# mmaker/c-lwe-snarks

Hardware: AMD Instinct MI355X
Metric: snark_proofs_per_sec (higher is better)
Workload: dtype u32 limbs (704-bit integers mod 2^704) + AES-256 bytes; int8 digits on the matrix cores, int32 accumulation (exact)

## Files before the change

### c-lwe-snarks_amd/__init__.py

```python
from __future__ import annotations

import ctypes
import os
from dataclasses import dataclass

import numpy as np

_HERE = os.path.dirname(os.path.abspath(__file__))
LIB_PATH = os.environ.get("MFHIP_LIB") or os.path.join(_HERE, "libmfhip.so")
P = 0xFFFFFFFB


class MfhError(RuntimeError):
    pass


@dataclass(frozen=True)
class Params:

    n: int = 1470
    logq: int = 736
    d: int = 1 << 15
    m: int = 21845

# ... 4 lines not shown
    @property
    def K(self):
        return self.logq // 64

    @property
    def lanes(self):
        return (64 * self.K + 55) // 56

    @property
    def ctb(self):
        return self.logq // 8

    @property
    def ctr_ct(self):
        return self.ctb * self.n

    @property
    def ctr_s(self):
        return 0

    @property
    def ctr_as(self):
        return self.ctr_ct * self.d

    @property
    def ctr_bt(self):
        return 2 * self.ctr_ct * self.d

    @property
    def ctr_bv(self):
        return 2 * self.ctr_ct * self.d + self.ctr_ct

    @property
    def ct_limbs(self):
        return (self.n + 1) * self.L


DEBUG = Params(d=256, m=64)
DEFAULT = Params()


class _CParams(ctypes.Structure):
    _fields_ = [("n", ctypes.c_uint32), ("logq", ctypes.c_uint32), ("d", ctypes.c_uint32), ("m", ctypes.c_uint32)]


_lib = None

EXPORTS = [
    "mfh_ctx_create", "mfh_ctx_destroy", "mfh_set_stream", "mfh_sync", "mfh_scrub_staging", "mfh_last_error", "mfh_set_seed",
    "mfh_keystream", "mfh_sample_rows", "mfh_ct_add", "mfh_ct_mul_ui", "mfh_ct_addmul_ui", "mfh_eval_rows",
    "mfh_encrypt_rows", "mfh_decrypt", "mfh_ct_smudge", "mfh_ssp_upload", "mfh_witness_poly", "mfh_version",
    "mfh_workspace_bytes", "mfh_last_kernel_ms", "mfh_set_timing", "mfh_set_overlap", "mfh_eval_rows_multi", "mfh_prove_batch", "mfh_crs_mm_image_bytes", "mfh_crs_expand_mm", "mfh_crs_set_resident_mm", "mfh_witness_poly_multi", "mfh_witness_poly_mm", "mfh_poly_h_multi", "mfh_poly_mul", "mfh_poly_add", "mfh_poly_prepare_t",
    "mfh_ssp_prepare", "mfh_poly_h", "mfh_setup_messages", "mfh_setup", "mfh_setup_image", "mfh_crs_image_set_b", "mfh_prove",
    "mfh_prove_partial", "mfh_prove_finish", "mfh_ct_to_lanes", "mfh_ct_from_lanes", "mfh_lanes_per_value", "mfh_digest128", "mfh_timing_drain", "mfh_timing_busy_ms", "mfh_timing_work_rows", "mfh_set_batch_image", "mfh_set_batch_slabs", "mfh_set_expand_path", "mfh_set_expand_periods", "mfh_set_encrypt_path", "mfh_set_batch_launch", "mfh_set_batch_bw", "mfh_set_mm_chunk_rows", "mfh_set_mm_pack", "mfh_set_poly_exact", "mfh_poly_exact_fallbacks", "mfh_poly_exact_points", "mfh_set_poly_exact_points", "mfh_set_mm_stream", "mfh_add_dotp", "mfh_set_encrypt_chunks", "mfh_set_witness_per", "mfh_set_eval_path", "mfh_set_decrypt_path", "mfh_decrypt_rows",
    "mfh_crs_mm_share_bytes", "mfh_crs_expand_mm_share", "mfh_crs_set_resident_mm_share", "mfh_batch_chain", "mfh_batch_witness_cols", "mfh_batch_chain_from_w", "mfh_witness_poly_mm_cols", "mfh_prove_batch_partial", "mfh_prove_batch_finish",
    "mfh_resident_row_bytes", "mfh_crs_expand", "mfh_eval_rows_resident", "mfh_crs_set_resident",
    "mfh_witness_lanes", "mfh_witness_from_lanes", "mfh_prove_partial_w", "mfh_verify",
    "mfh_ssp_set_prg", "mfh_ssp_prg_make_t", "mfh_ssp_prg_fill",
    "mfh_resident_share_rows", "mfh_crs_expand_share", "mfh_crs_set_resident_share", "mfh_crs_set_resident_prefix",
    "mfh_prove_batch_supergroup", "mfh_prove_batch_stream_wait", "mfh_set_mm_width", "mfh_set_mm_queue", "mfh_set_mm_claim_log", "mfh_mm_claim_log_launches",
    "mfh_setup_public", "mfh_prove_public", "mfh_prove_batch_public", "mfh_vk_derive", "mfh_verify_public",
    "mfh_ssp_from_rows", "mfh_ssp_set_rows", "mfh_ssp_rows_fill", "mfh_ssp_rows_violations", "mfh_circuit_create", "mfh_circuit_destroy", "mfh_circuit_assign",
    "mfh_circuit_create_global", "mfh_circuit_create_ex", "mfh_circuit_create_out", "mfh_circuit_create_sum",
    "mfh_merkle_create", "mfh_merkle_destroy", "mfh_merkle_set_leaves", "mfh_merkle_root", "mfh_merkle_nodes", "mfh_merkle_paths",
    "mfh_sha256_records", "mfh_merkle_set_records", "mfh_merkle_update_rows", "mfh_merkle_update_records",
    "mfh_merkle_absent_rows", "mfh_merkle_insert_keys", "mfh_merkle_update_rows_cut", "mfh_merkle_update_records_cut", "mfh_merkle_insert_keys_cut",
    "mfh_merkle_remove_keys", "mfh_merkle_remove_keys_cut", "mfh_merkle_transfer_keys", "mfh_merkle_transfer_keys_cut",
    "mfh_merkle_paths_cut", "mfh_merkle_absent_rows_cut", "mfh_merkle_range_rows", "mfh_merkle_range_rows_cut",
    "mfh_merkle_load_keys", "mfh_merkle_check_table", "mfh_merkle_grow", "mfh_merkle_grow_leaves",
]


OPTIONAL_EXPORTS = {
    "mfh_set_mm_queue": "tuning knob; older builds walk fixed lists",
    "mfh_set_mm_claim_log": "test instrumentation of mfh_set_mm_queue",
    "mfh_mm_claim_log_launches": "test instrumentation of mfh_set_mm_queue",
    "mfh_set_expand_periods": "test knob; older builds pick the periods per chunk from the row count",
}


def load_library():
    global _lib
    if _lib is not None:
        return _lib
    if not os.path.exists(LIB_PATH):
        raise MfhError(f"{LIB_PATH} is missing: run `python -c 'import __graft_entry__ as g; g.build()'` "
                       "(hipcc --offload-arch=gfx950).  There is no CPU fallback.")
    lib = ctypes.CDLL(LIB_PATH)
    vp, u64, sz, i32, u32 = ctypes.c_void_p, ctypes.c_uint64, ctypes.c_size_t, ctypes.c_int, ctypes.c_uint32
    sig = {
        "mfh_ctx_create": (i32, [ctypes.POINTER(vp), i32, ctypes.POINTER(_CParams)]),
        "mfh_ctx_destroy": (None, [vp]),
        "mfh_set_stream": (i32, [vp, vp]),
        "mfh_sync": (i32, [vp]),
        "mfh_scrub_staging": (i32, [vp]),
        "mfh_last_error": (ctypes.c_char_p, [vp]),
        "mfh_set_seed": (i32, [vp, ctypes.c_char_p]),
        "mfh_keystream": (i32, [vp, u64, vp, sz]),
        "mfh_sample_rows": (i32, [vp, u64, sz, vp]),
        "mfh_ct_add": (i32, [vp, vp, vp, vp, sz]),
        "mfh_ct_mul_ui": (i32, [vp, vp, vp, u32, sz]),
        "mfh_ct_addmul_ui": (i32, [vp, vp, vp, u32, sz]),
        "mfh_eval_rows": (i32, [vp, u64, sz, vp, vp, vp, vp, vp, i32]),
        "mfh_encrypt_rows": (i32, [vp, u64, sz, vp, vp, vp, vp]),
        "mfh_decrypt": (i32, [vp, vp, vp, sz, vp]),
        "mfh_ct_smudge": (i32, [vp, vp, sz, ctypes.c_char_p, sz, ctypes.c_char_p]),
        "mfh_ssp_upload": (i32, [vp, vp, vp, sz, sz]),
        "mfh_witness_poly": (i32, [vp, vp, ctypes.c_char_p, u32, vp]),
        "mfh_version": (ctypes.c_char_p, []),
        "mfh_workspace_bytes": (sz, [vp]),
        "mfh_last_kernel_ms": (ctypes.c_float, [vp, ctypes.c_char_p]),
        "mfh_set_timing": (i32, [vp, i32]),
        "mfh_set_overlap": (i32, [vp, i32]),
        "mfh_eval_rows_multi": (i32, [vp, u64, sz, vp, vp, u32, u32, vp, i32]),
        "mfh_poly_h_multi": (i32, [vp, vp, vp, u32]),
        "mfh_witness_poly_mm": (i32, [vp, vp, u32, ctypes.c_char_p, sz, vp, vp]),
        "mfh_witness_poly_multi": (i32, [vp, vp, u32, ctypes.c_char_p, sz, vp, vp]),
        "mfh_crs_mm_image_bytes": (sz, [vp]),
        "mfh_crs_expand_mm": (i32, [vp, vp, vp]),
        "mfh_crs_set_resident_mm": (i32, [vp, vp]),
        "mfh_prove_batch": (i32, [vp, vp, vp, u32, ctypes.c_char_p, sz, vp, ctypes.c_char_p, sz, ctypes.c_char_p, vp]),
        "mfh_prove_batch_supergroup": (u32, [vp]),
        "mfh_set_mm_width": (i32, [vp, u32, i32]),
        "mfh_set_mm_queue": (i32, [vp, i32, u32, i32]),
        "mfh_set_mm_claim_log": (i32, [vp, vp, sz]),
        "mfh_mm_claim_log_launches": (u32, [vp, ctypes.POINTER(u32), u32]),
        "mfh_prove_batch_stream_wait": (i32, [vp, u32, vp]),
        "mfh_poly_mul": (i32, [vp, vp, sz, vp, sz, vp]),
        "mfh_poly_add": (i32, [vp, vp, vp, sz, vp]),
        "mfh_poly_prepare_t": (i32, [vp, vp]),
        "mfh_ssp_prepare": (i32, [vp, vp]),
        "mfh_poly_h": (i32, [vp, vp, vp]),
        "mfh_setup_messages": (i32, [vp, vp, u32, u32, u32, vp]),
        "mfh_setup": (i32, [vp, vp, u32, u32, u32, vp, vp, vp]),
        "mfh_setup_image": (i32, [vp, vp, u32, u32, u32, vp, vp, vp, vp]),
        "mfh_prove": (i32, [vp, vp, vp, ctypes.c_char_p, u32, ctypes.c_char_p, sz, ctypes.c_char_p, vp]),
        "mfh_prove_partial": (i32, [vp, vp, vp, ctypes.c_char_p, u32, u32, u32, vp]),
        "mfh_prove_finish": (i32, [vp, vp, ctypes.c_char_p, sz, ctypes.c_char_p]),
        "mfh_lanes_per_value": (u32, [vp]),
        "mfh_digest128": (i32, [vp, vp, sz, vp]),
        "mfh_ct_to_lanes": (i32, [vp, vp, sz, vp]),
        "mfh_ct_from_lanes": (i32, [vp, vp, sz, vp]),
        "mfh_add_dotp": (i32, [vp, vp, vp, vp, sz]),
        "mfh_crs_set_resident_prefix": (i32, [vp, vp, sz]),
        "mfh_resident_share_rows": (sz, [vp, u32, u32]),
        "mfh_crs_expand_share": (i32, [vp, vp, u32, u32, vp]),
        "mfh_crs_set_resident_share": (i32, [vp, vp, u32, u32]),
        "mfh_ssp_set_prg": (i32, [vp, u64, vp]),
        "mfh_ssp_prg_make_t": (i32, [vp, u64, ctypes.c_char_p, vp]),
        "mfh_ssp_prg_fill": (i32, [vp, u64, sz, sz, vp]),
        "mfh_verify": (i32, [vp, vp, u32, u32, u32, vp, vp, sz, vp]),
        "mfh_witness_lanes": (i32, [vp, vp, ctypes.c_char_p, u32, u32, vp]),
        "mfh_witness_from_lanes": (i32, [vp, vp, vp, u32, vp]),
        "mfh_prove_partial_w": (i32, [vp, vp, vp, ctypes.c_char_p, u32, u32, u32, vp, vp]),
        "mfh_resident_row_bytes": (sz, [vp]),
        "mfh_crs_expand": (i32, [vp, u64, sz, vp, vp]),
        "mfh_crs_image_set_b": (i32, [vp, sz, sz, vp, vp]),
        "mfh_eval_rows_resident": (i32, [vp, vp, sz, sz, vp, vp, vp, vp, i32]),
        "mfh_crs_set_resident": (i32, [vp, vp]),
        "mfh_timing_drain": (i32, [vp, ctypes.c_char_p, ctypes.POINTER(u64), ctypes.POINTER(ctypes.c_double), ctypes.POINTER(u64),
                                   ctypes.POINTER(ctypes.c_float)]),
        "mfh_timing_busy_ms": (ctypes.c_double, [vp]),
        "mfh_timing_work_rows": (u64, [vp]),
        "mfh_set_batch_image": (i32, [vp, i32]),
        "mfh_set_mm_chunk_rows": (i32, [vp, u32]),
        "mfh_set_mm_pack": (i32, [vp, i32]),
        "mfh_set_poly_exact": (i32, [vp, i32]),
        "mfh_poly_exact_fallbacks": (ctypes.c_long, [vp]),
        "mfh_poly_exact_points": (i32, [vp, ctypes.POINTER(u32)]),
        "mfh_set_poly_exact_points": (i32, [vp, ctypes.POINTER(u32)]),
        "mfh_set_mm_stream": (i32, [vp, i32, i32, i32, u32]),
        "mfh_set_batch_launch": (i32, [vp, u32, i32]),
        "mfh_set_batch_bw": (i32, [vp, i32]),
        "mfh_set_encrypt_path": (i32, [vp, i32]),
        "mfh_set_expand_path": (i32, [vp, i32]),
        "mfh_set_expand_periods": (i32, [vp, u32]),
        "mfh_set_batch_slabs": (i32, [vp, u32]),
        "mfh_set_encrypt_chunks": (i32, [vp, u32]),
        "mfh_set_eval_path": (i32, [vp, i32]),
        "mfh_set_decrypt_path": (i32, [vp, i32]),
        "mfh_decrypt_rows": (i32, [vp, u64, sz, vp, vp, vp]),
        "mfh_set_witness_per": (i32, [vp, u32]),
        "mfh_crs_mm_share_bytes": (sz, [vp, u32, u32]),
        "mfh_crs_expand_mm_share": (i32, [vp, vp, u32, u32, vp]),
        "mfh_crs_set_resident_mm_share": (i32, [vp, vp, u32, u32]),
        "mfh_batch_chain": (i32, [vp, vp, u32, ctypes.c_char_p, sz, vp, vp, vp, vp]),
        "mfh_batch_witness_cols": (i32, [vp, vp, u32, ctypes.c_char_p, sz, vp, u32, u32, vp, sz]),
        "mfh_batch_chain_from_w": (i32, [vp, vp, u32, vp, vp, vp]),
        "mfh_witness_poly_mm_cols": (i32, [vp, vp, u32, ctypes.c_char_p, sz, vp, u32, u32, vp, sz]),
        "mfh_prove_batch_partial": (i32, [vp, vp, u32, u32, u32, ctypes.c_char_p, sz, vp, vp, vp, sz, vp]),
        "mfh_prove_batch_finish": (i32, [vp, vp, u32, vp, ctypes.c_char_p, sz, ctypes.c_char_p, vp]),
        "mfh_setup_public": (i32, [vp, vp, u32, u32, u32, u32, vp, vp, vp, vp]),
        "mfh_prove_public": (i32, [vp, vp, vp, u32, ctypes.c_char_p, u32, ctypes.c_char_p, sz, ctypes.c_char_p, vp]),
        "mfh_prove_batch_public": (i32, [vp, vp, vp, u32, u32, ctypes.c_char_p, sz, vp, ctypes.c_char_p, sz, ctypes.c_char_p, vp]),
        "mfh_vk_derive": (i32, [vp, vp, u32, u32, vp]),
        "mfh_verify_public": (i32, [vp, vp, u32, u32, u32, vp, vp, ctypes.c_char_p, sz, sz, vp]),
        "mfh_ssp_from_rows": (i32, [vp, u32, vp, vp, vp, vp]),
        "mfh_ssp_set_rows": (i32, [vp, u32, vp, vp, vp, u32]),
        "mfh_ssp_rows_fill": (i32, [vp, sz, sz, vp]),
        "mfh_ssp_rows_violations": (i32, [vp, u32, vp, sz, vp, vp]),
        "mfh_circuit_create": (i32, [vp, u32, u32, vp, u32, vp, ctypes.POINTER(vp)]),
        "mfh_circuit_create_global": (i32, [vp, u32, u32, vp, u32, vp, ctypes.POINTER(vp)]),
        "mfh_circuit_create_ex": (i32, [vp, u32, u32, vp, u32, vp, u32, vp, u32, ctypes.POINTER(vp)]),
        "mfh_circuit_create_out": (i32, [vp, u32, u32, vp, u32, vp, u32, vp, u32, vp, u32, ctypes.POINTER(vp)]),
        "mfh_circuit_create_sum": (i32, [vp, u32, u32, vp, u32, vp, u32, vp, u32, vp, u32, vp, u32, ctypes.POINTER(vp)]),
        "mfh_circuit_destroy": (None, [vp]),
        "mfh_circuit_assign": (i32, [vp, vp, u32, vp, sz, vp, sz, vp]),
        "mfh_merkle_create": (i32, [vp, u32, ctypes.POINTER(vp)]),
        "mfh_merkle_destroy": (None, [vp]),
        "mfh_merkle_set_leaves": (i32, [vp, vp, u32, u32, vp]),
        "mfh_merkle_root": (i32, [vp, vp, vp]),
        "mfh_merkle_nodes": (i32, [vp, u32, ctypes.POINTER(vp)]),
        "mfh_merkle_paths": (i32, [vp, vp, u32, vp, vp, sz]),
        "mfh_sha256_records": (i32, [vp, vp, sz, u32, u32, vp]),
        "mfh_merkle_set_records": (i32, [vp, vp, u32, u32, vp, sz, u32]),
        "mfh_merkle_update_rows": (i32, [vp, vp, u32, vp, vp, vp, sz, vp]),
        "mfh_merkle_update_records": (i32, [vp, vp, u32, vp, vp, sz, u32, vp, sz, vp, sz, vp]),
        "mfh_merkle_absent_rows": (i32, [vp, vp, vp, sz, u32, u32, u32, vp, sz, vp, sz, vp, vp]),
        "mfh_merkle_insert_keys": (i32, [vp, vp, vp, sz, u32, u32, u32, vp, sz, vp, sz, vp, sz, vp, vp, vp]),
        "mfh_merkle_update_rows_cut": (i32, [vp, vp, u32, vp, vp, u32, vp, vp, vp, vp]),
        "mfh_merkle_update_records_cut": (i32, [vp, vp, u32, vp, vp, sz, u32, vp, sz, u32, vp, vp, vp, vp]),
        "mfh_merkle_insert_keys_cut": (i32, [vp, vp, vp, sz, u32, u32, u32, vp, sz, vp, sz, u32, vp, vp, vp, vp, vp, vp]),
        "mfh_merkle_remove_keys": (i32, [vp, vp, vp, sz, u32, u32, u32, vp, sz, vp, sz, vp, vp, vp]),
        "mfh_merkle_remove_keys_cut": (i32, [vp, vp, vp, sz, u32, u32, u32, vp, sz, u32, vp, vp, vp, vp, vp, vp]),
        "mfh_merkle_transfer_keys": (i32, [vp, vp, vp, sz, u32, u32, u32, u32, vp, vp, sz, vp, vp, sz, vp, vp, vp]),
        "mfh_merkle_transfer_keys_cut": (i32, [vp, vp, vp, sz, u32, u32, u32, u32, vp, vp, sz, vp, u32, vp, vp, vp, vp, vp, vp]),
# ... 784 lines not shown

    def sync(self):
        self._chk(self.lib.mfh_sync(self._h))

    def set_stream(self, stream):
        self._chk(self.lib.mfh_set_stream(self._h, ctypes.c_void_p(stream.cuda_stream if stream is not None else 0)))

    def scrub_staging(self):
        rc = self.lib.mfh_scrub_staging(self._h)
        self._chk(rc)
        return rc

    def workspace_bytes(self):
        return int(self.lib.mfh_workspace_bytes(self._h))

    def set_timing(self, on=True):
        self._chk(self.lib.mfh_set_timing(self._h, 1 if on else 0))

    def set_overlap(self, mode=1):
        self._chk(self.lib.mfh_set_overlap(self._h, int(mode)))

    def set_batch_image(self, on=True):
        self._chk(self.lib.mfh_set_batch_image(self._h, 1 if on else 0))

    def set_batch_slabs(self, nslabs=0):
        self._chk(self.lib.mfh_set_batch_slabs(self._h, int(nslabs)))

    def set_expand_path(self, path=0):
        self._chk(self.lib.mfh_set_expand_path(self._h, int(path)))

    def set_expand_periods(self, periods=0):
        if not 0 <= int(periods) <= 0xFFFFFFFF:
            raise MfhError("set_expand_periods: 0 or 2 .. 10")
        self._chk(self.lib.mfh_set_expand_periods(self._h, int(periods)))

    def set_encrypt_path(self, path=0):
        self._chk(self.lib.mfh_set_encrypt_path(self._h, int(path)))

    def set_eval_path(self, path=0):
        self._chk(self.lib.mfh_set_eval_path(self._h, int(path)))

    def set_encrypt_chunks(self, chunks=0):
        self._chk(self.lib.mfh_set_encrypt_chunks(self._h, int(chunks)))

    def set_witness_per(self, statements=0):
        self._chk(self.lib.mfh_set_witness_per(self._h, int(statements)))

    def set_batch_launch(self, groups_per_launch=4, merge_regions=True):
        self._chk(self.lib.mfh_set_batch_launch(self._h, int(groups_per_launch), 1 if merge_regions else 0))

    def set_batch_bw(self, merged=True):
        self._chk(self.lib.mfh_set_batch_bw(self._h, 1 if merged else 0))

    def set_mm_stream(self, map=0, persistent=False, sync_mode=0, spin_max=64):
        self._chk(self.lib.mfh_set_mm_stream(self._h, int(map), int(persistent), int(sync_mode), int(spin_max)))

    def set_mm_width(self, per_xcd=32, early_chain=False):
        self._chk(self.lib.mfh_set_mm_width(self._h, int(per_xcd), 1 if early_chain else 0))

    def set_mm_queue(self, mode=1, start_shift=0, prefix=-8):
        self._chk(self.lib.mfh_set_mm_queue(self._h, int(mode), int(start_shift), int(prefix)))

    def set_mm_claim_log(self, log):
        if log is None:
            self._chk(self.lib.mfh_set_mm_claim_log(self._h, None, 0))
        else:
            self._chk(self.lib.mfh_set_mm_claim_log(self._h, log.data_ptr(), log.numel()))

    def mm_claim_log_launches(self):
        out = (ctypes.c_uint32 * (16 * 12))()
        n = int(self.lib.mfh_mm_claim_log_launches(self._h, out, 16))
        keys = ("offset", "nchunks", "nblk", "ngt", "ngr", "map", "tgs", "width", "coeff_bytes", "queue", "prefix", "shift")
        return [dict(zip(keys, (int(x) for x in out[12 * i:12 * i + 12]))) for i in range(n)]

    def set_mm_pack(self, on=True):
        self._chk(self.lib.mfh_set_mm_pack(self._h, 1 if on else 0))

    def set_poly_exact(self, mode=1):
        self._chk(self.lib.mfh_set_poly_exact(self._h, int(mode)))

    def poly_exact_fallbacks(self):
        return int(self.lib.mfh_poly_exact_fallbacks(self._h))

    def exact_points(self):
        out = (ctypes.c_uint32 * 4)()
        self._chk(self.lib.mfh_poly_exact_points(self._h, out))
        return [int(x) for x in out]

    def set_exact_points(self, pts):
        if pts is None:
            self._chk(self.lib.mfh_set_poly_exact_points(self._h, None))
            return
        pts = [int(x) for x in pts]
        if len(pts) != 4 or not all(0 <= x < 2**32 for x in pts):
            raise MfhError(f"set_exact_points: four uint32 values, got {pts!r}")
        self._chk(self.lib.mfh_set_poly_exact_points(self._h, (ctypes.c_uint32 * 4)(*pts)))

    def set_mm_chunk_rows(self, rows=0):
        self._chk(self.lib.mfh_set_mm_chunk_rows(self._h, int(rows)))

    def timing_drain(self, which):
        n, rows, ms, last = ctypes.c_uint64(), ctypes.c_uint64(), ctypes.c_double(), ctypes.c_float()
        self._chk(self.lib.mfh_timing_drain(self._h, which.encode(), ctypes.byref(n), ctypes.byref(ms), ctypes.byref(rows), ctypes.byref(last)))
        return n.value, ms.value, rows.value

    def timing_busy_ms(self):
# ... 196 lines not shown
    def poly_h(self, d_v):
        out = self.empty(self.params.d * 4)
        self._chk(self.lib.mfh_poly_h(self._h, _ptr(d_v), _ptr(out)))
        return out

    def poly_h_many(self, d_v, nb):
        out = self.empty(nb * self.params.d * 4)
        self._chk(self.lib.mfh_poly_h_multi(self._h, _ptr(d_v), _ptr(out), nb))
        return out

    def setup_messages(self, d_ssp, alpha, beta, s):
        p = self.params
        out = self.empty((2 * p.d + p.m) * 4)
        self._chk(self.lib.mfh_setup_messages(self._h, _ptr(d_ssp), alpha, beta, s, _ptr(out)))
        return out

    def setup(self, d_ssp, alpha, beta, s, d_sk, d_err, out=None):
        p = self.params
        out = self.empty((2 * p.d + p.m) * p.ctb) if out is None else out
        self._chk(self.lib.mfh_setup(self._h, _ptr(d_ssp), alpha, beta, s, _ptr(d_sk), _ptr(d_err), _ptr(out)))
        return out

    def setup_image(self, d_ssp, alpha, beta, s, d_sk, d_err, out=None, rows=None):
        p = self.params
        out = self.empty((2 * p.d + p.m) * p.ctb) if out is None else out
        rows = self.empty((2 * p.d + p.m) * self.resident_row_bytes()) if rows is None else rows
        self._chk(self.lib.mfh_setup_image(self._h, _ptr(d_ssp), alpha, beta, s, _ptr(d_sk), _ptr(d_err), _ptr(out), _ptr(rows)))
        return out, rows

    def prove(self, d_crs, d_ssp, witness_bits: bytes, delta, smudge_mag: bytes, smudge_sign: bytes, maglen=80, out=None):
        p = self.params
        out = self.empty(5 * p.ct_limbs * 8) if out is None else out
        assert len(smudge_mag) == 5 * maglen and len(smudge_sign) == 5
        self._chk(self.lib.mfh_prove(self._h, _ptr(d_crs), _ptr(d_ssp), bytes(witness_bits), delta, bytes(smudge_mag), maglen,
                                     bytes(smudge_sign), _ptr(out)))
        return out

    def crs_expand_mm(self, d_crs, out=None):
        out = self.empty(int(self.lib.mfh_crs_mm_image_bytes(self._h))) if out is None else out
        self._chk(self.lib.mfh_crs_expand_mm(self._h, _ptr(d_crs), _ptr(out)))
        return out

    def set_resident_mm(self, image):
        self._resident_mm = image
        self._chk(self.lib.mfh_crs_set_resident_mm(self._h, _ptr(image)))

    def witness_poly_many(self, d_ssp, witness_bits_list, deltas, mm=True):
        p = self.params
        nb = len(witness_bits_list)
        stride = (p.m + 6) // 8
        bits = b"".join(bytes(w[:stride]).ljust(stride, b"\0") for w in witness_bits_list)
        dl = (ctypes.c_uint32 * nb)(*[int(x) for x in deltas])
        out = self.empty(nb * p.d * 4)
        fn = self.lib.mfh_witness_poly_mm if mm else self.lib.mfh_witness_poly_multi
        self._chk(fn(self._h, _ptr(d_ssp), nb, bits, stride, ctypes.cast(dl, ctypes.c_void_p), _ptr(out)))
        return out

    def prove_batch(self, d_crs, d_ssp, witness_bits_list, deltas, smudge_mags, smudge_signs, maglen=80, out=None):
        p = self.params
        nb = len(witness_bits_list)
        stride = (p.m + 6) // 8
        bits = b"".join(bytes(w[:stride]).ljust(stride, b"\0") for w in witness_bits_list)
        dl = (ctypes.c_uint32 * nb)(*[int(x) for x in deltas])
        mags = b"".join(bytes(x) for x in smudge_mags)
        signs = b"".join(bytes(x) for x in smudge_signs)
        assert len(mags) == nb * 5 * maglen and len(signs) == nb * 5
        out = self.empty(nb * 5 * p.ct_limbs * 8) if out is None else out
        self._chk(self.lib.mfh_prove_batch(self._h, _ptr(d_crs), _ptr(d_ssp), nb, bits, stride, ctypes.cast(dl, ctypes.c_void_p), mags, maglen,
                                           signs, _ptr(out)))
        return out

    def prove_batch_supergroup(self):
        return int(self.lib.mfh_prove_batch_supergroup(self._h))

    def prove_batch_stream_wait(self, upto, stream):
        self._chk(self.lib.mfh_prove_batch_stream_wait(self._h, int(upto), ctypes.c_void_p(stream.cuda_stream)))

    def _pack_bits(self, witness_bits_list):
        stride = (self.params.m + 6) // 8
        return b"".join(bytes(w[:stride]).ljust(stride, b"\0") for w in witness_bits_list), stride

    def crs_expand_mm_share(self, d_crs, rank, world, out=None):
        out = self.empty(int(self.lib.mfh_crs_mm_share_bytes(self._h, rank, world))) if out is None else out
        self._chk(self.lib.mfh_crs_expand_mm_share(self._h, _ptr(d_crs), rank, world, _ptr(out)))
        return out

    def set_resident_mm_share(self, image, rank, world):
        self._resident_mm = image
        self._chk(self.lib.mfh_crs_set_resident_mm_share(self._h, _ptr(image), rank, world))

    def batch_chain(self, d_ssp, witness_bits_list, deltas, out=None):
        p = self.params
        nb = len(witness_bits_list)
        out = self.torch.empty((3, nb, p.d), dtype=self.torch.int32, device=self.device) if out is None else out
        if nb == 0:
            return out
        bits, stride = self._pack_bits(witness_bits_list)
        dl = (ctypes.c_uint32 * nb)(*[int(x) for x in deltas])
        self._chk(self.lib.mfh_batch_chain(self._h, _ptr(d_ssp), nb, bits, stride, ctypes.cast(dl, ctypes.c_void_p), _ptr(out[0]), _ptr(out[1]), _ptr(out[2])))
        return out

    def batch_witness_cols(self, d_ssp, witness_bits_list, deltas, col0, ncols, out=None):
        nb = len(witness_bits_list)
        out = self.torch.empty((nb, ncols), dtype=self.torch.int32, device=self.device) if out is None else out
        if nb == 0 or ncols == 0:
            return out
        bits, stride = self._pack_bits(witness_bits_list)
# ... 178 lines not shown
```

### c-lwe-snarks_amd/csrc/ctx.hpp

```cpp
#pragma once
#include <hip/hip_runtime.h>

#include <stdint.h>
#include <string.h>

#include <string>
#include <vector>

#include "aes_dev.hpp"
#include "mfhip.h"
#include "ssp_prg.hpp"

#define HIP_TRY(ctx, expr)                                                        \
  do {                                                                            \
    hipError_t e_ = (expr);                                                       \
    if (e_ != hipSuccess) {                                                       \
      (ctx)->err = std::string(#expr) + ": " + hipGetErrorString(e_);             \
      return MFH_EDEVICE;                                                         \
    }                                                                             \
  } while (0)

struct PolyState;
struct SspInterp;
struct SspRows;
// ... 12 lines not shown
  size_t cap = 0;
  template <class T> T *as() const { return static_cast<T *>(p); }
};

struct mfh_ctx {
  mfh_params P{};
  int device = 0;
  hipStream_t own_stream = nullptr;
  hipStream_t stream = nullptr;
  mf::AesKey key{};
  bool have_seed = false;
  uint32_t *d_t0 = nullptr;
  DevBuf ws;
  DevBuf ws2;
  int mm_ws_sel = 0;
  DevBuf ws3;
  std::vector<hipEvent_t> ev_cdone, ev_rdone, ev_wdone;
  std::vector<hipEvent_t> ev_round;
  std::vector<hipEvent_t> ev_sgdone;
  uint32_t last_batch_sg = 0, last_batch_n = 0;
  DevBuf wws;
  DevBuf lazy;
  uint32_t *lazy_cnt = nullptr;
  bool eval_dense = false;
  bool overlap = true;
  int overlap_mode = 1;
  hipStream_t side = nullptr, side2 = nullptr;
  hipEvent_t ev_fork = nullptr, ev_join = nullptr;
  hipEvent_t ev_chain = nullptr, ev_chain_done = nullptr;
  std::string err;
  bool timing = false;
  struct Timed {
    hipEvent_t e0, e1;
    int kind;
    uint64_t rows;
    uint64_t work;
    int sub;
  };
  std::vector<Timed> timed;
  double last_busy_ms = 0;
  uint64_t last_work_rows = 0;
  std::vector<hipEvent_t> ev_pool;
  PolyState *poly = nullptr;
  DevBuf aux;
  DevBuf d_msg;
  DevBuf d_prover;
  std::vector<uint32_t> h_cw;
  const uint8_t *mm_image = nullptr;
  uint32_t mm_rank = 0, mm_world = 1;
  uint64_t mm_off[3] = {0, 0, 0}, mm_rows[3] = {0, 0, 0};
  size_t mm_base[3] = {0, 0, 0};
  DevBuf ssp_frag;
  const uint32_t *ssp_frag_src = nullptr;
  SspInterp *interp = nullptr;
  DevBuf circ_io;
  DevBuf circ_state;
  DevBuf d_batch;
  DevBuf batch_img;
  int batch_image = 1;
  int mm_map = 1;
  bool mm_persist = true;
  bool mm_wave1 = false;
  uint32_t mm_sync_mode = 0, mm_spin = 64;
  uint32_t mm_width = 32;
  size_t early_ws_half = 0;
  bool batch_early_chain = false;
  uint32_t *mm_sync = nullptr;
  uint32_t mm_queue = 1, mm_queue_shift = 0; int mm_queue_prefix = -8;
  uint32_t *mm_log = nullptr; size_t mm_log_words = 0, mm_log_used = 0; uint32_t mm_log_n = 0, mm_log_desc[16][12];
  int poly_exact = 1;
  bool poly_pts_pinned = false;
  uint32_t poly_pts[4] = {0, 0, 0, 0};
  bool mm_pack = true;
  uint32_t mm_chunk_rows = 131071;
  int expand_path = 0;
  uint32_t expand_periods = 0;
  int enc_path = 0;
  uint32_t ncu = 256;
  int dec_path = 0;
  int eval_path = 0;
  uint32_t enc_chunks = 0;
  uint32_t witness_per = 0;
  uint32_t batch_slabs = 0;
  int batch_bw_merged = 1;
  int batch_merge = 1;
  uint32_t batch_ngl = 8;
  PinBuf pin_rows, pin_cw, pin_smudge;
  PinBuf pin_pub;
  DevBuf d_pub;
  PinBuf pin_wring[8];
  uint32_t pin_wnext = 0;
  hipEvent_t ev_sample = nullptr;
  DevBuf sample_tmp;
  void *uploader = nullptr;
  bool prg_on = false;
  uint64_t prg_seed = 0;
  const uint32_t *prg_t = nullptr;
  SspRows *rows = nullptr;
  RowsTree *rows_tree = nullptr;
  const uint32_t *rows_prefix = nullptr;
  uint32_t rows_lu_max = 0;
  const uint8_t *resident_rows = nullptr;
  uint64_t resident_nrows = ~0ull;
  bool resident_sharded = false;
  uint32_t res_rank = 0, res_world = 1;
};

struct Timer {
  mfh_ctx *c;
  mfh_ctx::Timed t{};
  bool on;
  Timer(mfh_ctx *c_, int kind, uint64_t rows, uint64_t work = 0, int sub = 0) : c(c_), on(c_->timing) {
    if (!on) return;
    auto get = [&]() {
      hipEvent_t e;
      if (!c->ev_pool.empty()) { e = c->ev_pool.back(); c->ev_pool.pop_back(); }
      else hipEventCreate(&e);
      return e;
    };
    t.e0 = get(); t.e1 = get(); t.kind = kind; t.rows = rows; t.work = work ? work : rows; t.sub = sub;
    hipEventRecord(t.e0, c->stream);
  }
  ~Timer() {
    if (!on) return;
    hipEventRecord(t.e1, c->stream);
    c->timed.push_back(t);
  }
};

inline void *pin_acquire(mfh_ctx *c, PinBuf &b, size_t bytes) {
  if (b.pending) { hipEventSynchronize(b.ev); b.pending = false; }
  if (bytes > b.cap) {
    if (b.p) hipHostFree(b.p);
    b.cap = (bytes + 4095) & ~(size_t)4095;
    if (hipHostMalloc(&b.p, b.cap, hipHostMallocDefault) != hipSuccess) { b.p = nullptr; b.cap = 0; c->err = "hipHostMalloc failed"; return nullptr; }
  }
  if (!b.ev) hipEventCreateWithFlags(&b.ev, hipEventDisableTiming);
  b.used = bytes;
  return b.p;
}
inline void pin_release(mfh_ctx *c, PinBuf &b) {
  hipEventRecord(b.ev, c->stream);
  b.pending = true;
}
inline void pin_scrub(PinBuf &b) {
  if (b.pending) { hipEventSynchronize(b.ev); b.pending = false; }
  if (b.p && b.used) {
    volatile unsigned char *q = (volatile unsigned char *)b.p;
    memset((void *)q, 0, b.used);
    __asm__ __volatile__("" : : "r"(b.p) : "memory");
  }
  b.used = 0;
}
inline void pin_free(PinBuf &b) {
  if (b.pending) hipEventSynchronize(b.ev);
  if (b.p) hipHostFree(b.p);
  if (b.ev) hipEventDestroy(b.ev);
  b = PinBuf();
}

// ... 55 lines not shown
    return MFH_OK;
  }
  if (!c->prg_on || !c->prg_t) { c->err = "d_ssp is NULL and no generator-defined SSP is registered (mfh_ssp_set_prg)"; return MFH_EINVAL; }
  src = mf::SspSrc{nullptr, c->prg_t, c->prg_seed};
  return MFH_OK;
}

void mfh_poly_destroy(mfh_ctx *c);
void ssp_interp_free(mfh_ctx *c);
void ssp_rows_free(mfh_ctx *c, bool tree);
int ssp_rows_check(mfh_ctx *c, const char *who, uint32_t nrows, const uint32_t *h_row_ptr, const uint32_t *h_wire, const uint32_t *h_coef);
int ssp_rows_tree(mfh_ctx *c, const char *who, const uint32_t *&d_t, const uint32_t *&h_w);
int ssp_rows_witness(mfh_ctx *c, uint32_t nstmt, const uint8_t *h_bits, size_t bits_stride, const uint32_t *h_delta, uint32_t *d_w, size_t w_stride);
int ssp_rows_msg_evals(mfh_ctx *c, uint32_t s, uint32_t beta, uint32_t *d_msg_evals);
inline bool ssp_is_rows(const mfh_ctx *c, const uint32_t *d_ssp) { return !d_ssp && c->rows_prefix; }
inline int ssp_rows_lu_check(mfh_ctx *c, const uint32_t *d_ssp, uint32_t lu) {
  if (ssp_is_rows(c, d_ssp) && lu > c->rows_lu_max) { c->err = "lu exceeds the lu_max the row SSP was registered with (mfh_ssp_set_rows)"; return MFH_EINVAL; }
  return MFH_OK;
}
extern "C" int mfh_witness_poly_mm(mfh_ctx *c, const uint32_t *d_ssp, uint32_t nstmt, const uint8_t *h_bits, size_t bits_stride, const uint32_t *h_delta,
                                   uint32_t *d_w);
extern "C" int mfh_witness_poly_mm_cols(mfh_ctx *c, const uint32_t *d_ssp, uint32_t nstmt, const uint8_t *h_bits, size_t bits_stride, const uint32_t *h_delta,
                                        uint32_t col0, uint32_t ncols, uint32_t *d_w, size_t w_stride);
extern "C" int mfh_poly_h_multi(mfh_ctx *c, const uint32_t *d_v, uint32_t *d_h, uint32_t nb);
int expand_mm_region(mfh_ctx *c, uint64_t off, uint32_t nrows, const uint8_t *c8, uint8_t *image);
int encrypt_rows_mm(mfh_ctx *c, uint64_t off, size_t nrows, const uint64_t *sk, const uint32_t *msg, const uint64_t *err, uint8_t *c8);
int decrypt_mm(mfh_ctx *c, const uint64_t *sk, const uint64_t *cts, size_t count, uint32_t *out);
int decrypt_rows_mm(mfh_ctx *c, uint64_t off, size_t nrows, const uint64_t *sk, const uint8_t *c8, uint32_t *out);

struct MmIo {
  const uint32_t *coef[2];
  uint32_t csplit;
  uint64_t *out[2];
  uint32_t osplit;
  uint64_t ostride;
  const uint8_t *bits;
  uint32_t bits_stride;
  int64_t *sc_zeroed;
  uint64_t cstride;
  uint32_t bits_row0;
  const uint64_t *add_ct;
  const uint32_t *add_scale;
  uint32_t sa_from1;
};
int eval_rows_multi_io(mfh_ctx *c, uint64_t off, size_t nrows, const uint8_t *d_c8, const MmIo &io, uint32_t nvec, uint32_t coeff_bytes, int accumulate);
int eval_rows_multi_io_set(mfh_ctx *c, uint64_t off, size_t nrows, const uint8_t *d_c8, const MmIo *ios, const uint32_t *nvecs, uint32_t ng,
                           uint32_t coeff_bytes);
struct MmRegion { uint64_t off; const uint8_t *c8; };
int eval_rows_multi_io_regions(mfh_ctx *c, const MmRegion *regs, uint32_t nreg, size_t nrows, const MmIo *ios, const uint32_t *nvecs, uint32_t ng,
                               uint32_t coeff_bytes, int accumulate);
bool mm_image_covers(const mfh_ctx *c, uint64_t off, size_t nrows);
struct MmsPlan {
  uint32_t ng, ngt, ND, nrows, nchunks, rpc, rpad, ntiles, mtiles;
  size_t cd_bytes, part_bytes;
  const uint8_t *img[2];
  int8_t *cd;
  int *part;
};
bool mms_plan(mfh_ctx *c, const MmRegion *regs, uint32_t nreg, size_t nrows, const MmIo *ios, const uint32_t *nvecs, uint32_t ng, uint32_t coeff_bytes,
              MmsPlan &P);
size_t mms_ws_bytes(const MmsPlan &P);
void mms_bind(MmsPlan &P, void *ws);
int mms_digits(mfh_ctx *c, const MmsPlan &P, const MmIo *ios, const uint32_t *nvecs);
int mms_stream(mfh_ctx *c, const MmsPlan &P);
int mms_finish(mfh_ctx *c, const MmsPlan &P, const MmIo *ios, const uint32_t *nvecs, int accumulate);
```

### c-lwe-snarks_amd/csrc/evalmm.hip

```cpp
#include <algorithm>
#include <cstring>

#include "ctx.hpp"
#include "mms_slots.hpp"

namespace {

using mf::AesKey;

constexpr int CT = 4;
constexpr int SB = 88;
constexpr int VB = 92;
constexpr int MB = CT * SB;
constexpr int MT = MB / 32;
constexpr int RT = 128;
constexpr int TSTRIDE = 384;
constexpr int BLK_PER_ROW = 24;
static_assert(MB % 32 == 0 && CT * VB + 15 <= TSTRIDE, "tile geometry");

typedef int v4i __attribute__((ext_vector_type(4)));
typedef int v16i __attribute__((ext_vector_type(16)));

__device__ __forceinline__ uint32_t coef_at(const MmIo &io, uint32_t v, uint32_t nrows, uint32_t i) {
  if (io.bits) {
// ... 943 lines not shown
      sv[l][1][vl] = (uint32_t)(val >> 32);
      sv[l][2][vl] = (uint32_t)(val >> 64);
    }
  }
  __syncthreads();
  if (lq != 0 || v >= nvec) return;
  uint32_t *out = reinterpret_cast<uint32_t *>((v < io.osplit ? io.out[0] + (uint64_t)v * io.ostride : io.out[1] + (uint64_t)(v - io.osplit) * io.ostride) +
                                               (uint64_t)j * LL);
  const bool wide4 = (LL & 1) == 0 && (io.ostride & 1) == 0 && ((reinterpret_cast<uintptr_t>(io.out[0]) | reinterpret_cast<uintptr_t>(io.out[1])) & 15) == 0;
  uint32_t pend[4] = {0, 0, 0, 0};
  uint64_t carry = 0;
  const uint32_t *actw = io.add_ct ? reinterpret_cast<const uint32_t *>(io.add_ct + (uint64_t)j * LL) : nullptr;
  const uint64_t ax = io.add_ct ? io.add_scale[v] : 0;
  uint64_t acarry = 0;
  for (uint32_t l = 0; l < KWv; l++) {
    uint64_t word = carry + sv[l][0][vl];
    if (l >= 1) word += sv[l - 1][1][vl];
    if (l >= 2) word += sv[l - 2][2][vl];
    if (accumulate) word += out[l];
    if (actw) {
      const uint64_t t = (uint64_t)actw[l] * ax + acarry;
      word += (uint32_t)t;
      acarry = t >> 32;
    }
    carry = word >> 32;
    pend[l & 3] = (uint32_t)word;
    if (wide4 ? (l & 3) == 3 : (l & 1) == 1) {
      if (wide4) *reinterpret_cast<uint4 *>(out + (l & ~3u)) = uint4{pend[0], pend[1], pend[2], pend[3]};
      else *reinterpret_cast<uint2 *>(out + (l & ~1u)) = uint2{pend[(l & 2)], pend[(l & 2) + 1]};
    }
  }
  if (wide4) {
    if (KWv & 3) *reinterpret_cast<uint4 *>(out + (KWv & ~3u)) = uint4{pend[0], (KWv & 3) > 1 ? pend[1] : 0u, (KWv & 3) > 2 ? pend[2] : 0u, 0u};
    for (uint32_t l = (KWv + 3) & ~3u; l < 2 * LL; l += 4) *reinterpret_cast<uint4 *>(out + l) = uint4{0u, 0u, 0u, 0u};
  } else {
    if (KWv & 1) *reinterpret_cast<uint2 *>(out + (KWv & ~1u)) = uint2{pend[(KWv & 2)], 0u};
    for (uint32_t l = (KWv + 1) & ~1u; l < 2 * LL; l += 2) *reinterpret_cast<uint2 *>(out + l) = uint2{0u, 0u};
  }
}

template <int ND, int KWM, bool PK>
__global__ __launch_bounds__(256) void k_evalmm_finish(const int *__restrict__ part, const int64_t *__restrict__ sc, uint32_t nchunks, uint32_t ntiles,
                                                        uint32_t N, uint32_t nvec, uint32_t n, uint32_t nrows, uint32_t ct, uint32_t MBv, uint32_t sby,
                                                        uint32_t LL, MmIo io, int accumulate) {
  evalmm_finish_body<ND, KWM, PK>(part, sc, nchunks, ntiles, N, nvec, n, nrows, ct, MBv, sby, LL, io, accumulate, part, ND * nvec);
}
template <int ND, int KWM, bool PK>
__global__ __launch_bounds__(256) void k_evalmm_finish_groups(const int *__restrict__ part, uint64_t part_stride, uint32_t nchunks, uint32_t ntiles, uint32_t N,
                                                               uint32_t n, uint32_t nrows, uint32_t ct, uint32_t MBv, uint32_t sby, uint32_t LL, MmGroupArgs A,
                                                               int accumulate) {
  const uint32_t g = blockIdx.z, lender = A.io[g].sa_from1 ? A.io[g].sa_from1 - 1 : g;
  evalmm_finish_body<ND, KWM, PK>(part + g * part_stride, A.io[g].sc_zeroed, nchunks, ntiles, N, A.nvec[g], n, nrows, ct, MBv, sby, LL, A.io[g], accumulate,
                                  part + lender * part_stride, ND * A.nvec[lender]);
}

}

extern "C" {

struct WideGeom { uint32_t ct, sby, vby, mt, mbp, LL; };
static WideGeom wide_geom(const mfh_ctx *c) {
  if (c->P.logq == 736) return {W16<736>::CT, W16<736>::SBY, W16<736>::VBY, W16<736>::MT, W16<736>::MBP, W16<736>::LL};
  return {W16<1472>::CT, W16<1472>::SBY, W16<1472>::VBY, W16<1472>::MT, W16<1472>::MBP, W16<1472>::LL};
}

#define FINISH_LAUNCH(kern, ND_, PK_, grid, ...)                                                                         \
  do {                                                                                                                   \
    if ((PK_) && wg.sby / 4 <= 22) hipLaunchKernelGGL((kern<ND_, 22, true>), grid, dim3(256), 0, c->stream, __VA_ARGS__);  \
    else if (PK_) hipLaunchKernelGGL((kern<ND_, 46, true>), grid, dim3(256), 0, c->stream, __VA_ARGS__);                 \
    else if (wg.sby / 4 <= 22) hipLaunchKernelGGL((kern<ND_, 22, false>), grid, dim3(256), 0, c->stream, __VA_ARGS__);   \
    else hipLaunchKernelGGL((kern<ND_, 46, false>), grid, dim3(256), 0, c->stream, __VA_ARGS__);                         \
  } while (0)

int mfh_eval_rows_multi(mfh_ctx *c, uint64_t off, size_t nrows, const uint8_t *d_c8, const uint32_t *d_coeffs, uint32_t nvec, uint32_t coeff_bytes,
                        uint64_t *d_rops, int accumulate) {
  if (!c || !d_rops || !nvec || (nrows && (!d_c8 || !d_coeffs)) || (coeff_bytes != 1 && coeff_bytes != 4)) return MFH_EINVAL;
  const MmIo io = {{d_coeffs, nullptr}, nvec, {d_rops, nullptr}, nvec, (uint64_t)(c->P.n + 1) * wide_geom(c).LL, nullptr, 0, nullptr};
  return eval_rows_multi_io(c, off, nrows, d_c8, io, nvec, coeff_bytes, accumulate);
}

}

int eval_rows_multi_io(mfh_ctx *c, uint64_t off, size_t nrows, const uint8_t *d_c8, const MmIo &io, uint32_t nvec, uint32_t coeff_bytes, int accumulate) {
  if (!c || !nvec || !io.out[0] || (io.osplit < nvec && !io.out[1]) || (coeff_bytes != 1 && coeff_bytes != 4)) return MFH_EINVAL;
  if (nrows && (!d_c8 || (!io.bits && (!io.coef[0] || (io.csplit < nvec && !io.coef[1]))) || (io.bits && coeff_bytes != 1))) return MFH_EINVAL;
  const uint32_t ND = coeff_bytes;
  const uint32_t n = c->P.n;
  const bool q736 = c->P.logq == 736;
  const WideGeom wg = wide_geom(c);
  const uint8_t *img_region = nullptr;
  for (int r = 0; r < 3 && c->mm_image; r++)
    if (c->mm_off[r] == off && c->mm_rows[r] == nrows && nrows) img_region = c->mm_image + c->mm_base[r];
  const bool wide = img_region || !q736 || nvec * ND + 1 > 128;
  if (nvec * ND + 1 > 256) { c->err = "mfh_eval_rows_multi: at most 63 four-byte (255 one-byte) coefficient vectors per call (256 digit columns)"; return MFH_EINVAL; }
  if (wide && ((off & 7) || (((uint64_t)n * wg.vby) & 7))) {
    c->err = "mfh_eval_rows_multi: the 256-column kernel needs off and the row length to be multiples of 8";
    return MFH_EINVAL;
  }
  if (!c->have_seed) { c->err = "mfh_set_seed has not been called"; return MFH_EINVAL; }
  if (nrows > 0xffffffffu - 256) return MFH_EINVAL;
  HIP_TRY(c, hipSetDevice(c->device));
  const size_t ctl = (size_t)(n + 1) * wg.LL;
  if (io.ostride < ctl) return MFH_EINVAL;
  if (nrows == 0) {
    const uint32_t n0 = std::min(nvec, io.osplit);
    if (!accumulate) {
// ... 100 lines not shown
}
size_t mms_ws_bytes(const MmsPlan &P) { return (size_t)P.ngt * (P.cd_bytes + P.part_bytes); }
void mms_bind(MmsPlan &P, void *ws) {
  P.cd = (int8_t *)ws;
  P.part = (int *)((uint8_t *)ws + (size_t)P.ngt * P.cd_bytes);
}
static bool mms_group_args(const MmsPlan &P, const MmIo *ios, const uint32_t *nvecs, MmGroupArgs &A) {
  if (P.ND != 4) return false;
  for (uint32_t g = 0; g < P.ngt; g++) {
    if (ios[g].bits) return false;
    A.io[g] = ios[g];
    A.nvec[g] = nvecs[g];
  }
  return true;
}
int mms_digits(mfh_ctx *c, const MmsPlan &P, const MmIo *ios, const uint32_t *nvecs) {
  MmGroupArgs A;
  if (mms_group_args(P, ios, nvecs, A)) {
    hipLaunchKernelGGL(k_mm_digits4w_groups, dim3((P.rpad / 16 + DG4 - 1) / DG4, P.ngt), dim3(256), 0, c->stream, A, P.nrows, P.rpad, P.cd, (uint64_t)P.cd_bytes);
    HIP_TRY(c, hipGetLastError());
    return MFH_OK;
  }
  for (uint32_t g = 0; g < P.ngt; g++) {
    if (P.ND == 4 && !ios[g].bits)
      hipLaunchKernelGGL(k_mm_digits4w, dim3((P.rpad / 16 + DG4 - 1) / DG4), dim3(256), 0, c->stream, ios[g], nvecs[g], P.nrows, P.rpad, P.cd + g * P.cd_bytes,
                         ios[g].sc_zeroed);
    else
      hipLaunchKernelGGL(k_mm_digits, dim3((P.rpad / 16 + DG_RG - 1) / DG_RG), dim3(N2), 0, c->stream, ios[g], nvecs[g], P.ND, P.nrows, P.rpad, (uint32_t)NQ2, 1,
                         P.cd + g * P.cd_bytes, ios[g].sc_zeroed);
  }
  HIP_TRY(c, hipGetLastError());
  return MFH_OK;
}
static bool mms_persistent(const mfh_ctx *c, const MmsPlan &P) {
  return P.ngt > 1 && c->mm_persist && c->ncu == 256 && ((c->mm_map && 32 % P.ng == 0) || 32 % P.ngt == 0);
}
static uint32_t mms_pk(const mfh_ctx *c, const MmsPlan &P) {
  if (!c->mm_pack || (mms_persistent(c, P) && c->mm_wave1)) return 0;
  return P.ND;
}
#ifdef MMS_ITEM_STAMPS
static unsigned long long *g_mms_stamps = nullptr;
static uint32_t g_mms_stamp_n = 0, g_mms_stamp_kind[64];
static unsigned long long *mms_stamps_next(uint32_t nd, uint32_t queue) {
  if (!g_mms_stamps && hipMalloc(&g_mms_stamps, 64 * 256 * 4 * sizeof(unsigned long long)) != hipSuccess) return nullptr;
  if (g_mms_stamp_n == 64) return nullptr;
  g_mms_stamp_kind[g_mms_stamp_n] = nd | queue << 8;
  return g_mms_stamps + (size_t)g_mms_stamp_n++ * 256 * 4;
}
#endif
int mms_stream(mfh_ctx *c, const MmsPlan &P) {
  const uint32_t KS = (P.nrows + RT2 - 1) / RT2 * (RT2 / 64), tgs = (P.mtiles + TPW - 1) / TPW;
  const bool will_persist = mms_persistent(c, P);
  Timer t(c, P.ngt > 1 ? (P.ND == 1 ? 14 : 10) : 8, P.nrows, (uint64_t)P.nrows * P.ngt, will_persist ? 1 : 0);
  MmsImages imgs{};
  for (uint32_t g = 0; g < P.ngt; g++) imgs.image[g] = (const v4i *)P.img[g / P.ng];
  const uint32_t pk = mms_pk(c, P);
  if (P.ngt > 1) {
    const uint32_t map = c->mm_map && 32 % P.ng == 0 ? 1u : 0u;
    const uint32_t slots = mms_slots(tgs, P.ngt, P.ng, map);
    const bool persistent = will_persist;
    if (persistent && c->mm_wave1) {
      hipLaunchKernelGGL(k_mmstream_w, dim3(256), dim3(WSW * 64), 0, c->stream, imgs, P.mtiles, KS, P.nrows, P.rpc, (const v4i *)P.cd, P.part, P.ngt, P.ng, map,
                         (uint64_t)(P.cd_bytes / 16), (uint64_t)(P.part_bytes / 4), (slots + 31) / 32, P.nchunks);
    } else if (persistent) {
      constexpr size_t SYNC_WORDS = 8 * 32 + 2 * 8;
      if (!c->mm_sync) HIP_TRY(c, hipMalloc(&c->mm_sync, SYNC_WORDS * sizeof(uint32_t)));
      const uint32_t width = P.ND == 1 ? 32u : c->mm_width;
      const uint32_t sync_mode = width == 32 ? c->mm_sync_mode : 0u, nblk = (slots + 31) / 32;
      uint32_t *qctr = c->mm_sync + 8 * 32 + 8 * (c->mm_ws_sel ? 1 : 0);
      MmsQueue q{qctr, nullptr, c->mm_queue && !sync_mode ? 1u : 0u, c->mm_queue_shift & 7, 0u, tgs};
      if (q.mode && !q.shift && nblk * 32 % width == 0) {
        const uint32_t rounds = P.nchunks * (nblk * 32 / width);
        q.prefix = c->mm_queue_prefix < 0 ? rounds - std::min(rounds, (uint32_t)-(int64_t)c->mm_queue_prefix) : std::min(rounds, (uint32_t)c->mm_queue_prefix);
      }
      if (sync_mode) HIP_TRY(c, hipMemsetAsync(c->mm_sync, 0, 8 * 32 * sizeof(uint32_t), c->stream));
      else if (q.mode) HIP_TRY(c, hipMemsetAsync(qctr, 0, 8 * sizeof(uint32_t), c->stream));
      if (c->mm_log) {
        const size_t need = (size_t)2 * P.nchunks * 8 * nblk * 32;
        if (c->mm_log_n == 16 || c->mm_log_used + need > c->mm_log_words) { c->err = "mfh_set_mm_claim_log: the log is too small for the call's launches"; return MFH_EINVAL; }
        q.log = c->mm_log + c->mm_log_used;
        const uint32_t desc[12] = {(uint32_t)c->mm_log_used, P.nchunks, nblk, P.ngt, P.ng, map, tgs, width, P.ND, q.mode, q.prefix, q.shift};
        memcpy(c->mm_log_desc[c->mm_log_n++], desc, sizeof(desc));
        c->mm_log_used += need;
      }
#ifdef MMS_ITEM_STAMPS
      unsigned long long *stamps = mms_stamps_next(P.ND, q.mode);
      if (!stamps) { c->err = "MMS_ITEM_STAMPS: no room for another launch"; return MFH_EINVAL; }
#endif
      hipLaunchKernelGGL(P.ND == 1 ? k_mmstream_pb : k_mmstream_p, dim3(8 * width), dim3(SW * 64), 0, c->stream, imgs, P.mtiles, KS, P.nrows, P.rpc, (const v4i *)P.cd, P.part, P.ngt, P.ng, map,
                         (uint64_t)(P.cd_bytes / 16), (uint64_t)(P.part_bytes / 4), nblk, P.nchunks, c->mm_sync, sync_mode, c->mm_spin, width, pk, q MMS_STAMP_ARG);
    } else {
      hipLaunchKernelGGL(k_mmstream, dim3(slots * 8, P.nchunks), dim3(SW * 64), 0, c->stream, imgs, P.mtiles, KS, P.nrows, P.rpc, (const v4i *)P.cd, P.part, P.ngt, P.ng,
                         map, (uint64_t)(P.cd_bytes / 16), (uint64_t)(P.part_bytes / 4), pk);
    }
  } else
    hipLaunchKernelGGL(k_mmstream1, dim3((tgs + 7) / 8 * 8, P.nchunks), dim3(SW * 64), 0, c->stream, imgs, P.mtiles, KS, P.nrows, P.rpc, (const v4i *)P.cd, P.part, pk);
  HIP_TRY(c, hipGetLastError());
  return MFH_OK;
}
int mms_finish(mfh_ctx *c, const MmsPlan &P, const MmIo *ios, const uint32_t *nvecs, int accumulate) {
  const WideGeom wg = wide_geom(c);
  const uint32_t n = c->P.n;
  const uint32_t pk = mms_pk(c, P);
  MmGroupArgs A;
  if (mms_group_args(P, ios, nvecs, A)) {
    uint32_t nvmax = 0;
    for (uint32_t g = 0; g < P.ngt; g++) nvmax = std::max(nvmax, nvecs[g]);
    FINISH_LAUNCH(k_evalmm_finish_groups, 4, pk, dim3(n + 1, (nvmax + 63) / 64, P.ngt), P.part, (uint64_t)(P.part_bytes / 4), P.nchunks, P.ntiles, (uint32_t)N2, n, P.nrows,
                  wg.ct, wg.mbp, wg.sby, wg.LL, A, accumulate);
    HIP_TRY(c, hipGetLastError());
    return MFH_OK;
  }
  for (uint32_t g = 0; g < P.ngt; g++) {
    const dim3 fgrid(n + 1, (nvecs[g] + 63) / 64);
    int *pg = P.part + g * (P.part_bytes / 4);
    if (P.ND == 4)
      FINISH_LAUNCH(k_evalmm_finish, 4, pk, fgrid, pg, ios[g].sc_zeroed, P.nchunks, P.ntiles, (uint32_t)N2, nvecs[g], n, P.nrows, wg.ct, wg.mbp, wg.sby, wg.LL, ios[g],
                    accumulate);
    else
      FINISH_LAUNCH(k_evalmm_finish, 1, pk, fgrid, pg, ios[g].sc_zeroed, P.nchunks, P.ntiles, (uint32_t)N2, nvecs[g], n, P.nrows, wg.ct, wg.mbp, wg.sby, wg.LL, ios[g],
                    accumulate);
  }
  HIP_TRY(c, hipGetLastError());
  return MFH_OK;
}
int eval_rows_multi_io_regions(mfh_ctx *c, const MmRegion *regs, uint32_t nreg, size_t nrows, const MmIo *ios, const uint32_t *nvecs, uint32_t ng,
                               uint32_t coeff_bytes, int accumulate) {
  if (!c || !regs || !ios || !nvecs || !ng || !nreg || nreg * ng > 16) return MFH_EINVAL;
  MmsPlan P;
  if (!mms_plan(c, regs, nreg, nrows, ios, nvecs, ng, coeff_bytes, P)) {
    for (uint32_t g = 0; g < nreg * ng; g++) {
      int rc = eval_rows_multi_io(c, regs[g / ng].off, nrows, regs[g / ng].c8, ios[g], nvecs[g], coeff_bytes, accumulate);
      if (rc) return rc;
    }
    return MFH_OK;
  }
  HIP_TRY(c, hipSetDevice(c->device));
  int rc = c->mm_ws_sel ? ws2_reserve(c, mms_ws_bytes(P)) : ws_reserve(c, mms_ws_bytes(P));
  if (rc) return rc;
  mms_bind(P, (c->mm_ws_sel ? c->ws2 : c->ws).p);
  rc = mms_digits(c, P, ios, nvecs);
  if (!rc) rc = mms_stream(c, P);
  if (!rc) rc = mms_finish(c, P, ios, nvecs, accumulate);
  return rc;
}
int eval_rows_multi_io_set(mfh_ctx *c, uint64_t off, size_t nrows, const uint8_t *d_c8, const MmIo *ios, const uint32_t *nvecs, uint32_t ng,
                           uint32_t coeff_bytes) {
  const MmRegion reg = {off, d_c8};
  return eval_rows_multi_io_regions(c, &reg, 1, nrows, ios, nvecs, ng, coeff_bytes, 0);
}
bool mm_image_covers(const mfh_ctx *c, uint64_t off, size_t nrows) {
  for (int r = 0; r < 3 && c->mm_image; r++)
    if (c->mm_off[r] == off && c->mm_rows[r] == nrows && nrows) return true;
  return false;
}

extern "C" {

static size_t mm_region_bytes(const mfh_ctx *c, uint64_t rows) {
  const WideGeom wg = wide_geom(c);
  const uint64_t mtiles = (uint64_t)((c->P.n + 1 + wg.ct - 1) / wg.ct) * wg.mt, ksteps = (rows + RT2 - 1) / RT2 * (RT2 / 64);
  return (size_t)(mtiles * ksteps * 1024);
}
struct MmShare { uint64_t row0[3], rows[3]; };
static MmShare mm_share(const mfh_ctx *c, uint32_t rank, uint32_t world) {
  const uint64_t d = c->P.d, m = c->P.m;
  const uint64_t loS = d * rank / world, cS = d * (rank + 1) / world - loS, lo = m * rank / world, cnt = m * (rank + 1) / world - lo;
  return MmShare{{loS, d + loS, 2 * d + lo}, {cS, cS, cnt}};
}
size_t mfh_crs_mm_share_bytes(const mfh_ctx *c, uint32_t rank, uint32_t world) {
  if (!c || !world || rank >= world) return 0;
  const MmShare sh = mm_share(c, rank, world);
  return mm_region_bytes(c, sh.rows[0]) + mm_region_bytes(c, sh.rows[1]) + mm_region_bytes(c, sh.rows[2]);
}
size_t mfh_crs_mm_image_bytes(const mfh_ctx *c) { return mfh_crs_mm_share_bytes(c, 0, 1); }
int mfh_crs_expand_mm_share(mfh_ctx *c, const uint8_t *d_crs_c8, uint32_t rank, uint32_t world, uint8_t *d_image) {
  if (!c || !d_crs_c8 || !d_image || !world || rank >= world) return MFH_EINVAL;
  if (!c->have_seed) { c->err = "mfh_set_seed has not been called"; return MFH_EINVAL; }
// ... 115 lines not shown
```

### c-lwe-snarks_amd/csrc/mfhip.hip

```cpp
#include <hip/hip_runtime.h>

#include <stdint.h>
#include <stdio.h>
#include <string.h>

#include <algorithm>
#include <string>
#include <thread>
#include <vector>

#include "aes_dev.hpp"
#include "mfhip.h"

using mf::AesKey;

template <int LOGQ>
struct PS {
  static constexpr int CTB = LOGQ / 8;
  static constexpr int EW = CTB / 4;
  static constexpr int L = (LOGQ + 63) / 64;
  static constexpr int K = LOGQ / 64;
  static constexpr int KW = 2 * K;
  static constexpr int TILE = LOGQ == 736 ? 512 : 256;
  static constexpr int ROWS = 2;
// ... 819 lines not shown
  if (P->logq != 736 && P->logq != 1472) return MFH_EUNSUPPORTED;
  if (P->n == 0 || P->n > (1u << 20)) return MFH_EINVAL;
  int ndev = 0;
  if (hipGetDeviceCount(&ndev) != hipSuccess || ndev <= 0 || device < 0 || device >= ndev) return MFH_EDEVICE;
  if (hipSetDevice(device) != hipSuccess) return MFH_EDEVICE;
  mfh_ctx *c = new mfh_ctx();
  c->P = *P;
  c->device = device;
  {
    int ncu = 0;
    if (hipDeviceGetAttribute(&ncu, hipDeviceAttributeMultiprocessorCount, device) == hipSuccess && ncu > 0) c->ncu = (uint32_t)ncu;
  }
  if (hipStreamCreateWithFlags(&c->own_stream, hipStreamNonBlocking) != hipSuccess) {
    delete c;
    return MFH_EDEVICE;
  }
  c->stream = c->own_stream;
  uint32_t t0[512];
  mf::make_t0_le(t0);
  for (int a = 0; a < 256; a++) t0[256 + a] = (t0[a] << 24) | (t0[a] >> 8);
  if (hipMalloc(&c->d_t0, sizeof t0) != hipSuccess || hipMemcpy(c->d_t0, t0, sizeof t0, hipMemcpyHostToDevice) != hipSuccess) {
    mfh_ctx_destroy(c);
    return MFH_EDEVICE;
  }
  *out = c;
  return MFH_OK;
}

void mfh_ctx_destroy(mfh_ctx *c) {
  if (!c) return;
  hipSetDevice(c->device);
  if (c->stream) hipStreamSynchronize(c->stream);
  mfh_poly_destroy(c);
  ssp_interp_free(c);
  ssp_rows_free(c, true);
  upload_free(c);
  if (c->ev_sample) hipEventDestroy(c->ev_sample);
  pin_free(c->pin_rows);
  for (auto &b : c->pin_wring) pin_free(b);
  pin_free(c->pin_cw);
  pin_free(c->pin_smudge);
  pin_free(c->pin_pub);
  if (c->side) hipStreamSynchronize(c->side);
  if (c->mm_sync) hipFree(c->mm_sync);
  for (hipEvent_t e : c->ev_round) hipEventDestroy(e);
  for (hipEvent_t e : c->ev_sgdone) hipEventDestroy(e);
  for (hipEvent_t e : c->ev_cdone) hipEventDestroy(e);
  for (hipEvent_t e : c->ev_rdone) hipEventDestroy(e);
  for (hipEvent_t e : c->ev_wdone) hipEventDestroy(e);
  if (c->ev_fork) hipEventDestroy(c->ev_fork);
  if (c->ev_join) hipEventDestroy(c->ev_join);
  if (c->ev_chain) hipEventDestroy(c->ev_chain);
  if (c->ev_chain_done) hipEventDestroy(c->ev_chain_done);
  if (c->side) hipStreamDestroy(c->side);
  if (c->side2) hipStreamDestroy(c->side2);
  for (DevBuf *b : {&c->ws, &c->ws2, &c->ws3, &c->wws, &c->lazy, &c->aux, &c->d_msg, &c->d_prover, &c->d_pub, &c->d_batch, &c->batch_img, &c->circ_io,
                    &c->circ_state, &c->ssp_frag, &c->sample_tmp})
    dev_free(*b);
  if (c->d_t0) hipFree(c->d_t0);
  for (auto &t : c->timed) { hipEventDestroy(t.e0); hipEventDestroy(t.e1); }
  for (auto e : c->ev_pool) hipEventDestroy(e);
  if (c->own_stream) hipStreamDestroy(c->own_stream);
  delete c;
}

int mfh_set_stream(mfh_ctx *c, void *s) {
  if (!c) return MFH_EINVAL;
  c->stream = (hipStream_t)s;
  return MFH_OK;
}

int mfh_sync(mfh_ctx *c) {
  if (!c) return MFH_EINVAL;
  HIP_TRY(c, hipStreamSynchronize(c->stream));
  return MFH_OK;
}

int mfh_scrub_staging(mfh_ctx *c) {
  if (!c) return MFH_EINVAL;
  pin_scrub(c->pin_rows);
  pin_scrub(c->pin_cw);
  pin_scrub(c->pin_smudge);
  for (auto &b : c->pin_wring) pin_scrub(b);
  return MFH_OK;
}

const char *mfh_last_error(const mfh_ctx *c) { return c ? c->err.c_str() : "null context"; }
size_t mfh_workspace_bytes(const mfh_ctx *c) { return c ? c->ws.cap : 0; }
int mfh_set_overlap(mfh_ctx *c, int en) {
  if (!c) return MFH_EINVAL;
  c->overlap = en != 0;
  c->overlap_mode = en > 1 ? en : 1;
  return MFH_OK;
}

int mfh_set_expand_path(mfh_ctx *c, int path) {
  if (!c || path < 0 || path > 1) return MFH_EINVAL;
  c->expand_path = path;
  return MFH_OK;
}

int mfh_set_expand_periods(mfh_ctx *c, uint32_t periods) {
  if (!c || (periods && (periods < EXPAND_MIN_PERIODS || periods > EXPAND_MAX_PERIODS))) return MFH_EINVAL;
  c->expand_periods = periods;
  return MFH_OK;
}

int mfh_set_encrypt_path(mfh_ctx *c, int path) {
  if (!c || path < 0 || path > 2) return MFH_EINVAL;
  c->enc_path = path;
  return MFH_OK;
}

int mfh_set_eval_path(mfh_ctx *c, int path) {
  if (!c || path < 0 || path > 1) return MFH_EINVAL;
  c->eval_path = path;
  return MFH_OK;
}
int mfh_set_encrypt_chunks(mfh_ctx *c, uint32_t chunks) {
  if (!c || chunks > 64) return MFH_EINVAL;
  c->enc_chunks = chunks;
  return MFH_OK;
}
int mfh_set_witness_per(mfh_ctx *c, uint32_t statements) {
  if (!c || (statements && (statements < 32 || statements > 256))) return MFH_EINVAL;
  c->witness_per = statements;
  return MFH_OK;
}
int mfh_set_batch_slabs(mfh_ctx *c, uint32_t nslabs) {
  if (!c || nslabs > 256) return MFH_EINVAL;
  c->batch_slabs = nslabs;
  return MFH_OK;
}

int mfh_set_batch_launch(mfh_ctx *c, uint32_t groups_per_launch, int merge_regions) {
  if (!c || groups_per_launch < 1 || groups_per_launch > 8) return MFH_EINVAL;
  c->batch_ngl = groups_per_launch;
  c->batch_merge = merge_regions != 0;
  return MFH_OK;
}

int mfh_set_batch_bw(mfh_ctx *c, int merged) {
  if (!c) return MFH_EINVAL;
  c->batch_bw_merged = merged != 0;
  return MFH_OK;
}

int mfh_set_batch_image(mfh_ctx *c, int en) {
  if (!c) return MFH_EINVAL;
  c->batch_image = en != 0;
  return en ? MFH_OK : batch_img_drop(c);
}

int mfh_set_timing(mfh_ctx *c, int en) {
  if (!c) return MFH_EINVAL;
  c->timing = en != 0;
  return MFH_OK;
}
static int timing_kind(const char *which) {
  if (!strcmp(which, "keystream")) return 0;
  if (!strcmp(which, "eval1")) return 1;
  if (!strcmp(which, "eval2")) return 2;
  if (!strcmp(which, "encrypt")) return 3;
  if (!strcmp(which, "eval")) return 12;
  if (!strcmp(which, "expand")) return 4;
  if (!strcmp(which, "mac1")) return 5;
  if (!strcmp(which, "mac2")) return 6;
  if (!strcmp(which, "evalmm")) return 7;
  if (!strcmp(which, "evalmm_resident")) return 8;
  if (!strcmp(which, "expandmm")) return 9;
  if (!strcmp(which, "decrypt")) return 11;
  if (!strcmp(which, "decrypt_rows")) return 13;
  if (!strcmp(which, "mmstream_bw")) return 14;
  if (!strcmp(which, "mmstream_rounds")) return 10;
  if (!strcmp(which, "mmstream_rounds_persistent")) return 110;
  if (!strcmp(which, "mmstream_bw_persistent")) return 114;
  if (!strcmp(which, "ssp_interp")) return 15;
  if (!strcmp(which, "circuit_assign")) return 16;
  if (!strcmp(which, "circuit_assign_global")) return 17;
  if (!strcmp(which, "circuit_assign_ex")) return 18;
  if (!strcmp(which, "circuit_assign_global_ex")) return 19;
  if (!strcmp(which, "circuit_assign_out")) return 20;
  if (!strcmp(which, "circuit_assign_global_out")) return 21;
  if (!strcmp(which, "circuit_assign_sum")) return 22;
  if (!strcmp(which, "circuit_assign_global_sum")) return 23;
  if (!strcmp(which, "ssp_rows_violations")) return 24;
  if (!strcmp(which, "merkle_level")) return 25;
  if (!strcmp(which, "merkle_paths")) return 26;
  if (!strcmp(which, "sha256_records")) return 27;
  if (!strcmp(which, "merkle_updates")) return 28;
  if (!strcmp(which, "merkle_record_rows")) return 29;
  if (!strcmp(which, "merkle_locate")) return 30;
  if (!strcmp(which, "merkle_absent_rows")) return 31;
  if (!strcmp(which, "merkle_inert")) return 32;
  if (!strcmp(which, "merkle_insert_records")) return 33;
  if (!strcmp(which, "merkle_segments")) return 34;
  if (!strcmp(which, "merkle_owners")) return 35;
  if (!strcmp(which, "merkle_remove_records")) return 36;
  if (!strcmp(which, "merkle_balances")) return 37;
  if (!strcmp(which, "merkle_transfer_records")) return 38;
  if (!strcmp(which, "merkle_climb_rows")) return 39;
  if (!strcmp(which, "merkle_range")) return 40;
  if (!strcmp(which, "merkle_range_order")) return 41;
  if (!strcmp(which, "merkle_adjust_records")) return 42;
  if (!strcmp(which, "merkle_balance_sum")) return 43;
  if (!strcmp(which, "merkle_sort")) return 44;
  if (!strcmp(which, "merkle_load")) return 45;
  if (!strcmp(which, "merkle_check")) return 46;
  if (!strcmp(which, "merkle_grow")) return 47;
  return -1;
}

int mfh_timing_drain(mfh_ctx *c, const char *which, uint64_t *count, double *total_ms, uint64_t *total_rows, float *last_ms) {
  if (!c || !which) return MFH_EINVAL;
  const int kind = timing_kind(which);
  if (kind < 0) return MFH_EINVAL;
  HIP_TRY(c, hipStreamSynchronize(c->stream));
  if (c->side) HIP_TRY(c, hipStreamSynchronize(c->side));
  uint64_t n = 0, rows = 0, work = 0;
  double tot = 0;
  float last = -1.f;
  std::vector<mfh_ctx::Timed> keep;
  std::vector<std::pair<float, float>> spans;
  hipEvent_t base = nullptr;
  for (auto &t : c->timed) {
    const bool match = t.kind == kind || (kind == 12 && (t.kind == 1 || t.kind == 2)) || (kind == 8 && (t.kind == 10 || t.kind == 14)) || (kind >= 100 && t.kind == kind - 100 && t.sub == 1);
    if (!match) { keep.push_back(t); continue; }
    float ms = 0;
    if (hipEventElapsedTime(&ms, t.e0, t.e1) == hipSuccess) {
      n++; tot += ms; rows += t.rows; work += t.work; last = ms;
      if (!base) base = t.e0;
      float s0 = 0;
      if (hipEventElapsedTime(&s0, base, t.e0) == hipSuccess) spans.emplace_back(s0, s0 + ms);
    }
  }
  std::sort(spans.begin(), spans.end());
  double busy = 0;
  float hi = -1e30f;
  for (auto &sp : spans) {
    if (sp.second <= hi) continue;
    busy += sp.second - std::max(sp.first, hi);
    hi = sp.second;
  }
  c->last_busy_ms = busy;
  c->last_work_rows = work;
  for (auto &t : c->timed) {
    const bool match = t.kind == kind || (kind == 12 && (t.kind == 1 || t.kind == 2)) || (kind == 8 && (t.kind == 10 || t.kind == 14)) || (kind >= 100 && t.kind == kind - 100 && t.sub == 1);
    if (!match) continue;
    c->ev_pool.push_back(t.e0);
    c->ev_pool.push_back(t.e1);
  }
  c->timed.swap(keep);
  if (count) *count = n;
  if (total_ms) *total_ms = tot;
  if (total_rows) *total_rows = rows;
  if (last_ms) *last_ms = last;
  return MFH_OK;
}

double mfh_timing_busy_ms(const mfh_ctx *c) { return c ? c->last_busy_ms : -1.0; }
uint64_t mfh_timing_work_rows(const mfh_ctx *c) { return c ? c->last_work_rows : 0; }

float mfh_last_kernel_ms(mfh_ctx *c, const char *which) {
  float last = -1.f;
  if (mfh_timing_drain(c, which, nullptr, nullptr, nullptr, &last) != MFH_OK) return -1.f;
  return last;
}

int mfh_set_seed(mfh_ctx *c, const uint8_t seed[40]) {
  if (!c || !seed) return MFH_EINVAL;
  mf::expand_key(c->key, seed);
// ... 441 lines not shown
  for (size_t i = 0; i < count; i++) {
    uint64_t carry = 0;
    for (uint32_t l = 0; l < KW; l++) {
      uint32_t w = 0;
      const size_t o = (size_t)l * 4;
      if (o < maglen) memcpy(&w, h_mag + i * maglen + o, std::min<size_t>(4, maglen - o));
      uint64_t t = (uint64_t)w * MFH_P + carry;
      up[i * KW + l] = (uint32_t)t;
      carry = t >> 32;
    }
  }
  memcpy(stage + ub, h_sign, count);
  int rc = aux_reserve(c, ub + count);
  if (rc) return rc;
  HIP_TRY(c, hipMemcpyAsync(c->aux.p, stage, ub + count, hipMemcpyHostToDevice, c->stream));
  pin_release(c, c->pin_smudge);
  DISPATCH_LOGQ(c, hipLaunchKernelGGL(k_smudge<736>, dim3(((uint32_t)count + 63) / 64), dim3(64), 0, c->stream, d_cts, c->P.n, c->aux.as<uint32_t>(),
                                      c->aux.as<uint8_t>() + ub, (uint32_t)count),
                hipLaunchKernelGGL(k_smudge<1472>, dim3(((uint32_t)count + 63) / 64), dim3(64), 0, c->stream, d_cts, c->P.n, c->aux.as<uint32_t>(),
                                   c->aux.as<uint8_t>() + ub, (uint32_t)count));
  HIP_TRY(c, hipGetLastError());
  return MFH_OK;
}

namespace {
constexpr size_t UP_CHUNK = (size_t)4 << 20;
constexpr int UP_T = 16;
struct UpLane {
  hipStream_t st = nullptr;
  hipEvent_t ev[2] = {nullptr, nullptr};
  uint8_t *pin[2] = {nullptr, nullptr};
  uint8_t *dev[2] = {nullptr, nullptr};
};
struct Uploader {
  UpLane lane[UP_T];
};
}
static void upload_free(mfh_ctx *c) {
  Uploader *u = (Uploader *)c->uploader;
  if (!u) return;
  for (auto &l : u->lane) {
    for (int i = 0; i < 2; i++) {
      if (l.pin[i]) hipHostFree(l.pin[i]);
      if (l.dev[i]) hipFree(l.dev[i]);
      if (l.ev[i]) hipEventDestroy(l.ev[i]);
    }
    if (l.st) hipStreamDestroy(l.st);
  }
  delete u;
  c->uploader = nullptr;
}
int mfh_ssp_upload(mfh_ctx *c, const void *h_ssp_u64, uint32_t *d_ssp, size_t first_slot, size_t nslots) {
  if (!c || !h_ssp_u64 || !d_ssp) return MFH_EINVAL;
  c->ssp_frag_src = nullptr;
  HIP_TRY(c, hipSetDevice(c->device));
  const size_t d = c->P.d;
  const size_t total = nslots * d * 8;
  if (!total) return MFH_OK;
  const uint8_t *src = (const uint8_t *)h_ssp_u64 + first_slot * d * 8;
  uint32_t *dst = d_ssp + first_slot * d;
  HIP_TRY(c, hipStreamSynchronize(c->stream));
  const size_t nchunks = (total + UP_CHUNK - 1) / UP_CHUNK;
  if (nchunks < 16) {
    void *stage = nullptr;
    HIP_TRY(c, hipMalloc(&stage, total));
    int rc = MFH_OK;
    if (hipMemcpyAsync(stage, src, total, hipMemcpyHostToDevice, c->stream) != hipSuccess) rc = MFH_EDEVICE;
    if (!rc) hipLaunchKernelGGL(k_ssp_reduce, dim3(2048), dim3(256), 0, c->stream, (const uint64_t *)stage, dst, (uint64_t)(total / 8));
    if (hipGetLastError() != hipSuccess || hipStreamSynchronize(c->stream) != hipSuccess) rc = MFH_EDEVICE;
    hipFree(stage);
    if (rc) c->err = "ssp upload failed";
    return rc;
  }
  static int nthreads = 0;
  if (!nthreads) {
    const char *e = getenv("MFH_UPLOAD_THREADS");
    const long want = e && *e ? atol(e) : 8;
    nthreads = (int)(want < 1 ? 1 : want > UP_T ? UP_T : want);
  }
  const int NT = nthreads;
  Uploader *u = (Uploader *)c->uploader;
  if (!u) c->uploader = u = new Uploader();
  for (int t = 0; t < NT; t++) {
    UpLane &l = u->lane[t];
    if (l.st) continue;
    bool ok = hipStreamCreateWithFlags(&l.st, hipStreamNonBlocking) == hipSuccess;
    for (int i = 0; ok && i < 2; i++)
      ok = hipEventCreateWithFlags(&l.ev[i], hipEventDisableTiming) == hipSuccess && hipHostMalloc((void **)&l.pin[i], UP_CHUNK, hipHostMallocDefault) == hipSuccess &&
           hipMalloc((void **)&l.dev[i], UP_CHUNK) == hipSuccess;
    if (!ok) {
      (void)hipGetLastError();
      upload_free(c);
      c->err = "ssp upload: no memory for the staging lanes";
      return MFH_ENOMEM;
    }
  }
  int failed[UP_T] = {};
  auto work = [&](int t) {
    if (hipSetDevice(c->device) != hipSuccess) { failed[t] = 1; return; }
    UpLane &l = u->lane[t];
    int slot = 0;
    bool used[2] = {false, false};
    for (size_t k = (size_t)t; k < nchunks; k += (size_t)NT, slot ^= 1) {
      const size_t off = k * UP_CHUNK, nb = std::min(UP_CHUNK, total - off);
      if (used[slot] && hipEventSynchronize(l.ev[slot]) != hipSuccess) { failed[t] = 1; return; }
      memcpy(l.pin[slot], src + off, nb);
      if (hipMemcpyAsync(l.dev[slot], l.pin[slot], nb, hipMemcpyHostToDevice, l.st) != hipSuccess) { failed[t] = 1; return; }
// ... 21 lines not shown
```

### c-lwe-snarks_amd/csrc/poly.hip

```cpp
#include <assert.h>
#include <errno.h>
#include <sys/syscall.h>
#include <unistd.h>

#include <algorithm>
#include <type_traits>

#include "ctx.hpp"
#include "ntt.hpp"

namespace {

#define MF_NEEDED(need, vs) do { if ((need) && (vs) >= *(need)) return; } while (0)

using namespace mf_ntt;

__device__ __forceinline__ uint32_t lz_mont(uint32_t a, uint32_t b, uint32_t p, uint32_t ninv) {
  uint64_t t = (uint64_t)a * b;
  uint32_t m = (uint32_t)t * ninv;
  return (uint32_t)((t + (uint64_t)m * p) >> 32);
}
__device__ __forceinline__ uint32_t lz_add(uint32_t a, uint32_t b, uint32_t p2) {
  uint32_t s = a + b;
  return min(s, s - p2);
// ... 860 lines not shown
    if (rc) return rc;
    hipLaunchKernelGGL(k_sub_const0, dim3(nb), dim3(64), 0, c->stream, S->d_tmp, 1u, Nmax, (const uint32_t *)nullptr);
    rc = poly_mul(c, {.a = S->d_tmp, .la = Nc, .lb = Nc, .bhat = S->d_That, .log_hat = logNc, .out = d_h, .keep = d, .nb = nb, .in_stride = Nmax, .out_stride = d,
                      .log_cyc = logNc});
    if (rc) return rc;
  }
  hipLaunchKernelGGL(k_exact_check, dim3(nb), dim3(1024), 0, c->stream, d_v, d_h, d, S->d_chk, Nc, uint4{S->chk_t[0], S->chk_t[1], S->chk_t[2], S->chk_t[3]},
                     S->d_need, S->h_seen);
  return MFH_OK;
}

int h_euclid(mfh_ctx *c, const uint32_t *d_v, uint32_t *d_h, uint32_t nb, const uint32_t *need) {
  PolyState *S = c->poly;
  const uint32_t d = S->d, n = S->n;
  const size_t Nmax = (size_t)1 << S->logmax;
  const uint32_t *map = need ? need + 2 : nullptr;
  int rc;
  if (S->dt >= 1) {
    rc = poly_mul(c, {.a = d_v, .la = d, .b = d_v, .lb = d, .out = S->d_tmp2, .keep = n, .nb = nb, .in_stride = d, .out_stride = Nmax, .need = need, .a_map = map,
                      .rev_top = (int64_t)(2 * d - 2), .nsrc = 2 * d - 1});
    if (rc) return rc;
    rc = poly_mul(c, {.a = S->d_tmp2, .la = n, .lb = n, .bhat = S->d_Ghat, .log_hat = S->logN2, .out = d_h, .keep = d, .nb = nb, .in_stride = Nmax, .out_stride = d,
                      .need = need, .out_map = map, .rev_top = (int64_t)n - 1, .nsrc = n});
    if (rc) return rc;
  } else {
    rc = poly_mul(c, {.a = d_v, .la = d, .b = d_v, .lb = d, .out = S->d_tmp, .keep = 2 * d - 1, .nb = nb, .in_stride = d, .out_stride = Nmax, .need = need,
                      .a_map = map});
    if (rc) return rc;
    hipLaunchKernelGGL(k_sub_const0, dim3(nb), dim3(64), 0, c->stream, S->d_tmp, 1u, Nmax, need);
    hipLaunchKernelGGL(k_reverse, dim3((n + 255) / 256, nb), dim3(256), 0, c->stream, S->d_tmp, (int64_t)(2 * d - 2), n, S->d_tmp2, Nmax, Nmax, need);
    rc = poly_mul(c, {.a = S->d_tmp2, .la = n, .lb = n, .bhat = S->d_Ghat, .log_hat = S->logN2, .out = S->d_tmp, .keep = n, .nb = nb, .in_stride = Nmax,
                      .out_stride = Nmax, .need = need});
    if (rc) return rc;
    hipLaunchKernelGGL(k_unreverse_pad, dim3((d + 255) / 256, nb), dim3(256), 0, c->stream, S->d_tmp, n, d, d_h, Nmax, (size_t)d, need, map);
  }
  HIP_TRY(c, hipGetLastError());
  return MFH_OK;
}

}

extern "C" {

int mfh_poly_mul(mfh_ctx *c, const uint32_t *d_a, size_t la, const uint32_t *d_b, size_t lb, uint32_t *d_c) {
  if (!c || !d_a || !d_b || !d_c || !la || !lb) return MFH_EINVAL;
  HIP_TRY(c, hipSetDevice(c->device));
  int rc = poly_init(c, std::max(ceil_log2(la + lb - 1), 1u));
  if (rc) return rc;
  return poly_mul(c, {.a = d_a, .la = (uint32_t)la, .b = d_b, .lb = (uint32_t)lb, .out = d_c, .keep = (uint32_t)(la + lb - 1)});
}

int mfh_poly_prepare_t(mfh_ctx *c, const uint32_t *d_t) {
  if (!c) return MFH_EINVAL;
  c->ssp_frag_src = nullptr;
  if (c->poly) {
    c->poly->have_t = false;
    c->poly->cyc = false;
  }
  if (!d_t) return MFH_EINVAL;
  HIP_TRY(c, hipSetDevice(c->device));
  const uint32_t d = c->P.d;
  std::vector<uint32_t> t(d);
  HIP_TRY(c, hipMemcpyAsync(t.data(), d_t, (size_t)d * 4, hipMemcpyDeviceToHost, c->stream));
  HIP_TRY(c, hipStreamSynchronize(c->stream));
  int64_t dt = -1;
  for (int64_t i = (int64_t)d - 1; i >= 0; i--)
    if (t[i]) { dt = i; break; }
  if (dt < 0) {
    c->err = "t(x) is the zero polynomial: (v^2-1)/t is undefined (nmod_poly_div would raise)";
    return MFH_EINVAL;
  }
  const uint32_t n = 2 * d - 1 - (uint32_t)dt;
  uint32_t logmax = std::max(ceil_log2((size_t)2 * d), ceil_log2((size_t)2 * n + dt + 2));
  int rc = poly_init(c, logmax);
  if (rc) return rc;
  PolyState *S = c->poly;
  S->have_t = false;
  S->d = d; S->dt = (uint32_t)dt; S->n = n;
  S->logN2 = std::max(ceil_log2((size_t)2 * n - 1), 1u);
  const uint32_t N2 = 1u << S->logN2;
  if ((rc = dev_reserve(c, S->d_G, (size_t)std::max(n, 2u) * 4 * 2))) return rc;
  if ((rc = dev_reserve(c, S->d_Ghat, (size_t)3 * N2 * 4))) return rc;
  if ((rc = dev_reserve(c, S->d_f, (size_t)(dt + 1) * 4))) return rc;
  hipLaunchKernelGGL(k_reverse, g1((uint32_t)dt + 1), dim3(256), 0, c->stream, d_t, dt, (uint32_t)dt + 1, S->d_f);
  if ((rc = newton_inverse(c, invp(t[dt])))) return rc;
  ntt_load(c, S->d_Ghat, N2, 1, {S->d_G, n});
  ntt_blocks_forward(c, S->d_Ghat, N2, S->logN2, 1);
  HIP_TRY(c, hipGetLastError());
  HIP_TRY(c, hipStreamSynchronize(c->stream));
  if ((rc = prepare_exact(c, d_t, t))) return rc;
  S->have_t = true;
  return MFH_OK;
}

int mfh_poly_h_multi(mfh_ctx *c, const uint32_t *d_v, uint32_t *d_h, uint32_t nb) {
  if (!c || !d_v || !d_h || !nb || nb > kMaxBatch) return MFH_EINVAL;
  PolyState *S = c->poly;
  if (!S || !S->have_t) {
    c->err = "mfh_poly_prepare_t has not been called for this SSP";
    return MFH_EINVAL;
  }
  HIP_TRY(c, hipSetDevice(c->device));
  int rc = poly_batch_reserve(c, S, nb);
  if (rc) return rc;
  const bool exact = exact_policy(c, nb);
  if (exact && (rc = h_exact(c, d_v, d_h, nb))) return rc;
  return h_euclid(c, d_v, d_h, nb, exact ? (const uint32_t *)S->d_need : nullptr);
// ... 48 lines not shown
```

### c-lwe-snarks_amd/csrc/snark.hip

```cpp
#include <algorithm>
#include <cstdlib>
#include <cstring>
#include <vector>

#include "ctx.hpp"
#include "p32.hpp"

namespace {

__device__ __forceinline__ uint32_t ssp_coef(const mf::SspSrc &src, uint32_t slot, uint32_t rowkey, uint32_t d, uint32_t k) {
  if (src.dense) return src.dense[(uint64_t)slot * d + k];
  return slot == 0 ? src.t[k] : mf::ssp_prg_coeff(rowkey, k);
}

__global__ void k_powers(uint32_t s, uint32_t d, uint32_t *__restrict__ pw) {
  uint32_t k = blockIdx.x * blockDim.x + threadIdx.x;
  if (k >= d) return;
  uint32_t r = 1, b = s, e = k;
  while (e) {
    if (e & 1) r = mulp(r, b);
    b = mulp(b, b);
    e >>= 1;
  }
  pw[k] = r;
// ... 559 lines not shown
      const uint64_t t = (uint64_t)w * P32 + carry;
      up[i * KW + l] = (uint32_t)t;
      carry = t >> 32;
    }
  }
  memcpy(st + ((uint8_t *)B.SMS - B.CW), h_sign, (size_t)nproofs * 5);
  HIP_TRY(c, hipMemcpyAsync(B.CW, st, total, hipMemcpyHostToDevice, c->stream));
  pin_release(c, c->pin_cw);
  return MFH_OK;
}
__global__ void k_smudge_batch(uint64_t *cts, uint32_t n, uint32_t L, uint32_t KW, const uint32_t *__restrict__ up, const uint8_t *__restrict__ sign,
                               uint32_t count, uint32_t per, uint32_t slot0, uint32_t uslot0) {
  const uint32_t i = blockIdx.x * blockDim.x + threadIdx.x;
  if (i >= count) return;
  const uint32_t pb = i / per, j = i % per;
  uint32_t *b = reinterpret_cast<uint32_t *>(cts + ((uint64_t)(pb * 5 + slot0 + j) * (n + 1) + n) * L);
  const uint32_t *u = up + (uint64_t)(pb * 5 + uslot0 + j) * KW;
  if (sign[pb * 5 + uslot0 + j] & 1) {
    uint32_t borrow = 0;
    for (uint32_t l = 0; l < KW; l++) {
      const uint64_t t = (uint64_t)b[l] - u[l] - borrow;
      b[l] = (uint32_t)t;
      borrow = (uint32_t)(t >> 63);
    }
  } else {
    uint32_t carry = 0;
    for (uint32_t l = 0; l < KW; l++) {
      const uint64_t t = (uint64_t)b[l] + u[l] + carry;
      b[l] = (uint32_t)t;
      carry = (uint32_t)(t >> 32);
    }
  }
  for (uint32_t l = KW; l < 2 * L; l++) b[l] = 0;
}
int batch_smudge_staged(mfh_ctx *c, const BatchScratch &B, uint64_t *sproofs, uint32_t s0, uint32_t sg) {
  const uint32_t L = (c->P.logq + 63) / 64, KW = 2 * (c->P.logq / 64);
  const uint32_t *up = B.SMU + (size_t)s0 * 5 * KW;
  const uint8_t *sn = B.SMS + (size_t)s0 * 5;
  hipLaunchKernelGGL(k_smudge_batch, dim3((sg * 4 + 63) / 64), dim3(64), 0, c->stream, sproofs, c->P.n, L, KW, up, sn, sg * 4, 4u, 0u, 0u);
  hipLaunchKernelGGL(k_smudge_batch, dim3((sg + 63) / 64), dim3(64), 0, c->stream, sproofs, c->P.n, L, KW, up, sn, sg, 1u, 3u, 4u);
  HIP_TRY(c, hipGetLastError());
  return MFH_OK;
}
int batch_streams(mfh_ctx *c) {
  if (!c->side) {
    HIP_TRY(c, hipStreamCreateWithFlags(&c->side, hipStreamNonBlocking));
    HIP_TRY(c, hipEventCreateWithFlags(&c->ev_fork, hipEventDisableTiming));
    HIP_TRY(c, hipEventCreateWithFlags(&c->ev_join, hipEventDisableTiming));
  }
  if (!c->ev_chain) {
    HIP_TRY(c, hipStreamCreateWithFlags(&c->side2, hipStreamNonBlocking));
    HIP_TRY(c, hipEventCreateWithFlags(&c->ev_chain, hipEventDisableTiming));
    HIP_TRY(c, hipEventCreateWithFlags(&c->ev_chain_done, hipEventDisableTiming));
  }
  return MFH_OK;
}

constexpr uint32_t kPubDirect = 64;
constexpr int kPubNB = 16;
struct PubBatch {
  uint32_t lu;
  const uint8_t *d_ubits;
  uint32_t ub;
  const uint8_t *h_pub;
  size_t pub_stride;
  const uint32_t *h_zero;
  PubBatch at(uint32_t s0) const {
    PubBatch p = *this;
    p.d_ubits += (size_t)s0 * ub;
    if (h_pub) p.h_pub += (size_t)s0 * pub_stride;
    if (h_zero) p.h_zero += s0;
    return p;
  }
};

int batch_chain_launch(mfh_ctx *c, const mf::SspSrc &src, const uint32_t *d_ssp, uint32_t sg, const uint8_t *h_bits, size_t bits_stride,
                       const uint32_t *h_delta, uint32_t *W, uint32_t *H, uint32_t *V, hipEvent_t ev_witness = nullptr, const PubBatch *pub = nullptr) {
  const uint32_t d = c->P.d;
  int rc = MFH_OK;
  auto witness_pass = [&](const uint8_t *bits, size_t stride, const uint32_t *delta, uint32_t *out) -> int {
    if (d % 128 == 0) {
      const uint32_t per = c->witness_per ? c->witness_per : 256u;
      for (uint32_t b0 = 0; b0 < sg; b0 += per) {
        int r = mfh_witness_poly_mm(c, d_ssp, std::min(per, sg - b0), bits + (size_t)b0 * stride, stride, delta + b0, out + (size_t)b0 * d);
        if (r) return r;
      }
    } else {
      for (uint32_t b0 = 0; b0 < sg; b0 += 12) {
        int r = mfh_witness_poly_multi(c, d_ssp, std::min(12u, sg - b0), bits + (size_t)b0 * stride, stride, delta + b0, out + (size_t)b0 * d);
        if (r) return r;
      }
    }
    return MFH_OK;
  };
  rc = witness_pass(h_bits, bits_stride, h_delta, W);
  if (rc) return rc;
  const bool pub_pass = pub && pub->lu > kPubDirect;
  if (pub_pass) {
    rc = witness_pass(pub->h_pub, pub->pub_stride, pub->h_zero, H);
    if (rc) return rc;
  }
  if (ev_witness) HIP_TRY(c, hipEventRecord(ev_witness, c->stream));
  if (pub)
    hipLaunchKernelGGL(k_add_public<kPubNB>, dim3((d + 255) / 256, (sg + kPubNB - 1) / kPubNB), dim3(256), 0, c->stream, W, src, d, pub_pass ? 0u : pub->lu,
                       pub->d_ubits, pub->ub, sg, pub_pass ? H : nullptr, V);
  else
// ... 155 lines not shown
  return MFH_OK;
}

int batch_smudge(mfh_ctx *c, uint64_t *sproofs, uint32_t sg, const uint8_t *h_smudge_mag, size_t maglen, const uint8_t *h_smudge_sign) {
  std::vector<uint8_t> mags((size_t)sg * 5 * maglen), signs((size_t)sg * 5);
  for (int pass = 0; pass < 2; pass++) {
    std::fill(mags.begin(), mags.end(), 0);
    std::fill(signs.begin(), signs.end(), 0);
    for (uint32_t b = 0; b < sg; b++) {
      const uint8_t *pm = h_smudge_mag + (size_t)b * 5 * maglen, *ps = h_smudge_sign + (size_t)b * 5;
      if (pass == 0) {
        memcpy(&mags[(size_t)b * 5 * maglen], pm, 4 * maglen);
        memcpy(&signs[(size_t)b * 5], ps, 4);
      } else {
        memcpy(&mags[((size_t)b * 5 + 3) * maglen], pm + 4 * maglen, maglen);
        signs[(size_t)b * 5 + 3] = ps[4];
      }
    }
    int rc = mfh_ct_smudge(c, sproofs, (size_t)sg * 5, mags.data(), maglen, signs.data());
    if (rc) return rc;
  }
  return MFH_OK;
}

int batch_ct_t(mfh_ctx *c, const uint8_t *d_crs_c8, const BatchScratch &B) {
  const uint32_t d = c->P.d, ctb = c->P.logq / 8;
  HIP_TRY(c, hipMemsetD32Async((hipDeviceptr_t)B.ONE, 1, 1, c->stream));
  return mfh_eval_rows(c, (uint64_t)ctb * c->P.n * 2 * d, 1, d_crs_c8 + (size_t)2 * d * ctb, B.ONE, nullptr, B.CT_T, nullptr, 0);
}

struct ImageGuard {
  mfh_ctx *c;
  bool on;
  ~ImageGuard() { if (on) mfh_crs_set_resident_mm(c, nullptr); }
};
int batch_transient_image(mfh_ctx *c, const uint8_t *d_crs_c8, uint32_t nproofs, uint32_t rank, uint32_t world, ImageGuard &guard) {
  const uint32_t ctb = c->P.logq / 8;
  if (c->mm_image || !c->batch_image || nproofs <= BG || (((uint64_t)c->P.n * ctb) & 7)) return MFH_OK;
  const size_t ib = mfh_crs_mm_share_bytes(c, rank, world);
  if (c->batch_img.cap < ib) {
    (void)batch_img_drop(c);
    size_t mem_free = 0, mem_total = 0;
    if (hipMemGetInfo(&mem_free, &mem_total) != hipSuccess) mem_free = 0;
    if (ib > mem_free / 4 * 3 || !dev_alloc(c->batch_img, ib)) (void)hipGetLastError();
  }
  if (!c->batch_img.p) return MFH_OK;
  int rc = mfh_crs_expand_mm_share(c, d_crs_c8, rank, world, c->batch_img.as<uint8_t>());
  if (rc) return rc;
  mfh_crs_set_resident_mm_share(c, c->batch_img.as<uint8_t>(), rank, world);
  guard.on = true;
  return MFH_OK;
}

int prove_batch_impl(mfh_ctx *c, const uint8_t *d_crs_c8, const uint32_t *d_ssp, uint32_t nproofs, const uint8_t *h_witness_bits,
                     size_t bits_stride, const uint32_t *h_delta, const uint8_t *h_smudge_mag, size_t maglen, const uint8_t *h_smudge_sign,
                     uint64_t *d_proofs, const PubBatch *pub) {
  if (!c) return MFH_EINVAL;
  if (!nproofs) return MFH_OK;
  if (!d_crs_c8 || !h_witness_bits || !h_delta || !h_smudge_mag || !h_smudge_sign || !d_proofs) return MFH_EINVAL;
  if (c->resident_rows) { c->err = "mfh_prove_batch regenerates the keystream: clear the resident CRS image first"; return MFH_EUNSUPPORTED; }
  if (c->mm_image && c->mm_world != 1) { c->err = "mfh_prove_batch: the registered matrix-core image holds one rank's row shares (use mfh_prove_batch_partial)"; return MFH_EINVAL; }
  mf::SspSrc src;
  {
    int rc0 = ssp_src(c, d_ssp, src, true);
    if (rc0) return rc0;
    if (pub && (rc0 = ssp_rows_lu_check(c, d_ssp, pub->lu))) return rc0;
  }
  const uint32_t d = c->P.d, m = c->P.m, n = c->P.n;
  if (bits_stride < (m + 6) / 8) { c->err = "bits_stride shorter than the m - 1 witness bits"; return MFH_EINVAL; }
  for (uint32_t b = 0; b < nproofs; b++)
    if (h_delta[b] >= P32) { c->err = "delta must be < p"; return MFH_EINVAL; }
  if (maglen + 4 > (size_t)(c->P.logq / 64) * 8) { c->err = "smudge magnitude too wide"; return MFH_EINVAL; }
  const size_t ctl = (size_t)(n + 1) * ((c->P.logq + 63) / 64);
  HIP_TRY(c, hipSetDevice(c->device));
  const bool will_stream = c->mm_image || (c->batch_image && nproofs > BG && (((uint64_t)n * (c->P.logq / 8)) & 7) == 0);
  const uint32_t SG = will_stream ? BSG : BSG_REGEN;
  const uint32_t nsg = (nproofs + SG - 1) / SG;
  uint32_t nsl = 1;
  const uint32_t ctb0 = c->P.logq / 8;
  const bool slabs_ok = !c->mm_image && c->batch_image && nproofs > BG && (((uint64_t)n * ctb0) & 7) == 0;
  if (slabs_ok && c->batch_slabs) nsl = std::min(c->batch_slabs, std::max(1u, std::min(d, m)));
  else if (slabs_ok) {
    size_t mem_free = 0, mem_total = 0;
    if (hipMemGetInfo(&mem_free, &mem_total) == hipSuccess) {
      const size_t ib = mfh_crs_mm_image_bytes(c), avail = mem_free + c->batch_img.cap + c->d_batch.cap;
      if (ib > avail / 4 * 3) {
        const size_t budget = std::max<size_t>(avail / 3, (size_t)1 << 30);
        nsl = (uint32_t)std::min<size_t>(256, (ib + budget - 1) / budget);
        const size_t area = (size_t)3 * BSG * d * 4, maxsg = std::max<size_t>(1, avail / 4 / area);
        if (nsg > maxsg) {
          const size_t ctl0 = (size_t)(n + 1) * ((c->P.logq + 63) / 64);
          for (uint32_t s0 = 0; s0 < nproofs; s0 += (uint32_t)maxsg * SG) {
            const uint32_t cnt = std::min<uint32_t>((uint32_t)maxsg * SG, nproofs - s0);
            const PubBatch sub = pub ? pub->at(s0) : PubBatch{};
            int r = prove_batch_impl(c, d_crs_c8, d_ssp, cnt, h_witness_bits + (size_t)s0 * bits_stride, bits_stride, h_delta + s0,
                                     h_smudge_mag + (size_t)s0 * 5 * maglen, maglen, h_smudge_sign + (size_t)s0 * 5, d_proofs + (size_t)s0 * 5 * ctl0,
                                     pub ? &sub : nullptr);
            if (r) return r;
          }
          c->last_batch_sg = 0;
          return MFH_OK;
        }
      }
    }
  }
  const uint32_t nbuf = nsl > 1 ? nsg : 2;
  while (c->ev_sgdone.size() < nsg) {
    hipEvent_t e;
    HIP_TRY(c, hipEventCreateWithFlags(&e, hipEventDisableTiming));
    c->ev_sgdone.push_back(e);
  }
  c->last_batch_sg = 0;
  BatchScratch B;
  int rc = batch_scratch(c, nproofs, nbuf, B, nsl > 1 ? 1 : nsg, nsl > 1 ? 0 : nproofs);
  if (rc) return rc;
  size_t slot = 0;
  HIP_TRY(c, hipMemsetAsync(B.SCZ, 0, B.nslots * 2048, c->stream));
  rc = batch_streams(c);
  if (rc) return rc;
  while (c->ev_cdone.size() < nbuf) {
    hipEvent_t e0, e1, e2;
    HIP_TRY(c, hipEventCreateWithFlags(&e0, hipEventDisableTiming));
    HIP_TRY(c, hipEventCreateWithFlags(&e1, hipEventDisableTiming));
    HIP_TRY(c, hipEventCreateWithFlags(&e2, hipEventDisableTiming));
    c->ev_cdone.push_back(e0);
    c->ev_rdone.push_back(e1);
    c->ev_wdone.push_back(e2);
  }
  hipStream_t const main_stream = c->stream, chain_stream = c->side2;
  auto whv_of = [&](uint32_t sgi, uint32_t *&W, uint32_t *&H, uint32_t *&V) {
    W = B.WHV + (size_t)(sgi % nbuf) * 3 * BSG * d;
    H = W + (size_t)BSG * d;
    V = H + (size_t)BSG * d;
  };
  auto launch_chain = [&](uint32_t sgi) -> int {
    const uint32_t s0 = sgi * SG, sg = std::min(SG, nproofs - s0);
    uint32_t *WALL, *HALL, *VALL;
    whv_of(sgi, WALL, HALL, VALL);
    OnStream chain(c, chain_stream);
    const PubBatch psg = pub ? pub->at(s0) : PubBatch{};
    int r = batch_chain_launch(c, src, d_ssp, sg, h_witness_bits + (size_t)s0 * bits_stride, bits_stride, h_delta + s0, WALL, HALL, VALL, c->ev_wdone[sgi % nbuf],
                               pub ? &psg : nullptr);
    if (r) return r;
    HIP_TRY(c, hipEventRecord(c->ev_cdone[sgi % nbuf], chain_stream));
    return MFH_OK;
  };
  HIP_TRY(c, hipEventRecord(c->ev_chain, main_stream));
  HIP_TRY(c, hipStreamWaitEvent(chain_stream, c->ev_chain, 0));
  rc = launch_chain(0);
  if (rc) return rc;
  if (nsl > 1) {
    for (uint32_t k = 1; k < nsg; k++) {
      rc = launch_chain(k);
      if (rc) return rc;
    }
    for (;;) {
      size_t ib = 0;
      for (uint32_t r = 0; r < nsl; r++) ib = std::max(ib, mfh_crs_mm_share_bytes(c, r, nsl));
      if (c->batch_img.cap >= ib) break;
      (void)batch_img_drop(c);
      size_t mem_free = 0, mem_total = 0;
      const bool fits = hipMemGetInfo(&mem_free, &mem_total) != hipSuccess || ib + ((size_t)8 << 30) <= mem_free;
      if (fits && dev_alloc(c->batch_img, ib)) break;
      (void)hipGetLastError();
      const uint32_t cap = std::min<uint32_t>(256u, std::max(1u, std::min(d, m)));
      if (nsl >= cap || c->batch_slabs) { c->err = "mfh_prove_batch: no room for a row slab of the CRS image"; return MFH_ENOMEM; }
      nsl = std::min(cap, nsl * 2);
    }
    rc = batch_ct_t(c, d_crs_c8, B);
    if (rc) return rc;
    ImageGuard slab{c, true};
    for (uint32_t r = 0; r < nsl; r++) {
      rc = mfh_crs_expand_mm_share(c, d_crs_c8, r, nsl, c->batch_img.as<uint8_t>());
      if (rc) return rc;
      mfh_crs_set_resident_mm_share(c, c->batch_img.as<uint8_t>(), r, nsl);
      HIP_TRY(c, hipMemsetAsync(B.SCZ, 0, B.nslots * 2048, c->stream));
      slot = 0;
      const uint32_t loS = (uint32_t)((uint64_t)d * r / nsl);
      for (uint32_t s0 = 0, sgi = 0; s0 < nproofs; s0 += SG, sgi++) {
        const uint32_t sg = std::min(SG, nproofs - s0);
        uint32_t *WALL, *HALL, *VALL;
        whv_of(sgi, WALL, HALL, VALL);
        const BatchCoef co = {WALL + loS, HALL + loS, VALL + loS, d};
        rc = batch_rows_supergroup(c, d_crs_c8, r, nsl, sg, h_witness_bits + (size_t)s0 * bits_stride, bits_stride, co, d_proofs + (size_t)s0 * 5 * ctl, B, slot,
                                   r == 0 ? h_delta + s0 : nullptr, r == 0 ? c->ev_cdone[sgi % nbuf] : nullptr, r > 0);
        if (rc) return rc;
      }
    }
    for (uint32_t s0 = 0; s0 < nproofs; s0 += SG) {
      rc = batch_smudge(c, d_proofs + (size_t)s0 * 5 * ctl, std::min(SG, nproofs - s0), h_smudge_mag + (size_t)s0 * 5 * maglen, maglen, h_smudge_sign + (size_t)s0 * 5);
      if (rc) return rc;
      HIP_TRY(c, hipEventRecord(c->ev_sgdone[s0 / SG], c->stream));
    }
    c->last_batch_sg = SG;
    c->last_batch_n = nproofs;
    return MFH_OK;
  }
  ImageGuard transient{c, false};
  rc = batch_transient_image(c, d_crs_c8, nproofs, 0, 1, transient);
  if (rc) return rc;
  rc = batch_stage_host(c, B, nproofs, h_witness_bits, bits_stride, h_delta, h_smudge_mag, maglen, h_smudge_sign, SG);
  if (rc) return rc;
  rc = batch_ct_t(c, d_crs_c8, B);
  if (rc) return rc;
  bool bw_done = false;
  if (c->batch_bw_merged && nsg > 1 && mm_image_covers(c, (uint64_t)ctb0 * n * 2 * d, m)) {
    const uint64_t ctr_ct = (uint64_t)ctb0 * n, pstride = 5 * ctl;
    const uint32_t bstride = (m + 6) / 8;
    const MmRegion reg = {ctr_ct * 2 * d, d_crs_c8 + (size_t)2 * d * ctb0};
    for (uint32_t g0 = 0; g0 < nsg; g0 += 8) {
      MmIo ios[8];
      uint32_t nvs[8];
      const uint32_t ng = std::min(8u, nsg - g0);
      for (uint32_t k = 0; k < ng; k++) {
        const uint32_t sgi = g0 + k, s0 = sgi * SG, sg = std::min(SG, nproofs - s0);
        const uint8_t *d_cw = B.CW + (size_t)sgi * B.cw_stride;
        ios[k] = MmIo{{nullptr, nullptr}, sg, {d_proofs + (size_t)s0 * 5 * ctl + 4 * ctl, nullptr}, sg, pstride, d_cw, bstride, B.SCZ + 256 * slot++};
        ios[k].add_ct = B.CT_T;
        ios[k].add_scale = (const uint32_t *)(d_cw + B.cw_delta_off);
        nvs[k] = sg;
      }
      rc = ng > 1 ? eval_rows_multi_io_regions(c, &reg, 1, m, ios, nvs, ng, 1, 0) : eval_rows_multi_io(c, reg.off, m, reg.c8, ios[0], nvs[0], 1, 0);
      if (rc) return rc;
    }
    bw_done = true;
  }
  const bool early = c->batch_early_chain && bw_done;
  bool any_on_side = false;
  for (uint32_t s0 = 0, sgi = 0; s0 < nproofs; s0 += SG, sgi++) {
    const uint32_t sg = std::min(SG, nproofs - s0);
    uint64_t *sproofs = d_proofs + (size_t)s0 * 5 * ctl;
    uint32_t *WALL, *HALL, *VALL;
    whv_of(sgi, WALL, HALL, VALL);
    const BatchCoef co = {WALL, HALL, VALL, d};
    if (early && sgi + 1 < nsg) {
      if (sgi >= 1) HIP_TRY(c, hipStreamWaitEvent(chain_stream, c->ev_rdone[(sgi - 1) % nbuf], 0));
      rc = launch_chain(sgi + 1);
      if (rc) return rc;
    }
    if (early && sgi >= 2) HIP_TRY(c, hipStreamWaitEvent(main_stream, c->ev_sgdone[sgi - 2], 0));
    HIP_TRY(c, hipStreamWaitEvent(main_stream, c->ev_wdone[sgi % nbuf], 0));
    bool on_side = false;
    rc = batch_rows_supergroup(c, d_crs_c8, 0, 1, sg, h_witness_bits + (size_t)s0 * bits_stride, bits_stride, co, sproofs, B, slot, h_delta + s0,
                               c->ev_cdone[sgi % nbuf], 0, B.CW + (size_t)sgi * B.cw_stride, bw_done, sgi, early ? &on_side : nullptr);
    if (rc) return rc;
    if (early) HIP_TRY(c, hipEventRecord(c->ev_rdone[sgi % nbuf], main_stream));
    else if (sgi + 1 < nsg) {
      HIP_TRY(c, hipEventRecord(c->ev_rdone[sgi % nbuf], main_stream));
      HIP_TRY(c, hipStreamWaitEvent(chain_stream, c->ev_rdone[sgi % nbuf], 0));
      rc = launch_chain(sgi + 1);
      if (rc) return rc;
    }
    {
      OnStream tail(c, on_side ? c->side : main_stream);
      rc = batch_smudge_staged(c, B, sproofs, s0, sg);
      if (rc) return rc;
      HIP_TRY(c, hipEventRecord(c->ev_sgdone[sgi], c->stream));
    }
    any_on_side = any_on_side || on_side;
  }
  if (any_on_side) {
    HIP_TRY(c, hipEventRecord(c->ev_join, c->side));
    HIP_TRY(c, hipStreamWaitEvent(main_stream, c->ev_join, 0));
  }
  c->last_batch_sg = SG;
  c->last_batch_n = nproofs;
  return MFH_OK;
}

}

extern "C" {

int mfh_prove_batch(mfh_ctx *c, const uint8_t *d_crs_c8, const uint32_t *d_ssp, uint32_t nproofs, const uint8_t *h_witness_bits,
                    size_t bits_stride, const uint32_t *h_delta, const uint8_t *h_smudge_mag, size_t maglen, const uint8_t *h_smudge_sign,
                    uint64_t *d_proofs) {
  return prove_batch_impl(c, d_crs_c8, d_ssp, nproofs, h_witness_bits, bits_stride, h_delta, h_smudge_mag, maglen, h_smudge_sign, d_proofs, nullptr);
}

int mfh_prove_batch_public(mfh_ctx *c, const uint8_t *d_crs_c8, const uint32_t *d_ssp, uint32_t lu, uint32_t nproofs, const uint8_t *h_bits,
                           size_t bits_stride, const uint32_t *h_delta, const uint8_t *h_smudge_mag, size_t maglen, const uint8_t *h_smudge_sign,
                           uint64_t *d_proofs) {
  if (!c) return MFH_EINVAL;
  if (lu >= c->P.m) { c->err = "lu must be < m (the m - 1 wires of the SSP)"; return MFH_EINVAL; }
  if (!lu) return mfh_prove_batch(c, d_crs_c8, d_ssp, nproofs, h_bits, bits_stride, h_delta, h_smudge_mag, maglen, h_smudge_sign, d_proofs);
  if (!nproofs) return MFH_OK;
  if (!h_bits) return MFH_EINVAL;
  const uint32_t m = c->P.m, bstride = (m + 6) / 8, ub = (lu + 7) / 8;
  if (bits_stride < bstride) { c->err = "bits_stride shorter than the m - 1 witness bits"; return MFH_EINVAL; }
  std::vector<uint8_t> priv((size_t)nproofs * bstride), pubb;
  std::vector<uint32_t> zero;
  for (uint32_t b = 0; b < nproofs; b++) {
    uint8_t *x = priv.data() + (size_t)b * bstride;
    memcpy(x, h_bits + (size_t)b * bits_stride, bstride);
// ... 181 lines not shown
```

### c-lwe-snarks_amd/csrc/ssp_interp.hip

```cpp
#include <algorithm>
#include <vector>

#include "ctx.hpp"
#include "p32.hpp"

namespace {

constexpr int IG = 32;
constexpr uint32_t IWG = 256;
constexpr uint32_t CH_MIN = 256;
constexpr uint32_t MAX_CUT = 512;

__global__ __launch_bounds__(256) void k_seed_local(const uint32_t *__restrict__ tpad, uint32_t n, uint32_t NB, uint32_t *__restrict__ seeds) {
  const uint64_t idx = (uint64_t)blockIdx.x * blockDim.x + threadIdx.x;
  if (idx >= (uint64_t)n * NB) return;
  const uint32_t j = (uint32_t)(idx / NB), b = (uint32_t)(idx % NB);
  const uint64_t r = j + 2;
  uint32_t q = 0;
#pragma unroll
  for (int s = IG - 1; s >= 0; s--) q = red_p32(r * q + tpad[(size_t)b * IG + s]);
  seeds[idx] = q;
}
__global__ __launch_bounds__(256) void k_seed_scan(uint32_t n, uint32_t NB, uint32_t *__restrict__ seeds) {
  const uint32_t j = blockIdx.x * blockDim.x + threadIdx.x;
// ... 115 lines not shown
  for (uint32_t e = h_row_ptr[0]; e < h_row_ptr[nrows]; e++)
    if (h_coef[e]) cnt[h_wire[e]]++;
  HIP_TRY(c, hipSetDevice(c->device));
  const uint32_t *tpad, *w;
  if (int rc = ssp_rows_tree(c, "mfh_ssp_from_rows", tpad, w)) return rc;
  if (int rc = interp_prepare(c, tpad)) return rc;
  SspInterp *s = c->interp;
  cnt[0] += n - nrows;

  std::vector<uint64_t> off(m + 1, 0);
  for (uint32_t i = 0; i < m; i++) off[i + 1] = off[i] + cnt[i];
  const uint64_t nnz = off[m];
  const uint64_t ch = std::max<uint64_t>(CH_MIN, (nnz + MAX_CUT - 1) / MAX_CUT);
  std::vector<uint32_t> parts_h, splits_h;
  std::vector<std::pair<uint32_t, uint32_t>> whole;
  uint32_t ncut = 0;
  for (uint32_t i = 0; i < m; i++) {
    if (cnt[i] <= ch) { whole.emplace_back(cnt[i], i); continue; }
    const uint32_t np = (uint32_t)((cnt[i] + ch - 1) / ch);
    splits_h.insert(splits_h.end(), {i + 1, ncut, np, 0});
    for (uint32_t q = 0; q < np; q++) {
      const uint64_t a = off[i] + q * ch, b = std::min<uint64_t>(off[i] + (q + 1) * ch, off[i + 1]);
      parts_h.insert(parts_h.end(), {(uint32_t)a, (uint32_t)(b - a), ncut + q, 1});
    }
    ncut += np;
  }
  std::stable_sort(whole.begin(), whole.end(), [](const std::pair<uint32_t, uint32_t> &x, const std::pair<uint32_t, uint32_t> &y) { return x.first > y.first; });
  for (auto &wc : whole) parts_h.insert(parts_h.end(), {(uint32_t)off[wc.second], wc.first, wc.second + 1, 0});
  const uint32_t nparts = (uint32_t)(parts_h.size() / 4), nsplit = (uint32_t)(splits_h.size() / 4);

  const size_t nz_words = 2 * (size_t)nnz, bytes = (nz_words + parts_h.size() + splits_h.size()) * 4;
  std::vector<uint32_t> host(nz_words + parts_h.size() + splits_h.size());
  {
    std::vector<uint64_t> pos(off.begin(), off.end() - 1);
    for (uint32_t j = 0; j < nrows; j++)
      for (uint32_t e = h_row_ptr[j]; e < h_row_ptr[j + 1]; e++) {
        if (!h_coef[e]) continue;
        const uint64_t q = pos[h_wire[e]]++;
        host[2 * q] = j;
        host[2 * q + 1] = mulp(h_coef[e], w[j]);
      }
    for (uint32_t j = nrows; j < n; j++) {
      const uint64_t q = pos[0]++;
      host[2 * q] = j;
      host[2 * q + 1] = w[j];
    }
  }
  std::copy(parts_h.begin(), parts_h.end(), host.begin() + nz_words);
  std::copy(splits_h.begin(), splits_h.end(), host.begin() + nz_words + parts_h.size());
  if (int rc = work_reserve(c, s->buf, std::max<size_t>(bytes, 16))) return rc;
  if (ncut)
    if (int rc = work_reserve(c, s->scratch, (size_t)ncut * d * 4)) return rc;

  c->ssp_frag_src = nullptr;
  HIP_TRY(c, hipMemcpyAsync(s->buf.p, host.data(), bytes, hipMemcpyHostToDevice, c->stream));
  const uint2 *d_nz = s->buf.as<const uint2>();
  const uint4 *d_parts = (const uint4 *)(s->buf.as<uint32_t>() + nz_words), *d_splits = d_parts + nparts;
  HIP_TRY(c, hipMemcpyAsync(d_ssp, tpad, (size_t)d * 4, hipMemcpyDeviceToDevice, c->stream));
  HIP_TRY(c, hipMemsetAsync(d_ssp + (size_t)(m + 1) * d, 0, (size_t)2 * d * 4, c->stream));
  {
    Timer tm(c, 15, nnz);
    const uint32_t wg_per_part = (s->NB + IWG - 1) / IWG;
    const int vec4 = d % 4 == 0 && ((uintptr_t)d_ssp & 15) == 0;
    hipLaunchKernelGGL(k_interp, dim3(nparts * wg_per_part), dim3(IWG), 0, c->stream, d_nz, d_parts, wg_per_part, (const uint32_t *)s->seeds, s->NB, tpad, d,
                       vec4, d_ssp, s->scratch.as<uint32_t>());
    if (nsplit) hipLaunchKernelGGL(k_interp_sum, dim3((d + 255) / 256, nsplit), dim3(256), 0, c->stream, d_splits, s->scratch.as<const uint32_t>(), d, d_ssp);
  }
  if (hipGetLastError() != hipSuccess || hipStreamSynchronize(c->stream) != hipSuccess) { c->err = "mfh_ssp_from_rows: launch failed"; return MFH_EDEVICE; }
  return MFH_OK;
}
```

### c-lwe-snarks_amd/csrc/ssp_rows.hip

```cpp
#include <algorithm>
#include <vector>

#include "ctx.hpp"
#include "ntt.hpp"

using namespace mf_ntt;

namespace {

constexpr uint32_t kLeafMax = 64;
constexpr size_t kChunkBytes = (size_t)128 << 20;
constexpr size_t kViolStageBytes = (size_t)64 << 20;

__global__ __launch_bounds__(64) void k_rows_tree_bottom(uint32_t n, uint32_t G, uint32_t nodes, uint32_t *__restrict__ tb) {
  __shared__ uint32_t sm[kLeafMax + 1][64];
  const uint32_t node = blockIdx.x * 64 + threadIdx.x;
  if (node >= nodes) return;
  uint32_t *cf = &sm[0][threadIdx.x];
  cf[0] = 1;
  for (uint32_t l = 0; l < G; l++) {
    const uint32_t j = node * G + l, nr = j < n ? P32 - (j + 2) : 0u;
    cf[64 * (l + 1)] = cf[64 * l];
    for (uint32_t k = l; k > 0; k--) cf[64 * k] = red_p32((uint64_t)nr * cf[64 * k] + cf[64 * (k - 1)]);
    cf[0] = mulp(nr, cf[0]);
// ... 320 lines not shown
  std::vector<uint32_t> msg(m);
  msg[0] = mulp(ts, beta);
  for (uint32_t r = 1; r < m; r++) msg[r] = mulp((uint32_t)(acc[r] % P32), beta);
  HIP_TRY(c, hipMemcpyAsync(d_msg_evals, msg.data(), (size_t)m * 4, hipMemcpyHostToDevice, c->stream));
  HIP_TRY(c, hipStreamSynchronize(c->stream));
  return MFH_OK;
}

extern "C" {

int mfh_ssp_set_rows(mfh_ctx *c, uint32_t nrows, const uint32_t *h_row_ptr, const uint32_t *h_wire, const uint32_t *h_coef, uint32_t lu_max) {
  if (!c) return MFH_EINVAL;
  if (!h_row_ptr) {
    if (nrows) return MFH_EINVAL;
    HIP_TRY(c, hipSetDevice(c->device));
    ssp_rows_free(c, true);
    return MFH_OK;
  }
  if (int rc = ssp_rows_check(c, "mfh_ssp_set_rows", nrows, h_row_ptr, h_wire, h_coef)) return rc;
  const uint32_t d = c->P.d, e0 = h_row_ptr[0], e1 = h_row_ptr[nrows];
  if (lu_max >= c->P.m) { c->err = "mfh_ssp_set_rows: lu_max must be < m"; return MFH_EINVAL; }
  HIP_TRY(c, hipSetDevice(c->device));
  if (int rc = rows_tree_build(c, "mfh_ssp_set_rows")) return rc;
  SspRows *R = new SspRows();
  struct Guard { SspRows *p; ~Guard() { delete p; } } guard{R};
  R->nrows = nrows;
  R->lu_max = lu_max;
  R->h_ptr.resize(nrows + 1);
  for (uint32_t j = 0; j <= nrows; j++) R->h_ptr[j] = h_row_ptr[j] - e0;
  R->h_wire.assign(h_wire + e0, h_wire + e1);
  R->h_coef.assign(h_coef + e0, h_coef + e1);
  const size_t nnz = e1 - e0, rows_w = nrows + 1 + 2 * nnz;
  if (hipMalloc(&R->d_rows, rows_w * 4) != hipSuccess || hipMalloc(&R->d_prefix, (size_t)(lu_max + 2) * d * 4) != hipSuccess) {
    (void)hipGetLastError();
    c->err = "mfh_ssp_set_rows: no memory for the rows";
    return MFH_ENOMEM;
  }
  HIP_TRY(c, hipMemcpyAsync(R->d_rows, R->h_ptr.data(), (size_t)(nrows + 1) * 4, hipMemcpyHostToDevice, c->stream));
  if (nnz) {
    HIP_TRY(c, hipMemcpyAsync(R->d_rows + nrows + 1, R->h_wire.data(), nnz * 4, hipMemcpyHostToDevice, c->stream));
    HIP_TRY(c, hipMemcpyAsync(R->d_rows + nrows + 1 + nnz, R->h_coef.data(), nnz * 4, hipMemcpyHostToDevice, c->stream));
  }
  HIP_TRY(c, hipMemcpyAsync(R->d_prefix, c->rows_tree->d_t, (size_t)d * 4, hipMemcpyDeviceToDevice, c->stream));
  if (int rc = rows_interp(c, R, lu_max + 1, nullptr, 0, 0, nullptr, R->d_prefix + d, d)) return rc;
  if (hipGetLastError() != hipSuccess || hipStreamSynchronize(c->stream) != hipSuccess) { c->err = "mfh_ssp_set_rows: interpolation failed"; return MFH_EDEVICE; }
  if (c->side) hipStreamSynchronize(c->side);
  delete c->rows;
  c->rows = R;
  guard.p = nullptr;
  c->rows_prefix = R->d_prefix;
  c->rows_lu_max = lu_max;
  c->prg_on = false;
  c->prg_t = nullptr;
  c->ssp_frag_src = nullptr;
  return MFH_OK;
}

int mfh_ssp_rows_fill(mfh_ctx *c, size_t first_slot, size_t nslots, uint32_t *d_out) {
  if (!c || (nslots && !d_out)) return MFH_EINVAL;
  if (!c->rows) { c->err = "mfh_ssp_rows_fill: no row SSP registered (mfh_ssp_set_rows)"; return MFH_EINVAL; }
  const uint32_t d = c->P.d, m = c->P.m;
  if (first_slot + nslots > (size_t)m + 3) { c->err = "mfh_ssp_rows_fill: slots beyond m + 2"; return MFH_EINVAL; }
  HIP_TRY(c, hipSetDevice(c->device));
  for (size_t k = 0; k < nslots;) {
    const size_t slot = first_slot + k;
    uint32_t *o = d_out + k * d;
    if (slot == 0) {
      HIP_TRY(c, hipMemcpyAsync(o, c->rows_tree->d_t, (size_t)d * 4, hipMemcpyDeviceToDevice, c->stream));
      k++;
    } else if (slot > m) {
      HIP_TRY(c, hipMemsetAsync(o, 0, (size_t)d * 4, c->stream));
      k++;
    } else {
      const uint32_t cnt = (uint32_t)std::min<size_t>(nslots - k, (size_t)m + 1 - slot);
      if (int rc = rows_interp(c, c->rows, cnt, nullptr, 0, (uint32_t)slot - 1, nullptr, o, d)) return rc;
      k += cnt;
    }
  }
  HIP_TRY(c, hipGetLastError());
  return MFH_OK;
}

int mfh_ssp_rows_violations(mfh_ctx *c, uint32_t nstmt, const uint8_t *h_bits, size_t bits_stride, uint32_t *h_count, uint32_t *h_first) {
  if (!c) return MFH_EINVAL;
  const SspRows *R = c->rows;
  if (!R) { c->err = "mfh_ssp_rows_violations: no row SSP registered (mfh_ssp_set_rows)"; return MFH_EINVAL; }
  const uint32_t bs = (c->P.m + 6) / 8;
  if (bits_stride < bs) { c->err = "mfh_ssp_rows_violations: bits_stride shorter than the m - 1 witness bits"; return MFH_EINVAL; }
  if (nstmt && (!h_bits || !h_count)) { c->err = "mfh_ssp_rows_violations: statements without h_bits / h_count"; return MFH_EINVAL; }
  if (!nstmt) return MFH_OK;
  HIP_TRY(c, hipSetDevice(c->device));
  const uint32_t ch = (uint32_t)std::min<size_t>({(size_t)nstmt, std::max<size_t>(1, kViolStageBytes / bs), (size_t)65535});
  const size_t bb = ((size_t)ch * bs + 255) & ~(size_t)255;
  if (int rc = wws_reserve(c, bb + (size_t)ch * 8)) return rc;
  const uint8_t *d_bits = c->wws.as<const uint8_t>();
  uint32_t *d_count = reinterpret_cast<uint32_t *>(c->wws.as<uint8_t>() + bb), *d_first = d_count + ch;
  for (uint32_t s0 = 0; s0 < nstmt; s0 += ch) {
    const uint32_t k = std::min(ch, nstmt - s0);
    uint8_t *st = (uint8_t *)pin_acquire(c, c->pin_rows, (size_t)k * bs);
    if (!st) return MFH_ENOMEM;
    for (uint32_t b = 0; b < k; b++) memcpy(st + (size_t)b * bs, h_bits + (size_t)(s0 + b) * bits_stride, bs);
    HIP_TRY(c, hipMemcpyAsync(c->wws.p, st, (size_t)k * bs, hipMemcpyHostToDevice, c->stream));
    pin_release(c, c->pin_rows);
    HIP_TRY(c, hipMemsetAsync(d_count, 0, (size_t)k * 4, c->stream));
    HIP_TRY(c, hipMemsetAsync(d_first, 0xFF, (size_t)k * 4, c->stream));
    if (R->nrows) {
      Timer tm(c, 24, (uint64_t)R->nrows * k);
// ... 12 lines not shown
```

### c-lwe-snarks_amd/csrc/witness.hip

```cpp
#include <algorithm>
#include <type_traits>

#include "ctx.hpp"

namespace {

typedef int v4i __attribute__((ext_vector_type(4)));
typedef int v16i __attribute__((ext_vector_type(16)));

__device__ __forceinline__ uint64_t partial_sum(const uint64_t *__restrict__ partial, uint32_t G, uint32_t d, uint32_t k, uint64_t s) {
  for (uint32_t g = 0; g < G; g++) s = (s + partial[(uint64_t)g * d + k] % MFH_P) % MFH_P;
  return s;
}
__device__ __forceinline__ uint32_t byte_plane(uint32_t x0, uint32_t x1, uint32_t x2, uint32_t x3, int w) {
  return __builtin_amdgcn_perm(x1, x0, 0x0c0c0400u + 0x00000101u * w)
         | __builtin_amdgcn_perm(x3, x2, 0x04000c0cu + 0x01010000u * w);
}
__device__ __forceinline__ constexpr uint32_t acc_row(uint32_t e, uint32_t h) { return (e & 3) + 8 * (e >> 2) + 4 * h; }

__global__ __launch_bounds__(256) void k_witness_partial(const uint32_t *__restrict__ ssp, const uint32_t *__restrict__ rows, uint32_t nsel,
                                                         uint32_t d, uint64_t *__restrict__ partial) {
  const uint32_t k4 = blockIdx.x * blockDim.x + threadIdx.x;
  if (k4 * 4 >= d) return;
  const uint32_t G = gridDim.y, g = blockIdx.y;
// ... 67 lines not shown
  for (uint32_t i = g; i < nsel; i += G) {
    const uint2 e = list[i];
    const uint32_t rk = mf::ssp_prg_rowkey(seed, e.x);
    const uint32_t v0 = mf::ssp_prg_raw(rk, k), v1 = mf::ssp_prg_raw(rk, k + 1), v2 = mf::ssp_prg_raw(rk, k + 2), v3 = mf::ssp_prg_raw(rk, k + 3);
#pragma unroll
    for (int b = 0; b < NB; b++)
      if ((e.y >> b) & 1) { acc[b][0] += v0; acc[b][1] += v1; acc[b][2] += v2; acc[b][3] += v3; }
  }
#pragma unroll
  for (int b = 0; b < NB; b++) {
    uint64_t *o = partial + ((uint64_t)b * G + g) * d + k;
    o[0] = acc[b][0]; o[1] = acc[b][1]; o[2] = acc[b][2]; o[3] = acc[b][3];
  }
}
__global__ void k_ssp_prg_fill(uint64_t seed, uint32_t first_slot, uint32_t d, uint64_t total, uint32_t *__restrict__ out) {
  for (uint64_t i = (uint64_t)blockIdx.x * blockDim.x + threadIdx.x; i < total; i += (uint64_t)gridDim.x * blockDim.x) {
    const uint32_t slot = first_slot + (uint32_t)(i / d), k = (uint32_t)(i % d);
    out[i] = mf::ssp_prg_coeff(mf::ssp_prg_rowkey(seed, slot), k);
  }
}
__global__ void k_ssp_prg_make_t(uint64_t seed, const uint64_t *__restrict__ partial, uint32_t G, uint32_t d, uint32_t *__restrict__ t) {
  uint32_t k = blockIdx.x * blockDim.x + threadIdx.x;
  if (k >= d) return;
  uint64_t s = partial_sum(partial, G, d, k, mf::ssp_prg_coeff(mf::ssp_prg_rowkey(seed, 1), k));
  if (k == 0) s = (s + MFH_P - 1) % MFH_P;
  t[k] = (uint32_t)s;
}
__global__ void k_witness_finish(const uint32_t *__restrict__ ssp, const uint64_t *__restrict__ partial, uint32_t G, uint32_t d, uint32_t delta,
                                 uint32_t *__restrict__ w) {
  uint32_t k = blockIdx.x * blockDim.x + threadIdx.x;
  if (k >= d) return;
  w[k] = (uint32_t)partial_sum(partial, G, d, k, ((uint64_t)ssp[k] * delta) % MFH_P);
}
__global__ void k_witness_lanes(const uint64_t *__restrict__ partial, uint32_t G, uint32_t d, uint64_t *__restrict__ lanes) {
  uint32_t k = blockIdx.x * blockDim.x + threadIdx.x;
  if (k >= d) return;
  lanes[k] = partial_sum(partial, G, d, k, 0);
}

__global__ void k_ssp_frag(const uint32_t *__restrict__ ssp, uint32_t nrowsel, uint32_t d, uint32_t *__restrict__ frag) {
  const uint64_t gid = (uint64_t)blockIdx.x * blockDim.x + threadIdx.x;
  const uint32_t KT = d / 32;
  const uint32_t lane = gid & 63, eg = (gid >> 6) & 3;
  const uint64_t tile = gid >> 8;
  const uint32_t kt = (uint32_t)(tile % KT), K = (uint32_t)(tile / KT);
  const uint32_t KSt = (nrowsel + 31) / 32;
  if (K >= KSt) return;
  const uint32_t k = kt * 32 + (lane & 31), rb = K * 32 + 16 * (lane >> 5) + 4 * eg;
  uint32_t x[4];
#pragma unroll
  for (int e = 0; e < 4; e++) x[e] = rb + e < nrowsel ? ssp[(uint64_t)(rb + e + 2) * d + k] ^ 0x80808080u : 0u;
#pragma unroll
  for (int w = 0; w < 4; w++) frag[(((((uint64_t)kt * KSt + K) * 4 + w) * 64 + lane) << 2) + eg] = byte_plane(x[0], x[1], x[2], x[3], w);
}
struct WCols {
  uint32_t kt0;
  uint32_t KS;
  uint64_t wstride;
};
template <int MT>
__global__ __launch_bounds__(256) void k_witness_mm(const v4i *__restrict__ sspfrag, const v4i *__restrict__ bitfrag, uint32_t nrowsel ,
                                                    uint32_t ksteps_per_chunk, uint32_t d, int *__restrict__ part, WCols wc) {
  const uint32_t lane = threadIdx.x & 63, wave = threadIdx.x >> 6;
  const uint32_t r32 = lane & 31, h = lane >> 5;
  const uint32_t ktl = blockIdx.x * 4 + wave, kt = wc.kt0 + ktl;
  const uint32_t k = ktl * 32 + r32;
  const uint32_t K0 = blockIdx.y * ksteps_per_chunk, K1 = min((nrowsel + 31) / 32, K0 + ksteps_per_chunk);
  v16i acc[MT][4];
#pragma unroll
  for (int t = 0; t < MT; t++)
#pragma unroll
    for (int w = 0; w < 4; w++)
#pragma unroll
      for (int e = 0; e < 16; e++) acc[t][w][e] = 0;
  if (K0 >= K1) return;
  constexpr int PF = 3;
  v4i bq[PF][4], aq[PF][MT];
  auto fetch = [&](int slot, uint32_t K) {
    K = min(K, K1 - 1);
    const v4i *src = sspfrag + (((uint64_t)kt * wc.KS + K) * 4) * 64 + lane;
#pragma unroll
    for (int w = 0; w < 4; w++) bq[slot][w] = src[64 * w];
#pragma unroll
    for (int t = 0; t < MT; t++) aq[slot][t] = bitfrag[((uint64_t)K * MT + t) * 64 + lane];
  };
#pragma unroll
  for (int i = 0; i < PF; i++) fetch(i, K0 + i);
  for (uint32_t K = K0; K < K1; K += PF) {
#pragma unroll
    for (int i = 0; i < PF; i++) {
      if (K + i < K1) {
#pragma unroll
        for (int t = 0; t < MT; t++)
#pragma unroll
          for (int w = 0; w < 4; w++) acc[t][w] = __builtin_amdgcn_mfma_i32_32x32x32_i8(aq[i][t], bq[i][w], acc[t][w], 0, 0, 0);
        fetch(i, K + i + PF);
      }
    }
  }
#pragma unroll
  for (int t = 0; t < MT; t++)
#pragma unroll
    for (int w = 0; w < 4; w++)
#pragma unroll
      for (int e = 0; e < 16; e++) {
        const uint32_t stmt = 32 * t + acc_row(e, h);
// ... 345 lines not shown
  size_t bytes(int i) const { return off[i + 1] - off[i]; }
  int reserve(mfh_ctx *c) const { return wws_reserve(c, off[N]); }
  template <class T> T *at(const mfh_ctx *c, int i) const { return reinterpret_cast<T *>(c->wws.as<uint8_t>() + off[i]); }
};

template <class F> int witness_partials(mfh_ctx *c, const mf::SspSrc &src, const uint8_t *h_bits, uint32_t rank, uint32_t world, F &&finish) {
  const uint32_t d = c->P.d, m = c->P.m;
  if (d % 4) { c->err = "d must be a multiple of 4"; return MFH_EINVAL; }
  uint32_t *rows = (uint32_t *)pin_acquire(c, c->pin_rows, (size_t)m * 4 + 4);
  if (!rows) return MFH_ENOMEM;
  uint32_t nall = 0;
  for (uint32_t i = 1; i < m; i++)
    if (witness_bit(h_bits, i)) rows[nall++] = i + 1;
  const uint32_t lo = (uint32_t)((uint64_t)nall * rank / world), hi = (uint32_t)((uint64_t)nall * (rank + 1) / world);
  const uint32_t nsel = hi - lo, G = std::max(1u, std::min(64u, nsel / 8 + 1));
  const WwsCarve<2> ws({up256((size_t)m * 4), (size_t)G * d * 8});
  if (int rc = ws.reserve(c)) return rc;
  uint32_t *d_rows = ws.at<uint32_t>(c, 0);
  uint64_t *partial = ws.at<uint64_t>(c, 1);
  if (nsel) HIP_TRY(c, hipMemcpyAsync(d_rows, rows + lo, (size_t)nsel * 4, hipMemcpyHostToDevice, c->stream));
  pin_release(c, c->pin_rows);
  if (src.dense)
    hipLaunchKernelGGL(k_witness_partial, dim3((d / 4 + 255) / 256, G), dim3(256), 0, c->stream, src.dense, d_rows, nsel, d, partial);
  else
    hipLaunchKernelGGL(k_witness_partial_prg, dim3((d / 4 + 255) / 256, G), dim3(256), 0, c->stream, src.seed, d_rows, nsel, d, partial);
  HIP_TRY(c, hipGetLastError());
  finish(partial, G);
  HIP_TRY(c, hipGetLastError());
  return MFH_OK;
}

struct MmPlan {
  uint32_t MT;
  uint32_t nrowsel, ksteps;
  bool fused;
  uint32_t nchunks, kpc, ychunks;
  size_t packed, cd_off;
  enum { HEAD, BITFRAG, PART, ROWKEYS };
  WwsCarve<4> ws;
  MmPlan(const mfh_ctx *c, bool dense, uint32_t nstmt, size_t bits_stride, uint32_t nc)
      : MT(nstmt > 128 ? 8 : nstmt > 64 ? 4 : nstmt > 32 ? 2 : 1), nrowsel(c->P.m - 1), ksteps((nrowsel + 31) / 32),
        fused(MT == 8 && dense && c->P.m < 65536 && (nc >= 16384 || ksteps <= 64)), nchunks(fused ? 1u : std::min(ksteps, 4u)),
        kpc((ksteps + nchunks - 1) / nchunks), ychunks((ksteps + kpc - 1) / kpc), packed((size_t)nstmt * bits_stride), cd_off(packed + (8 - packed % 8) % 8),
        ws({up256(packed + 8 + 256 * 8), (size_t)ksteps * MT * 1024, (size_t)nchunks * 4 * 32 * MT * nc * 4, dense ? 0 : up256((size_t)ksteps * 32 * 4)}) {}
};
template <class F> void with_mt(uint32_t MT, F &&f) {
  if (MT == 1) f(std::integral_constant<int, 1>{});
  else if (MT == 2) f(std::integral_constant<int, 2>{});
  else f(std::integral_constant<int, 4>{});
}

}

extern "C" {

int mfh_ssp_set_prg(mfh_ctx *c, uint64_t seed, const uint32_t *d_t) {
  if (!c) return MFH_EINVAL;
  if (d_t) ssp_rows_free(c, false);
  c->prg_on = d_t != nullptr;
  c->prg_seed = seed;
  c->prg_t = d_t;
  return MFH_OK;
}

int mfh_ssp_prg_fill(mfh_ctx *c, uint64_t seed, size_t first_slot, size_t nslots, uint32_t *d_out) {
  if (!c || !d_out) return MFH_EINVAL;
  HIP_TRY(c, hipSetDevice(c->device));
  const uint64_t total = (uint64_t)nslots * c->P.d;
  if (!total) return MFH_OK;
  hipLaunchKernelGGL(k_ssp_prg_fill, dim3((uint32_t)std::min<uint64_t>((total + 255) / 256, 4096)), dim3(256), 0, c->stream, seed, (uint32_t)first_slot,
                     c->P.d, total, d_out);
  HIP_TRY(c, hipGetLastError());
  return MFH_OK;
}

int mfh_ssp_prg_make_t(mfh_ctx *c, uint64_t seed, const uint8_t *h_bits, uint32_t *d_t) {
  if (!c || !h_bits || !d_t) return MFH_EINVAL;
  HIP_TRY(c, hipSetDevice(c->device));
  return witness_partials(c, mf::SspSrc{nullptr, d_t, seed}, h_bits, 0, 1, [&](const uint64_t *partial, uint32_t G) {
    hipLaunchKernelGGL(k_ssp_prg_make_t, dim3((c->P.d + 255) / 256), dim3(256), 0, c->stream, seed, partial, G, c->P.d, d_t);
  });
}

int mfh_witness_poly(mfh_ctx *c, const uint32_t *d_ssp, const uint8_t *h_bits, uint32_t delta, uint32_t *d_w) {
  if (!witness_args_ok(c, 1, 1, h_bits, &delta, d_w)) return MFH_EINVAL;
  if (int rc = witness_deltas(c, 1, &delta)) return rc;
  HIP_TRY(c, hipSetDevice(c->device));
  if (ssp_is_rows(c, d_ssp)) return ssp_rows_witness(c, 1, h_bits, (c->P.m + 6) / 8, &delta, d_w, c->P.d);
  mf::SspSrc src;
  if (int rc = ssp_src(c, d_ssp, src)) return rc;
  return witness_partials(c, src, h_bits, 0, 1, [&](const uint64_t *partial, uint32_t G) {
    hipLaunchKernelGGL(k_witness_finish, dim3((c->P.d + 255) / 256), dim3(256), 0, c->stream, src.t, partial, G, c->P.d, delta, d_w);
  });
}

int mfh_witness_poly_multi(mfh_ctx *c, const uint32_t *d_ssp, uint32_t nstmt, const uint8_t *h_bits, size_t bits_stride, const uint32_t *h_delta, uint32_t *d_w) {
  constexpr int NB = 12;
  if (!witness_args_ok(c, nstmt, NB, h_bits, h_delta, d_w)) return MFH_EINVAL;
  if (ssp_is_rows(c, d_ssp)) return ssp_rows_witness(c, nstmt, h_bits, bits_stride, h_delta, d_w, c->P.d);
  mf::SspSrc src;
  if (int rc = ssp_src(c, d_ssp, src)) return rc;
  const uint32_t d = c->P.d, m = c->P.m;
  if (d % 4) { c->err = "d must be a multiple of 4"; return MFH_EINVAL; }
  if (int rc = witness_deltas(c, nstmt, h_delta)) return rc;
  HIP_TRY(c, hipSetDevice(c->device));
  uint2 *list = (uint2 *)pin_acquire(c, c->pin_rows, (size_t)m * 8 + 8);
  if (!list) return MFH_ENOMEM;
// ... 114 lines not shown
```

### include/mfhip.h

```cpp
#pragma once
#include <stddef.h>
#include <stdint.h>

#ifdef __cplusplus
extern "C" {
#endif

#define MFH_P 0xfffffffbu

enum {
  MFH_OK = 0,
  MFH_EINVAL = -1,
  MFH_EDEVICE = -2,
  MFH_ENOMEM = -3,
  MFH_EUNSUPPORTED = -4
};

typedef struct {
  uint32_t n;
  uint32_t logq;
  uint32_t d;
  uint32_t m;
} mfh_params;

// ... 149 lines not shown
int mfh_merkle_load_keys(mfh_ctx *ctx, mfh_merkle *t, uint8_t *d_table, size_t table_stride, uint32_t length, uint32_t key_bytes, uint32_t nk,
                         const uint8_t *d_keys, const uint8_t *d_payloads, uint32_t payload_bytes, uint32_t h_status[3]);
int mfh_merkle_check_table(mfh_ctx *ctx, const mfh_merkle *t, const uint8_t *d_table, size_t table_stride, uint32_t length, uint32_t key_bytes,
                           uint32_t h_out[4]);
int mfh_merkle_grow(mfh_ctx *ctx, const mfh_merkle *t, uint32_t new_depth, const uint8_t *d_table, size_t table_stride, uint32_t length,
                    uint8_t *d_new_table, size_t new_stride, mfh_merkle **out, uint8_t *h_roots);
int mfh_merkle_grow_leaves(mfh_ctx *ctx, const mfh_merkle *t, uint32_t new_depth, mfh_merkle **out, uint8_t *h_roots);

int mfh_poly_mul(mfh_ctx *ctx, const uint32_t *d_a, size_t la, const uint32_t *d_b, size_t lb, uint32_t *d_c);
int mfh_poly_add(mfh_ctx *ctx, const uint32_t *d_a, const uint32_t *d_b, size_t count, uint32_t *d_out);
int mfh_poly_prepare_t(mfh_ctx *ctx, const uint32_t *d_t);
int mfh_ssp_prepare(mfh_ctx *ctx, const uint32_t *d_ssp);
int mfh_poly_h(mfh_ctx *ctx, const uint32_t *d_v, uint32_t *d_h);
int mfh_poly_h_multi(mfh_ctx *ctx, const uint32_t *d_v, uint32_t *d_h, uint32_t nb);
int mfh_set_poly_exact(mfh_ctx *ctx, int mode);
long mfh_poly_exact_fallbacks(mfh_ctx *ctx);
int mfh_poly_exact_points(mfh_ctx *ctx, uint32_t *out);
int mfh_set_poly_exact_points(mfh_ctx *ctx, const uint32_t *pts);

int mfh_setup_messages(mfh_ctx *ctx, const uint32_t *d_ssp, uint32_t alpha, uint32_t beta, uint32_t s, uint32_t *d_msg);
int mfh_setup(mfh_ctx *ctx, const uint32_t *d_ssp, uint32_t alpha, uint32_t beta, uint32_t s, const uint64_t *d_sk,
              const uint64_t *d_err, uint8_t *d_crs_c8);
int mfh_setup_image(mfh_ctx *ctx, const uint32_t *d_ssp, uint32_t alpha, uint32_t beta, uint32_t s, const uint64_t *d_sk,
                    const uint64_t *d_err, uint8_t *d_crs_c8, void *d_rows_image);
int mfh_prove(mfh_ctx *ctx, const uint8_t *d_crs_c8, const uint32_t *d_ssp, const uint8_t *h_witness_bits, uint32_t delta,
              const uint8_t *h_smudge_mag, size_t maglen, const uint8_t *h_smudge_sign, uint64_t *d_proof);

int mfh_verify(mfh_ctx *ctx, const uint32_t *d_ssp, uint32_t alpha, uint32_t beta, uint32_t s, const uint64_t *d_sk,
               const uint64_t *d_proofs, size_t count, uint8_t *d_ok);

int mfh_setup_public(mfh_ctx *ctx, const uint32_t *d_ssp, uint32_t alpha, uint32_t beta, uint32_t s, uint32_t lu, const uint64_t *d_sk,
                     const uint64_t *d_err, uint8_t *d_crs_c8, void *d_rows_image);
int mfh_prove_public(mfh_ctx *ctx, const uint8_t *d_crs_c8, const uint32_t *d_ssp, uint32_t lu, const uint8_t *h_bits, uint32_t delta,
                     const uint8_t *h_smudge_mag, size_t maglen, const uint8_t *h_smudge_sign, uint64_t *d_proof);
int mfh_prove_batch_public(mfh_ctx *ctx, const uint8_t *d_crs_c8, const uint32_t *d_ssp, uint32_t lu, uint32_t nproofs, const uint8_t *h_bits,
                           size_t bits_stride, const uint32_t *h_delta, const uint8_t *h_smudge_mag, size_t maglen, const uint8_t *h_smudge_sign,
                           uint64_t *d_proofs);
int mfh_vk_derive(mfh_ctx *ctx, const uint32_t *d_ssp, uint32_t s, uint32_t lu, uint32_t *d_vk);
int mfh_verify_public(mfh_ctx *ctx, const uint32_t *d_vk, uint32_t lu, uint32_t alpha, uint32_t beta, const uint64_t *d_sk, const uint64_t *d_proofs,
                      const uint8_t *h_statements, size_t stmt_stride, size_t count, uint8_t *d_ok);

size_t mfh_crs_mm_image_bytes(const mfh_ctx *ctx);
int mfh_crs_expand_mm(mfh_ctx *ctx, const uint8_t *d_crs_c8, uint8_t *d_image);
int mfh_crs_set_resident_mm(mfh_ctx *ctx, const uint8_t *d_image);
int mfh_set_expand_path(mfh_ctx *ctx, int path);
int mfh_set_expand_periods(mfh_ctx *ctx, uint32_t periods);
int mfh_set_batch_image(mfh_ctx *ctx, int enabled);
int mfh_set_batch_slabs(mfh_ctx *ctx, uint32_t nslabs);
int mfh_set_encrypt_chunks(mfh_ctx *ctx, uint32_t chunks);
int mfh_set_eval_path(mfh_ctx *ctx, int path);
int mfh_set_witness_per(mfh_ctx *ctx, uint32_t statements);
int mfh_set_batch_launch(mfh_ctx *ctx, uint32_t groups_per_launch, int merge_regions);
int mfh_set_batch_bw(mfh_ctx *ctx, int merged);
int mfh_set_mm_stream(mfh_ctx *ctx, int map, int persistent, int sync_mode, uint32_t spin_max);
int mfh_set_mm_width(mfh_ctx *ctx, uint32_t per_xcd, int early_chain);
int mfh_set_mm_queue(mfh_ctx *ctx, int mode, uint32_t start_shift, int prefix);
int mfh_set_mm_claim_log(mfh_ctx *ctx, uint32_t *d_log, size_t words);
uint32_t mfh_mm_claim_log_launches(const mfh_ctx *ctx, uint32_t *desc, uint32_t max_launches);
int mfh_set_mm_chunk_rows(mfh_ctx *ctx, uint32_t rows);
int mfh_set_mm_pack(mfh_ctx *ctx, int on);
int mfh_prove_batch(mfh_ctx *ctx, const uint8_t *d_crs_c8, const uint32_t *d_ssp, uint32_t nproofs, const uint8_t *h_witness_bits,
                    size_t bits_stride, const uint32_t *h_delta, const uint8_t *h_smudge_mag, size_t maglen, const uint8_t *h_smudge_sign,
                    uint64_t *d_proofs);
uint32_t mfh_prove_batch_supergroup(const mfh_ctx *ctx);
int mfh_prove_batch_stream_wait(mfh_ctx *ctx, uint32_t upto, void *hip_stream);
size_t mfh_crs_mm_share_bytes(const mfh_ctx *ctx, uint32_t rank, uint32_t world);
int mfh_crs_expand_mm_share(mfh_ctx *ctx, const uint8_t *d_crs_c8, uint32_t rank, uint32_t world, uint8_t *d_image);
int mfh_crs_set_resident_mm_share(mfh_ctx *ctx, const uint8_t *d_image, uint32_t rank, uint32_t world);
int mfh_batch_chain(mfh_ctx *ctx, const uint32_t *d_ssp, uint32_t nstmt, const uint8_t *h_witness_bits, size_t bits_stride, const uint32_t *h_delta,
                    uint32_t *d_w, uint32_t *d_h, uint32_t *d_v);
int mfh_batch_witness_cols(mfh_ctx *ctx, const uint32_t *d_ssp, uint32_t nstmt, const uint8_t *h_witness_bits, size_t bits_stride, const uint32_t *h_delta,
                           uint32_t col0, uint32_t ncols, uint32_t *d_w, size_t w_stride);
int mfh_batch_chain_from_w(mfh_ctx *ctx, const uint32_t *d_ssp, uint32_t nstmt, const uint32_t *d_w, uint32_t *d_h, uint32_t *d_v);
int mfh_prove_batch_partial(mfh_ctx *ctx, const uint8_t *d_crs_c8, uint32_t rank, uint32_t world, uint32_t nstmt, const uint8_t *h_witness_bits,
                            size_t bits_stride, const uint32_t *d_w, const uint32_t *d_h, const uint32_t *d_v, size_t coef_stride, uint64_t *d_partial);
int mfh_prove_batch_finish(mfh_ctx *ctx, const uint8_t *d_crs_c8, uint32_t nstmt, const uint32_t *h_delta, const uint8_t *h_smudge_mag, size_t maglen,
                           const uint8_t *h_smudge_sign, uint64_t *d_proofs);

int mfh_prove_partial(mfh_ctx *ctx, const uint8_t *d_crs_c8, const uint32_t *d_ssp, const uint8_t *h_witness_bits, uint32_t delta,
                      uint32_t rank, uint32_t world, uint64_t *d_partial);
int mfh_prove_finish(mfh_ctx *ctx, uint64_t *d_proof, const uint8_t *h_smudge_mag, size_t maglen, const uint8_t *h_smudge_sign);
int mfh_witness_poly_multi(mfh_ctx *ctx, const uint32_t *d_ssp, uint32_t nstmt, const uint8_t *h_bits, size_t bits_stride, const uint32_t *h_delta,
                           uint32_t *d_w);
int mfh_witness_poly_mm(mfh_ctx *ctx, const uint32_t *d_ssp, uint32_t nstmt, const uint8_t *h_bits, size_t bits_stride, const uint32_t *h_delta,
                        uint32_t *d_w);
int mfh_witness_poly_mm_cols(mfh_ctx *ctx, const uint32_t *d_ssp, uint32_t nstmt, const uint8_t *h_bits, size_t bits_stride, const uint32_t *h_delta,
                             uint32_t col0, uint32_t ncols, uint32_t *d_w, size_t w_stride);
int mfh_witness_lanes(mfh_ctx *ctx, const uint32_t *d_ssp, const uint8_t *h_witness_bits, uint32_t rank, uint32_t world, uint64_t *d_lanes);
int mfh_witness_from_lanes(mfh_ctx *ctx, const uint32_t *d_ssp, const uint64_t *d_lanes, uint32_t delta, uint32_t *d_w);
int mfh_prove_partial_w(mfh_ctx *ctx, const uint8_t *d_crs_c8, const uint32_t *d_ssp, const uint8_t *h_witness_bits, uint32_t delta,
                        uint32_t rank, uint32_t world, const uint64_t *d_wlanes, uint64_t *d_partial);
uint32_t mfh_lanes_per_value(const mfh_ctx *ctx);
int mfh_ct_to_lanes(mfh_ctx *ctx, const uint64_t *d_cts, size_t count, uint64_t *d_lanes);
int mfh_ct_from_lanes(mfh_ctx *ctx, const uint64_t *d_lanes, size_t count, uint64_t *d_cts);

const char *mfh_version(void);
int mfh_digest128(mfh_ctx *ctx, const void *d_buf, size_t nbytes, uint64_t h_digest[2]);
size_t mfh_workspace_bytes(const mfh_ctx *ctx);
int mfh_eval_rows_multi(mfh_ctx *ctx, uint64_t off, size_t nrows, const uint8_t *d_c8, const uint32_t *d_coeffs, uint32_t nvec,
                        uint32_t coeff_bytes, uint64_t *d_rops, int accumulate);

int mfh_set_timing(mfh_ctx *ctx, int enabled);
int mfh_set_overlap(mfh_ctx *ctx, int mode);
int mfh_timing_drain(mfh_ctx *ctx, const char *which, uint64_t *count, double *total_ms, uint64_t *total_rows, float *last_ms);
float mfh_last_kernel_ms(mfh_ctx *ctx, const char *which);
double mfh_timing_busy_ms(const mfh_ctx *ctx);
uint64_t mfh_timing_work_rows(const mfh_ctx *ctx);

#ifdef __cplusplus
}
#endif
```

Baseline: 14250.

## Stream batch witness polynomial on matrix cores, sharing digits with the bw pass

```diff
diff --git a/c-lwe-snarks_amd/__init__.py b/c-lwe-snarks_amd/__init__.py
--- a/c-lwe-snarks_amd/__init__.py
+++ b/c-lwe-snarks_amd/__init__.py
@@ -80,7 +80,7 @@
     "mfh_encrypt_rows", "mfh_decrypt", "mfh_ct_smudge", "mfh_ssp_upload", "mfh_witness_poly", "mfh_version",
     "mfh_workspace_bytes", "mfh_last_kernel_ms", "mfh_set_timing", "mfh_set_overlap", "mfh_eval_rows_multi", "mfh_prove_batch", "mfh_crs_mm_image_bytes", "mfh_crs_expand_mm", "mfh_crs_set_resident_mm", "mfh_witness_poly_multi", "mfh_witness_poly_mm", "mfh_poly_h_multi", "mfh_poly_mul", "mfh_poly_add", "mfh_poly_prepare_t",
     "mfh_ssp_prepare", "mfh_poly_h", "mfh_setup_messages", "mfh_setup", "mfh_setup_image", "mfh_crs_image_set_b", "mfh_prove",
-    "mfh_prove_partial", "mfh_prove_finish", "mfh_ct_to_lanes", "mfh_ct_from_lanes", "mfh_lanes_per_value", "mfh_digest128", "mfh_timing_drain", "mfh_timing_busy_ms", "mfh_timing_work_rows", "mfh_set_batch_image", "mfh_set_batch_slabs", "mfh_set_expand_path", "mfh_set_expand_periods", "mfh_set_encrypt_path", "mfh_set_batch_launch", "mfh_set_batch_bw", "mfh_set_mm_chunk_rows", "mfh_set_mm_pack", "mfh_set_poly_exact", "mfh_poly_exact_fallbacks", "mfh_poly_exact_points", "mfh_set_poly_exact_points", "mfh_set_mm_stream", "mfh_add_dotp", "mfh_set_encrypt_chunks", "mfh_set_witness_per", "mfh_set_eval_path", "mfh_set_decrypt_path", "mfh_decrypt_rows",
+    "mfh_prove_partial", "mfh_prove_finish", "mfh_ct_to_lanes", "mfh_ct_from_lanes", "mfh_lanes_per_value", "mfh_digest128", "mfh_timing_drain", "mfh_timing_busy_ms", "mfh_timing_work_rows", "mfh_set_batch_image", "mfh_set_batch_slabs", "mfh_set_expand_path", "mfh_set_expand_periods", "mfh_set_encrypt_path", "mfh_set_batch_launch", "mfh_set_batch_bw", "mfh_set_batch_witness", "mfh_witness_poly_stream", "mfh_set_mm_chunk_rows", "mfh_set_mm_pack", "mfh_set_poly_exact", "mfh_poly_exact_fallbacks", "mfh_poly_exact_points", "mfh_set_poly_exact_points", "mfh_set_mm_stream", "mfh_add_dotp", "mfh_set_encrypt_chunks", "mfh_set_witness_per", "mfh_set_eval_path", "mfh_set_decrypt_path", "mfh_decrypt_rows",
     "mfh_crs_mm_share_bytes", "mfh_crs_expand_mm_share", "mfh_crs_set_resident_mm_share", "mfh_batch_chain", "mfh_batch_witness_cols", "mfh_batch_chain_from_w", "mfh_witness_poly_mm_cols", "mfh_prove_batch_partial", "mfh_prove_batch_finish",
     "mfh_resident_row_bytes", "mfh_crs_expand", "mfh_eval_rows_resident", "mfh_crs_set_resident",
     "mfh_witness_lanes", "mfh_witness_from_lanes", "mfh_prove_partial_w", "mfh_verify",
@@ -104,6 +104,8 @@
     "mfh_set_mm_claim_log": "test instrumentation of mfh_set_mm_queue",
     "mfh_mm_claim_log_launches": "test instrumentation of mfh_set_mm_queue",
     "mfh_set_expand_periods": "test knob; older builds pick the periods per chunk from the row count",
+    "mfh_set_batch_witness": "tuning knob; older builds run the witness pass per super-group",
+    "mfh_witness_poly_stream": "the streamed pass alone (tests); older builds have mfh_witness_poly_mm only",
 }
 
 
@@ -144,6 +146,7 @@
         "mfh_poly_h_multi": (i32, [vp, vp, vp, u32]),
         "mfh_witness_poly_mm": (i32, [vp, vp, u32, ctypes.c_char_p, sz, vp, vp]),
         "mfh_witness_poly_multi": (i32, [vp, vp, u32, ctypes.c_char_p, sz, vp, vp]),
+        "mfh_witness_poly_stream": (i32, [vp, vp, u32, ctypes.c_char_p, sz, vp, vp]),
         "mfh_crs_mm_image_bytes": (sz, [vp]),
         "mfh_crs_expand_mm": (i32, [vp, vp, vp]),
         "mfh_crs_set_resident_mm": (i32, [vp, vp]),
@@ -200,6 +203,7 @@
         "mfh_set_mm_stream": (i32, [vp, i32, i32, i32, u32]),
         "mfh_set_batch_launch": (i32, [vp, u32, i32]),
         "mfh_set_batch_bw": (i32, [vp, i32]),
+        "mfh_set_batch_witness": (i32, [vp, i32]),
         "mfh_set_encrypt_path": (i32, [vp, i32]),
         "mfh_set_expand_path": (i32, [vp, i32]),
         "mfh_set_expand_periods": (i32, [vp, u32]),
@@ -1090,6 +1094,9 @@
     def set_batch_bw(self, merged=True):
         self._chk(self.lib.mfh_set_batch_bw(self._h, 1 if merged else 0))
 
+    def set_batch_witness(self, streamed=True):
+        self._chk(self.lib.mfh_set_batch_witness(self._h, 1 if streamed else 0))
+
     def set_mm_stream(self, map=0, persistent=False, sync_mode=0, spin_max=64):
         self._chk(self.lib.mfh_set_mm_stream(self._h, int(map), int(persistent), int(sync_mode), int(spin_max)))
 
@@ -1392,7 +1399,7 @@
         bits = b"".join(bytes(w[:stride]).ljust(stride, b"\0") for w in witness_bits_list)
         dl = (ctypes.c_uint32 * nb)(*[int(x) for x in deltas])
         out = self.empty(nb * p.d * 4)
-        fn = self.lib.mfh_witness_poly_mm if mm else self.lib.mfh_witness_poly_multi
+        fn = self.lib.mfh_witness_poly_stream if mm == "stream" else self.lib.mfh_witness_poly_mm if mm else self.lib.mfh_witness_poly_multi
         self._chk(fn(self._h, _ptr(d_ssp), nb, bits, stride, ctypes.cast(dl, ctypes.c_void_p), _ptr(out)))
         return out
 
diff --git a/c-lwe-snarks_amd/csrc/ctx.hpp b/c-lwe-snarks_amd/csrc/ctx.hpp
--- a/c-lwe-snarks_amd/csrc/ctx.hpp
+++ b/c-lwe-snarks_amd/csrc/ctx.hpp
@@ -88,6 +88,11 @@
   size_t mm_base[3] = {0, 0, 0};
   DevBuf ssp_frag;
   const uint32_t *ssp_frag_src = nullptr;
+  DevBuf ssp_img;
+  const uint32_t *ssp_img_src = nullptr;
+  DevBuf wstream;
+  hipEvent_t ev_wstage = nullptr, ev_wdigits = nullptr;
+  int batch_witness = 1;
   SspInterp *interp = nullptr;
   DevBuf circ_io;
   DevBuf circ_state;
@@ -142,6 +147,8 @@
   uint32_t res_rank = 0, res_world = 1;
 };
 
+inline void ssp_images_stale(mfh_ctx *c) { c->ssp_frag_src = c->ssp_img_src = nullptr; }
+
 struct Timer {
   mfh_ctx *c;
   mfh_ctx::Timed t{};
@@ -303,6 +310,8 @@
 bool mm_image_covers(const mfh_ctx *c, uint64_t off, size_t nrows);
 struct MmsPlan {
   uint32_t ng, ngt, ND, nrows, nchunks, rpc, rpad, ntiles, mtiles;
+  uint32_t ssp = 0;
+  bool nolog = false;
   size_t cd_bytes, part_bytes;
   const uint8_t *img[2];
   int8_t *cd;
@@ -315,3 +324,8 @@
 int mms_digits(mfh_ctx *c, const MmsPlan &P, const MmIo *ios, const uint32_t *nvecs);
 int mms_stream(mfh_ctx *c, const MmsPlan &P);
 int mms_finish(mfh_ctx *c, const MmsPlan &P, const MmIo *ios, const uint32_t *nvecs, int accumulate);
+bool mms_ssp_ok(const mfh_ctx *c);
+bool mms_plan_ssp(mfh_ctx *c, const uint8_t *image, uint32_t ng, MmsPlan &P);
+int mms_witness_finish(mfh_ctx *c, const MmsPlan &P, const MmIo *ios, const uint32_t *nvecs, const uint32_t *d_t, const uint32_t *const *d_delta, uint32_t *const *W,
+                       const uint32_t *d_v0 = nullptr, uint32_t *const *V = nullptr);
+const uint8_t *ssp_image(mfh_ctx *c, const uint32_t *d_ssp);
diff --git a/c-lwe-snarks_amd/csrc/evalmm.hip b/c-lwe-snarks_amd/csrc/evalmm.hip
--- a/c-lwe-snarks_amd/csrc/evalmm.hip
+++ b/c-lwe-snarks_amd/csrc/evalmm.hip
@@ -1019,6 +1019,45 @@
   const uint32_t g = blockIdx.z, lender = A.io[g].sa_from1 ? A.io[g].sa_from1 - 1 : g;
   evalmm_finish_body<ND, KWM, PK>(part + g * part_stride, A.io[g].sc_zeroed, nchunks, ntiles, N, A.nvec[g], n, nrows, ct, MBv, sby, LL, A.io[g], accumulate,
                                   part + lender * part_stride, ND * A.nvec[lender]);
+}
+
+constexpr int WFK = 32;
+struct WfinArgs {
+  const int64_t *sc[16];
+  const uint32_t *delta[16];
+  uint32_t *w[16];
+  uint32_t *v[16];
+  uint32_t nvec[16];
+};
+__global__ __launch_bounds__(N2) void k_witness_stream_finish(const long long *__restrict__ part, uint64_t part_stride , uint32_t nchunks, uint32_t nrows,
+                                                              uint32_t d, const uint32_t *__restrict__ t, const uint32_t *__restrict__ v0, WfinArgs A) {
+  __shared__ uint32_t tile[N2][WFK + 1];
+  const uint32_t g = blockIdx.y, b = threadIdx.x, k0 = blockIdx.x * WFK, nvec = A.nvec[g];
+  const long long *pg = part + g * part_stride;
+  if (b < nvec) {
+    const uint64_t corr = (uint64_t)(128 * A.sc[g][b] + 16384ll * nrows) * 0x01010101ull;
+    const uint64_t delta = A.delta[g][b], P = MFH_P;
+#pragma unroll 4
+    for (int kk = 0; kk < WFK; kk++) {
+      long long U = 0, SA = 0;
+      for (uint32_t ch = 0; ch < nchunks; ch++) {
+        const long long *row = pg + ((uint64_t)ch * d + k0 + kk) * N2;
+        U += row[b];
+        SA += row[nvec];
+      }
+      const uint64_t S = (uint64_t)(U + 128 * SA) + corr;
+      tile[b][kk] = (uint32_t)((S % P + (uint64_t)t[k0 + kk] * delta % P) % P);
+    }
+  }
+  __syncthreads();
+  uint32_t *wg = A.w[g], *vg = A.v[g];
+  const uint32_t v0k = v0 ? v0[k0 + threadIdx.x % WFK] : 0u;
+  for (uint32_t i = threadIdx.x; i < nvec * WFK; i += N2) {
+    const uint32_t w = tile[i / WFK][i % WFK];
+    const uint64_t at = (uint64_t)(i / WFK) * d + k0 + i % WFK;
+    wg[at] = w;
+    if (v0) vg[at] = (uint32_t)(((uint64_t)w + v0k) % MFH_P);
+  }
 }
 
 }
@@ -1225,7 +1264,7 @@
 int mms_stream(mfh_ctx *c, const MmsPlan &P) {
   const uint32_t KS = (P.nrows + RT2 - 1) / RT2 * (RT2 / 64), tgs = (P.mtiles + TPW - 1) / TPW;
   const bool will_persist = mms_persistent(c, P);
-  Timer t(c, P.ngt > 1 ? (P.ND == 1 ? 14 : 10) : 8, P.nrows, (uint64_t)P.nrows * P.ngt, will_persist ? 1 : 0);
+  Timer t(c, P.ssp ? 48 : P.ngt > 1 ? (P.ND == 1 ? 14 : 10) : 8, P.nrows, (uint64_t)P.nrows * P.ngt, will_persist ? 1 : 0);
   MmsImages imgs{};
   for (uint32_t g = 0; g < P.ngt; g++) imgs.image[g] = (const v4i *)P.img[g / P.ng];
   const uint32_t pk = mms_pk(c, P);
@@ -1249,7 +1288,7 @@
       }
       if (sync_mode) HIP_TRY(c, hipMemsetAsync(c->mm_sync, 0, 8 * 32 * sizeof(uint32_t), c->stream));
       else if (q.mode) HIP_TRY(c, hipMemsetAsync(qctr, 0, 8 * sizeof(uint32_t), c->stream));
-      if (c->mm_log) {
+      if (c->mm_log && !P.nolog) {
         const size_t need = (size_t)2 * P.nchunks * 8 * nblk * 32;
         if (c->mm_log_n == 16 || c->mm_log_used + need > c->mm_log_words) { c->err = "mfh_set_mm_claim_log: the log is too small for the call's launches"; return MFH_EINVAL; }
         q.log = c->mm_log + c->mm_log_used;
@@ -1298,6 +1337,48 @@
   HIP_TRY(c, hipGetLastError());
   return MFH_OK;
 }
+bool mms_ssp_ok(const mfh_ctx *c) { return c->mm_pack && !c->mm_wave1; }
+bool mms_plan_ssp(mfh_ctx *c, const uint8_t *image, uint32_t ng, MmsPlan &P) {
+  if (!c || !image || !ng || ng > 16) return false;
+  const uint32_t d = c->P.d, m = c->P.m;
+  if (d % 64 || m < 2 || m > 0xffffffffu - 256 || !mms_ssp_ok(c)) return false;
+  P = MmsPlan{};
+  P.ssp = 1;
+  P.img[0] = image;
+  P.img[1] = nullptr;
+  P.ng = P.ngt = ng;
+  P.ND = 1;
+  P.nrows = m;
+  P.ntiles = 0;
+  P.mtiles = d / 4;
+  const uint32_t lim = std::max<uint32_t>(RT2, c->mm_chunk_rows / RT2 * RT2);
+  const uint32_t nchunks = (m + lim - 1) / lim;
+  P.rpc = ((m + nchunks - 1) / nchunks + RT2 - 1) / RT2 * RT2;
+  P.nchunks = (m + P.rpc - 1) / P.rpc;
+  P.rpad = P.nchunks * P.rpc;
+  P.cd_bytes = ((size_t)N2 * P.rpad + 255) & ~(size_t)255;
+  P.part_bytes = (size_t)P.nchunks * d * N2 * 8;
+  P.cd = nullptr;
+  P.part = nullptr;
+  return true;
+}
+int mms_witness_finish(mfh_ctx *c, const MmsPlan &P, const MmIo *ios, const uint32_t *nvecs, const uint32_t *d_t, const uint32_t *const *d_delta, uint32_t *const *W,
+                       const uint32_t *d_v0, uint32_t *const *V) {
+  if (!P.ssp || P.ngt > 16) return MFH_EINVAL;
+  WfinArgs A{};
+  for (uint32_t g = 0; g < P.ngt; g++) {
+    A.sc[g] = ios[g].sc_zeroed;
+    A.delta[g] = d_delta[g];
+    A.w[g] = W[g];
+    A.v[g] = d_v0 ? V[g] : nullptr;
+    A.nvec[g] = nvecs[g];
+  }
+  hipLaunchKernelGGL(k_witness_stream_finish, dim3(c->P.d / WFK, P.ngt), dim3(N2), 0, c->stream, (const long long *)P.part, (uint64_t)(P.part_bytes / 8), P.nchunks, P.nrows,
+                     c->P.d, d_t, d_v0, A);
+  HIP_TRY(c, hipGetLastError());
+  return MFH_OK;
+}
+
 int eval_rows_multi_io_regions(mfh_ctx *c, const MmRegion *regs, uint32_t nreg, size_t nrows, const MmIo *ios, const uint32_t *nvecs, uint32_t ng,
                                uint32_t coeff_bytes, int accumulate) {
   if (!c || !regs || !ios || !nvecs || !ng || !nreg || nreg * ng > 16) return MFH_EINVAL;
diff --git a/c-lwe-snarks_amd/csrc/mfhip.hip b/c-lwe-snarks_amd/csrc/mfhip.hip
--- a/c-lwe-snarks_amd/csrc/mfhip.hip
+++ b/c-lwe-snarks_amd/csrc/mfhip.hip
@@ -895,10 +895,12 @@
   if (c->ev_join) hipEventDestroy(c->ev_join);
   if (c->ev_chain) hipEventDestroy(c->ev_chain);
   if (c->ev_chain_done) hipEventDestroy(c->ev_chain_done);
+  if (c->ev_wstage) hipEventDestroy(c->ev_wstage);
+  if (c->ev_wdigits) hipEventDestroy(c->ev_wdigits);
   if (c->side) hipStreamDestroy(c->side);
   if (c->side2) hipStreamDestroy(c->side2);
   for (DevBuf *b : {&c->ws, &c->ws2, &c->ws3, &c->wws, &c->lazy, &c->aux, &c->d_msg, &c->d_prover, &c->d_pub, &c->d_batch, &c->batch_img, &c->circ_io,
-                    &c->circ_state, &c->ssp_frag, &c->sample_tmp})
+                    &c->circ_state, &c->ssp_frag, &c->ssp_img, &c->wstream, &c->sample_tmp})
     dev_free(*b);
   if (c->d_t0) hipFree(c->d_t0);
   for (auto &t : c->timed) { hipEventDestroy(t.e0); hipEventDestroy(t.e1); }
@@ -986,6 +988,12 @@
 int mfh_set_batch_bw(mfh_ctx *c, int merged) {
   if (!c) return MFH_EINVAL;
   c->batch_bw_merged = merged != 0;
+  return MFH_OK;
+}
+
+int mfh_set_batch_witness(mfh_ctx *c, int streamed) {
+  if (!c) return MFH_EINVAL;
+  c->batch_witness = streamed != 0;
   return MFH_OK;
 }
 
@@ -1018,6 +1026,7 @@
   if (!strcmp(which, "mmstream_rounds")) return 10;
   if (!strcmp(which, "mmstream_rounds_persistent")) return 110;
   if (!strcmp(which, "mmstream_bw_persistent")) return 114;
+  if (!strcmp(which, "mmstream_witness")) return 48;
   if (!strcmp(which, "ssp_interp")) return 15;
   if (!strcmp(which, "circuit_assign")) return 16;
   if (!strcmp(which, "circuit_assign_global")) return 17;
@@ -1060,6 +1069,7 @@
   if (kind < 0) return MFH_EINVAL;
   HIP_TRY(c, hipStreamSynchronize(c->stream));
   if (c->side) HIP_TRY(c, hipStreamSynchronize(c->side));
+  if (c->side2) HIP_TRY(c, hipStreamSynchronize(c->side2));
   uint64_t n = 0, rows = 0, work = 0;
   double tot = 0;
   float last = -1.f;
@@ -1607,7 +1617,7 @@
 }
 int mfh_ssp_upload(mfh_ctx *c, const void *h_ssp_u64, uint32_t *d_ssp, size_t first_slot, size_t nslots) {
   if (!c || !h_ssp_u64 || !d_ssp) return MFH_EINVAL;
-  c->ssp_frag_src = nullptr;
+  ssp_images_stale(c);
   HIP_TRY(c, hipSetDevice(c->device));
   const size_t d = c->P.d;
   const size_t total = nslots * d * 8;
diff --git a/c-lwe-snarks_amd/csrc/poly.hip b/c-lwe-snarks_amd/csrc/poly.hip
--- a/c-lwe-snarks_amd/csrc/poly.hip
+++ b/c-lwe-snarks_amd/csrc/poly.hip
@@ -936,7 +936,7 @@
 
 int mfh_poly_prepare_t(mfh_ctx *c, const uint32_t *d_t) {
   if (!c) return MFH_EINVAL;
-  c->ssp_frag_src = nullptr;
+  ssp_images_stale(c);
   if (c->poly) {
     c->poly->have_t = false;
     c->poly->cyc = false;
diff --git a/c-lwe-snarks_amd/csrc/snark.hip b/c-lwe-snarks_amd/csrc/snark.hip
--- a/c-lwe-snarks_amd/csrc/snark.hip
+++ b/c-lwe-snarks_amd/csrc/snark.hip
@@ -635,6 +635,10 @@
     HIP_TRY(c, hipStreamCreateWithFlags(&c->side2, hipStreamNonBlocking));
     HIP_TRY(c, hipEventCreateWithFlags(&c->ev_chain, hipEventDisableTiming));
     HIP_TRY(c, hipEventCreateWithFlags(&c->ev_chain_done, hipEventDisableTiming));
+  }
+  if (!c->ev_wstage) {
+    HIP_TRY(c, hipEventCreateWithFlags(&c->ev_wstage, hipEventDisableTiming));
+    HIP_TRY(c, hipEventCreateWithFlags(&c->ev_wdigits, hipEventDisableTiming));
   }
   return MFH_OK;
 }
@@ -896,6 +900,59 @@
   return MFH_OK;
 }
 
+int batch_witness_stream(mfh_ctx *c, const uint32_t *d_ssp, const MmRegion &reg, const MmIo *ios, const uint32_t *nvs, uint32_t ng, const uint32_t *const *d_delta,
+                         hipStream_t chain_stream, uint32_t *&Wall, uint32_t *&Vall, bool &taken) {
+  taken = false;
+  const uint32_t d = c->P.d, m = c->P.m;
+  hipStream_t const main_stream = c->stream;
+  MmsPlan BP, WP;
+  if (ng > 8 || !mms_plan(c, &reg, 1, m, ios, nvs, ng, 1, BP)) return MFH_OK;
+  const uint8_t *img;
+  {
+    OnStream chain(c, chain_stream);
+    img = ssp_image(c, d_ssp);
+  }
+  if (!img || !mms_plan_ssp(c, img, ng, WP) || WP.cd_bytes != BP.cd_bytes || WP.rpc != BP.rpc || WP.nchunks != BP.nchunks) return MFH_OK;
+  const size_t bw_b = (mms_ws_bytes(BP) + 255) & ~(size_t)255, wp_b = (size_t)ng * WP.part_bytes, w_b = (size_t)ng * BSG * d * 4;
+  if (c->wstream.cap < bw_b + wp_b + 2 * w_b) {
+    if (c->wstream.p) {
+      (void)hipDeviceSynchronize();
+      dev_free(c->wstream);
+    }
+    if (!dev_alloc(c->wstream, (bw_b + wp_b + 2 * w_b + ((size_t)1 << 20) - 1) & ~(((size_t)1 << 20) - 1))) {
+      (void)hipGetLastError();
+      return MFH_OK;
+    }
+  }
+  uint8_t *base = c->wstream.as<uint8_t>();
+  mms_bind(BP, base);
+  WP.cd = BP.cd;
+  WP.part = (int *)(base + bw_b);
+  WP.nolog = true;
+  Wall = (uint32_t *)(base + bw_b + wp_b);
+  Vall = (uint32_t *)(base + bw_b + wp_b + w_b);
+  int rc;
+  {
+    OnSide chain(c, chain_stream);
+    HIP_TRY(c, hipStreamWaitEvent(chain_stream, c->ev_wstage, 0));
+    rc = mms_digits(c, BP, ios, nvs);
+    if (rc) return rc;
+    HIP_TRY(c, hipEventRecord(c->ev_wdigits, chain_stream));
+    rc = mms_stream(c, WP);
+    if (rc) return rc;
+    uint32_t *W[8], *V[8];
+    for (uint32_t g = 0; g < ng; g++) W[g] = Wall + (size_t)g * BSG * d, V[g] = Vall + (size_t)g * BSG * d;
+    rc = mms_witness_finish(c, WP, ios, nvs, d_ssp, d_delta, W, d_ssp + d , V);
+    if (rc) return rc;
+  }
+  HIP_TRY(c, hipStreamWaitEvent(main_stream, c->ev_wdigits, 0));
+  rc = mms_stream(c, BP);
+  if (!rc) rc = mms_finish(c, BP, ios, nvs, 0);
+  if (rc) return rc;
+  taken = true;
+  return MFH_OK;
+}
+
 int prove_batch_impl(mfh_ctx *c, const uint8_t *d_crs_c8, const uint32_t *d_ssp, uint32_t nproofs, const uint8_t *h_witness_bits,
                      size_t bits_stride, const uint32_t *h_delta, const uint8_t *h_smudge_mag, size_t maglen, const uint8_t *h_smudge_sign,
                      uint64_t *d_proofs, const PubBatch *pub) {
@@ -972,10 +1029,13 @@
     c->ev_wdone.push_back(e2);
   }
   hipStream_t const main_stream = c->stream, chain_stream = c->side2;
+  bool wroute = false;
+  uint32_t *WSTREAM = nullptr, *VSTREAM = nullptr;
   auto whv_of = [&](uint32_t sgi, uint32_t *&W, uint32_t *&H, uint32_t *&V) {
     W = B.WHV + (size_t)(sgi % nbuf) * 3 * BSG * d;
     H = W + (size_t)BSG * d;
     V = H + (size_t)BSG * d;
+    if (wroute) W = WSTREAM + (size_t)sgi * BSG * d, V = VSTREAM + (size_t)sgi * BSG * d;
   };
   auto launch_chain = [&](uint32_t sgi) -> int {
     const uint32_t s0 = sgi * SG, sg = std::min(SG, nproofs - s0);
@@ -983,16 +1043,24 @@
     whv_of(sgi, WALL, HALL, VALL);
     OnStream chain(c, chain_stream);
     const PubBatch psg = pub ? pub->at(s0) : PubBatch{};
-    int r = batch_chain_launch(c, src, d_ssp, sg, h_witness_bits + (size_t)s0 * bits_stride, bits_stride, h_delta + s0, WALL, HALL, VALL, c->ev_wdone[sgi % nbuf],
-                               pub ? &psg : nullptr);
+    int r;
+    if (wroute)
+      r = mfh_poly_h_multi(c, VALL, HALL, sg);
+    else
+      r = batch_chain_launch(c, src, d_ssp, sg, h_witness_bits + (size_t)s0 * bits_stride, bits_stride, h_delta + s0, WALL, HALL, VALL, c->ev_wdone[sgi % nbuf],
+                             pub ? &psg : nullptr);
     if (r) return r;
     HIP_TRY(c, hipEventRecord(c->ev_cdone[sgi % nbuf], chain_stream));
     return MFH_OK;
   };
   HIP_TRY(c, hipEventRecord(c->ev_chain, main_stream));
   HIP_TRY(c, hipStreamWaitEvent(chain_stream, c->ev_chain, 0));
-  rc = launch_chain(0);
-  if (rc) return rc;
+  const bool try_ws = c->batch_witness && nsl == 1 && will_stream && !pub && d_ssp && src.dense && d % 64 == 0 && m >= 2 && nsg >= 2 && nsg <= 8 && c->batch_bw_merged &&
+                      mms_ssp_ok(c);
+  if (!try_ws) {
+    rc = launch_chain(0);
+    if (rc) return rc;
+  }
   if (nsl > 1) {
     for (uint32_t k = 1; k < nsg; k++) {
       rc = launch_chain(k);
@@ -1041,9 +1109,14 @@
     return MFH_OK;
   }
   ImageGuard transient{c, false};
+  if (try_ws) {
+    rc = batch_stage_host(c, B, nproofs, h_witness_bits, bits_stride, h_delta, h_smudge_mag, maglen, h_smudge_sign, SG);
+    if (rc) return rc;
+    HIP_TRY(c, hipEventRecord(c->ev_wstage, main_stream));
+  }
   rc = batch_transient_image(c, d_crs_c8, nproofs, 0, 1, transient);
   if (rc) return rc;
-  rc = batch_stage_host(c, B, nproofs, h_witness_bits, bits_stride, h_delta, h_smudge_mag, maglen, h_smudge_sign, SG);
+  if (!try_ws) rc = batch_stage_host(c, B, nproofs, h_witness_bits, bits_stride, h_delta, h_smudge_mag, maglen, h_smudge_sign, SG);
   if (rc) return rc;
   rc = batch_ct_t(c, d_crs_c8, B);
   if (rc) return rc;
@@ -1064,10 +1137,21 @@
         ios[k].add_scale = (const uint32_t *)(d_cw + B.cw_delta_off);
         nvs[k] = sg;
       }
+      if (try_ws) {
+        const uint32_t *dl[8];
+        for (uint32_t k = 0; k < ng; k++) dl[k] = ios[k].add_scale;
+        rc = batch_witness_stream(c, d_ssp, reg, ios, nvs, ng, dl, chain_stream, WSTREAM, VSTREAM, wroute);
+        if (rc) return rc;
+        if (wroute) continue;
+      }
       rc = ng > 1 ? eval_rows_multi_io_regions(c, &reg, 1, m, ios, nvs, ng, 1, 0) : eval_rows_multi_io(c, reg.off, m, reg.c8, ios[0], nvs[0], 1, 0);
       if (rc) return rc;
     }
     bw_done = true;
+  }
+  if (try_ws) {
+    rc = launch_chain(0);
+    if (rc) return rc;
   }
   const bool early = c->batch_early_chain && bw_done;
   bool any_on_side = false;
@@ -1083,7 +1167,7 @@
       if (rc) return rc;
     }
     if (early && sgi >= 2) HIP_TRY(c, hipStreamWaitEvent(main_stream, c->ev_sgdone[sgi - 2], 0));
-    HIP_TRY(c, hipStreamWaitEvent(main_stream, c->ev_wdone[sgi % nbuf], 0));
+    if (!wroute) HIP_TRY(c, hipStreamWaitEvent(main_stream, c->ev_wdone[sgi % nbuf], 0));
     bool on_side = false;
     rc = batch_rows_supergroup(c, d_crs_c8, 0, 1, sg, h_witness_bits + (size_t)s0 * bits_stride, bits_stride, co, sproofs, B, slot, h_delta + s0,
                                c->ev_cdone[sgi % nbuf], 0, B.CW + (size_t)sgi * B.cw_stride, bw_done, sgi, early ? &on_side : nullptr);
diff --git a/c-lwe-snarks_amd/csrc/ssp_interp.hip b/c-lwe-snarks_amd/csrc/ssp_interp.hip
--- a/c-lwe-snarks_amd/csrc/ssp_interp.hip
+++ b/c-lwe-snarks_amd/csrc/ssp_interp.hip
@@ -191,7 +191,7 @@
   if (ncut)
     if (int rc = work_reserve(c, s->scratch, (size_t)ncut * d * 4)) return rc;
 
-  c->ssp_frag_src = nullptr;
+  ssp_images_stale(c);
   HIP_TRY(c, hipMemcpyAsync(s->buf.p, host.data(), bytes, hipMemcpyHostToDevice, c->stream));
   const uint2 *d_nz = s->buf.as<const uint2>();
   const uint4 *d_parts = (const uint4 *)(s->buf.as<uint32_t>() + nz_words), *d_splits = d_parts + nparts;
diff --git a/c-lwe-snarks_amd/csrc/ssp_rows.hip b/c-lwe-snarks_amd/csrc/ssp_rows.hip
--- a/c-lwe-snarks_amd/csrc/ssp_rows.hip
+++ b/c-lwe-snarks_amd/csrc/ssp_rows.hip
@@ -396,7 +396,7 @@
   c->rows_lu_max = lu_max;
   c->prg_on = false;
   c->prg_t = nullptr;
-  c->ssp_frag_src = nullptr;
+  ssp_images_stale(c);
   return MFH_OK;
 }
 
diff --git a/c-lwe-snarks_amd/csrc/witness.hip b/c-lwe-snarks_amd/csrc/witness.hip
--- a/c-lwe-snarks_amd/csrc/witness.hip
+++ b/c-lwe-snarks_amd/csrc/witness.hip
@@ -143,6 +143,20 @@
   for (int e = 0; e < 4; e++) x[e] = rb + e < nrowsel ? ssp[(uint64_t)(rb + e + 2) * d + k] ^ 0x80808080u : 0u;
 #pragma unroll
   for (int w = 0; w < 4; w++) frag[(((((uint64_t)kt * KSt + K) * 4 + w) * 64 + lane) << 2) + eg] = byte_plane(x[0], x[1], x[2], x[3], w);
+}
+__global__ __launch_bounds__(256) void k_ssp_image(const uint32_t *__restrict__ ssp, uint32_t m, uint32_t d, uint32_t KS, uint4 *__restrict__ img) {
+  const uint64_t gid = (uint64_t)blockIdx.x * blockDim.x + threadIdx.x;
+  const uint32_t k = (uint32_t)(gid % d), rest = (uint32_t)(gid / d), g4 = rest & 3, ks = rest >> 2;
+  if (ks >= KS) return;
+  const uint32_t r0 = 64 * ks + 16 * g4;
+  uint32_t x[16];
+#pragma unroll
+  for (int e = 0; e < 16; e++) x[e] = (r0 + e < m ? ssp[(uint64_t)(r0 + e + 1) * d + k] : 0u) ^ 0x80808080u;
+  uint4 *o = img + (((uint64_t)(k >> 2) * KS + ks) * 64 + 16 * g4 + 4 * (k & 3));
+#pragma unroll
+  for (int w = 0; w < 4; w++)
+    o[w] = uint4{byte_plane(x[0], x[1], x[2], x[3], w), byte_plane(x[4], x[5], x[6], x[7], w), byte_plane(x[8], x[9], x[10], x[11], w),
+                 byte_plane(x[12], x[13], x[14], x[15], w)};
 }
 struct WCols {
   uint32_t kt0;
@@ -594,7 +608,79 @@
 
 }
 
+const uint8_t *ssp_image(mfh_ctx *c, const uint32_t *d_ssp) {
+  const uint32_t d = c->P.d, m = c->P.m;
+  if (!d_ssp || d % 64 || m < 2) return nullptr;
+  const uint32_t KS = (m + 255) / 256 * 4;
+  const size_t bytes = (size_t)(d / 4) * KS * 1024;
+  if (c->ssp_img_src == d_ssp && c->ssp_img.cap >= bytes) return c->ssp_img.as<uint8_t>();
+  c->ssp_img_src = nullptr;
+  if (c->ssp_img.cap < bytes) {
+    if (c->ssp_img.p) {
+      (void)hipDeviceSynchronize();
+      dev_free(c->ssp_img);
+    }
+    size_t mem_free = 0, mem_total = 0;
+    if (hipMemGetInfo(&mem_free, &mem_total) != hipSuccess) mem_free = 0;
+    if (bytes > mem_free / 4 * 3 || !dev_alloc(c->ssp_img, bytes)) {
+      (void)hipGetLastError();
+      return nullptr;
+    }
+  }
+  hipLaunchKernelGGL(k_ssp_image, dim3((uint32_t)((uint64_t)d * KS * 4 / 256)), dim3(256), 0, c->stream, d_ssp, m, d, KS, c->ssp_img.as<uint4>());
+  if (hipGetLastError() != hipSuccess || hipStreamSynchronize(c->stream) != hipSuccess) return nullptr;
+  c->ssp_img_src = d_ssp;
+  return c->ssp_img.as<uint8_t>();
+}
+
 extern "C" {
+
+int mfh_witness_poly_stream(mfh_ctx *c, const uint32_t *d_ssp, uint32_t nstmt, const uint8_t *h_bits, size_t bits_stride, const uint32_t *h_delta, uint32_t *d_w) {
+  if (!witness_args_ok(c, nstmt, 0xffffffffu, h_bits, h_delta, d_w)) return MFH_EINVAL;
+  const uint32_t d = c->P.d, m = c->P.m;
+  if (!d_ssp || d % 64 || m < 2 || !mms_ssp_ok(c)) { c->err = "mfh_witness_poly_stream: a dense SSP, d a multiple of 64 and packed partial products"; return MFH_EUNSUPPORTED; }
+  const uint32_t bstride = (m + 6) / 8;
+  if (bits_stride < bstride) { c->err = "bits_stride shorter than the m - 1 witness bits"; return MFH_EINVAL; }
+  if (int rc = witness_deltas(c, nstmt, h_delta)) return rc;
+  HIP_TRY(c, hipSetDevice(c->device));
+  const uint8_t *img = ssp_image(c, d_ssp);
+  if (!img) { c->err = "mfh_witness_poly_stream: no room for the SSP image"; return MFH_ENOMEM; }
+  constexpr uint32_t SG = 255, NG = 8;
+  for (uint32_t s0 = 0; s0 < nstmt; s0 += SG * NG) {
+    const uint32_t cnt = std::min(SG * NG, nstmt - s0), ng = (cnt + SG - 1) / SG;
+    MmsPlan P;
+    if (!mms_plan_ssp(c, img, ng, P)) return MFH_EINVAL;
+    const size_t head_g = up256((size_t)SG * bstride + 3) + up256((size_t)SG * 4), delta_off = up256((size_t)SG * bstride + 3);
+    const WwsCarve<4> ws({head_g * ng, (size_t)ng * 2048, P.cd_bytes * ng, P.part_bytes * ng});
+    if (int rc = ws.reserve(c)) return rc;
+    PinBuf &wpin = c->pin_wring[c->pin_wnext++ % 8];
+    uint8_t *stage = (uint8_t *)pin_acquire(c, wpin, head_g * ng);
+    if (!stage) return MFH_ENOMEM;
+    uint8_t *dev = ws.at<uint8_t>(c, 0);
+    MmIo ios[NG];
+    uint32_t nvs[NG], *W[NG];
+    const uint32_t *dl[NG];
+    for (uint32_t g = 0; g < ng; g++) {
+      const uint32_t b0 = s0 + g * SG, sg = std::min(SG, nstmt - b0);
+      for (uint32_t b = 0; b < sg; b++) memcpy(stage + g * head_g + (size_t)b * bstride, h_bits + (size_t)(b0 + b) * bits_stride, bstride);
+      memcpy(stage + g * head_g + delta_off, h_delta + b0, (size_t)sg * 4);
+      ios[g] = MmIo{{nullptr, nullptr}, sg, {nullptr, nullptr}, sg, 0, dev + g * head_g, bstride, ws.at<int64_t>(c, 1) + 256 * g};
+      nvs[g] = sg;
+      dl[g] = (const uint32_t *)(dev + g * head_g + delta_off);
+      W[g] = d_w + (size_t)b0 * d;
+    }
+    HIP_TRY(c, hipMemcpyAsync(dev, stage, head_g * ng, hipMemcpyHostToDevice, c->stream));
+    pin_release(c, wpin);
+    HIP_TRY(c, hipMemsetAsync(ws.at<uint8_t>(c, 1), 0, (size_t)ng * 2048, c->stream));
+    P.cd = ws.at<int8_t>(c, 2);
+    P.part = ws.at<int>(c, 3);
+    int rc = mms_digits(c, P, ios, nvs);
+    if (!rc) rc = mms_stream(c, P);
+    if (!rc) rc = mms_witness_finish(c, P, ios, nvs, d_ssp, dl, W);
+    if (rc) return rc;
+  }
+  return MFH_OK;
+}
 
 int mfh_ssp_set_prg(mfh_ctx *c, uint64_t seed, const uint32_t *d_t) {
   if (!c) return MFH_EINVAL;
diff --git a/include/mfhip.h b/include/mfhip.h
--- a/include/mfhip.h
+++ b/include/mfhip.h
@@ -225,6 +225,7 @@
 int mfh_set_witness_per(mfh_ctx *ctx, uint32_t statements);
 int mfh_set_batch_launch(mfh_ctx *ctx, uint32_t groups_per_launch, int merge_regions);
 int mfh_set_batch_bw(mfh_ctx *ctx, int merged);
+int mfh_set_batch_witness(mfh_ctx *ctx, int streamed);
 int mfh_set_mm_stream(mfh_ctx *ctx, int map, int persistent, int sync_mode, uint32_t spin_max);
 int mfh_set_mm_width(mfh_ctx *ctx, uint32_t per_xcd, int early_chain);
 int mfh_set_mm_queue(mfh_ctx *ctx, int mode, uint32_t start_shift, int prefix);
@@ -259,6 +260,8 @@
                         uint32_t *d_w);
 int mfh_witness_poly_mm_cols(mfh_ctx *ctx, const uint32_t *d_ssp, uint32_t nstmt, const uint8_t *h_bits, size_t bits_stride, const uint32_t *h_delta,
                              uint32_t col0, uint32_t ncols, uint32_t *d_w, size_t w_stride);
+int mfh_witness_poly_stream(mfh_ctx *ctx, const uint32_t *d_ssp, uint32_t nstmt, const uint8_t *h_bits, size_t bits_stride, const uint32_t *h_delta,
+                            uint32_t *d_w);
 int mfh_witness_lanes(mfh_ctx *ctx, const uint32_t *d_ssp, const uint8_t *h_witness_bits, uint32_t rank, uint32_t world, uint64_t *d_lanes);
 int mfh_witness_from_lanes(mfh_ctx *ctx, const uint32_t *d_ssp, const uint64_t *d_lanes, uint32_t delta, uint32_t *d_w);
 int mfh_prove_partial_w(mfh_ctx *ctx, const uint8_t *d_crs_c8, const uint32_t *d_ssp, const uint8_t *h_witness_bits, uint32_t delta,
```

Result: faster. 14440 (median of 6 runs) (+1.3%).
